# johnnyjana730/MVIN

Measured on AMD Instinct MI355X. Metric: (user,item) pairs scored/sec @ dim=64 hop=2 fan-out=32; % HBM roofline, higher is better.
Workload: dtype f32

## Files before the change

### include/mvin_hip.h

```cpp
#ifndef MVIN_HIP_H
#define MVIN_HIP_H

#include <stddef.h>
#include <stdint.h>

#ifdef __cplusplus
extern "C" {
#endif

#define MVIN_ABI_VERSION 12
#define MVIN_API __attribute__((visibility("default")))
#define MVIN_MAX_DIM 256
#define MVIN_MAX_SRC 8

MVIN_API int mvin_abi_version(void);
MVIN_API const char* mvin_last_error(void);

MVIN_API int mvin_debug_read_trace(long long* host_dst, size_t n);

MVIN_API size_t mvin_ent_elems(int B, int K, int levels);
MVIN_API size_t mvin_rel_elems(int B, int K, int levels);

MVIN_API int mvin_expand_ids(const int32_t* adj_entity, const int32_t* adj_relation,
                    const int64_t* items_i64, const int32_t* items_i32,
                    int B, int K, int levels, int n_entity,
                    int32_t* ent_out, int32_t* rel_out, void* stream);

MVIN_API int mvin_rel_score(const float* relation_emb, const float* urh_weights, int nR, int D,
                   float* t_out, void* stream);

typedef struct {
    const float* src[MVIN_MAX_SRC];
    const int32_t* ids[MVIN_MAX_SRC];
    int nsrc;
    int Dsrc;
    int Dout;
    int64_t rows;
    const float* W;
    const float* bias;
    const float* rowbias;
    int rows_per_group;
    int relu;
    int ids64;
    int sum_sources;
    float* out;
    int64_t ldo;
    int nz;
    int64_t w_zstride, bias_zstride, out_zstride;
    const float* score_u;
    float* score_out;
    float* sigmoid_out;
    int src_bf16;
    int64_t src_rows;
} mvin_linear_args;
MVIN_API int mvin_linear_fwd(const mvin_linear_args* args, void* stream);

MVIN_API int mvin_gather_attn_fwd(const float* table, const int32_t* adj_entity, const int32_t* adj_relation,
                         const int32_t* node_ids, const float* rel_score,
                         const float* self_vec, const float* Wc, const float* c_child,
                         const float* Wagg, const float* bagg,
                         int B, int N, int K, int D, int n_entity,
                         float* out, float* probs, void* stream);

MVIN_API int mvin_gather_attn_l2_fwd(const void* table, const int32_t* adj_entity, const int32_t* adj_relation,
                            const int32_t* parent_ids, const float* t0, const float* t1,
                            const float* W1, const float* W2, const float* b1, const float* b2,
                            const float* q, const float* A0, const float* a0,
                            int B, int parents_per_pair, int K, int D, int n_entity, int nR,
                            float* nagg0, float* nagg1, float* probs_parent, float* probs_child,
                            int table_bf16, void* stream);
MVIN_API int mvin_gather_attn_l2_fwd_i64(const void* table, const int32_t* adj_entity, const int32_t* adj_relation,
                                const int64_t* parent_ids, const float* t0, const float* t1,
                                const float* W1, const float* W2, const float* b1, const float* b2,
                                const float* q, const float* A0, const float* a0,
                                int B, int parents_per_pair, int K, int D, int n_entity, int nR,
                                float* nagg0, float* nagg1, float* probs_parent, float* probs_child,
                                int table_bf16, void* stream);
MVIN_API int mvin_gather_attn_l2_supported(int D, int K);
MVIN_API int mvin_gather_attn_l2_enc_fwd(const void* table, const int32_t* enc_entity, const int32_t* enc_relation,
                                const void* parent_ids, int parent_ids_i64, const float* t0, const float* t1,
                                const float* W1, const float* W2, const float* b1, const float* b2,
                                const float* q, const float* A0, const float* a0,
                                int B, int parents_per_pair, int K, int D, int n_entity, int nR,
                                float* nagg0, float* nagg1, int table_bf16, void* stream);
MVIN_API int mvin_gather_attn_l2_enc_supported(int D, int K);
MVIN_API int mvin_gather_attn_l2_prj_supported(int D, int K, int adjacency_encoded, int n_entity, int nR);
MVIN_API int mvin_project_rows(const float* src, int64_t rows, int D, const float* W1, const float* W2, const float* b1,
                               const float* b2, float* out, void* stream);
MVIN_API size_t mvin_project_tables_elems(int n_entity, int D);
MVIN_API int mvin_project_tables(const float* entity_emb, const float* W1, const float* W2, const float* b1, const float* b2,
                                 const float* A0, const float* a0, int attention, int K, int n_entity, int D, float* ws,
                                 void* stream);
MVIN_API int mvin_gather_attn_l2_prj_fwd(const float* ws, const int32_t* enc_entity, const int32_t* enc_relation, int adjacency_encoded,
                                const void* parent_ids, int parent_ids_i64, const float* t0, const float* t1, const float* q,
                                int B, int parents_per_pair, int K, int D, int n_entity, int nR, float* nagg0, float* nagg1,
                                void* stream);
MVIN_API size_t mvin_order_by_key_ws_elems(int64_t B);
MVIN_API int mvin_order_by_key(const int64_t* keys_i64, const int32_t* keys_i32, int64_t B, int32_t* workspace, int32_t* order, void* stream);
MVIN_API int mvin_gather_attn_l2_prj_ordered_fwd(const float* ws, const int32_t* enc_entity, const int32_t* enc_relation, int adjacency_encoded,
                                const void* parent_ids, int parent_ids_i64, const int32_t* order, const float* t0, const float* t1,
                                const float* q, int B, int parents_per_pair, int K, int D, int n_entity, int nR, float* nagg0,
                                float* nagg1, void* stream);
MVIN_API int mvin_gather_attn_l2_agg_supported(int D, int K, int n_entity, int nR);
MVIN_API size_t mvin_entity_aggregates_elems(int n_entity, int D);
MVIN_API int mvin_entity_aggregates(const float* ws, const int32_t* enc_entity, const int32_t* enc_relation, const float* t0, int K, int D,
                                    int n_entity, int nR, float* agg, void* stream);
MVIN_API int mvin_gather_attn_l2_agg_fwd(const float* ws, const float* agg, const int32_t* enc_entity, const int32_t* enc_relation,
                                const void* parent_ids, int parent_ids_i64, const int32_t* order, const float* t0, const float* t1,
                                const float* q, int B, int parents_per_pair, int K, int D, int n_entity, int nR, float* nagg0,
                                float* nagg1, void* stream);
MVIN_API int mvin_score_l2_folded_supported(int D, int K, int n_entity, int nR);
MVIN_API size_t mvin_fold_tables_elems(int n_entity, int D);
MVIN_API int mvin_fold_tables(const float* entity_emb, const int32_t* enc_entity, const int32_t* enc_relation, const float* t0, const float* W0,
                              const float* b0, const float* W1, const float* b1, const float* W2, const float* b2, const float* A0,
                              const float* a0, const float* Wmix, const float* bmix, const float* A1, int K, int D, int n_entity, int nR,
                              float* ws, void* stream);
MVIN_API int mvin_fold_tables_ex(const float* entity_emb, const int32_t* enc_entity, const int32_t* enc_relation, const float* t0, const float* W0,
                                 const float* b0, const float* W1, const float* b1, const float* W2, const float* b2, const float* A0,
                                 const float* a0, const float* Wmix, const float* bmix, const float* A1, int aggregates, int K, int D,
                                 int n_entity, int nR, float* ws, void* stream);
MVIN_API int mvin_score_l2_folded_gather_supported(int D, int K, int n_entity, int nR);
MVIN_API int mvin_score_l2_folded_gather_fwd(const float* ws, const int32_t* enc_entity, const int32_t* enc_relation, const int64_t* items_i64,
                                             const int32_t* items_i32, const int32_t* order, const float* t0, const float* t1, const float* q,
                                             const float* user_o, const float* A1, const float* a1, const float* Wmix, int64_t B, int K, int D,
                                             int n_entity, int nR, float* item_emb, float* scores, float* sig, void* stream);
MVIN_API int mvin_score_l2_folded_fwd(const float* ws, const int32_t* enc_entity, const int32_t* enc_relation, const int64_t* items_i64,
                                      const int32_t* items_i32, const float* t0, const float* t1, const float* q, const float* user_o,
                                      const float* A1, const float* a1, const float* Wmix, int64_t B, int K, int D, int n_entity, int nR,
                                      float* out0, float* z2, float* item_emb, float* scores, float* sig, void* stream);
MVIN_API int mvin_gather_attn_l2_variant(int D, int K, int64_t n_parents, int n_entity, int want_probs);
MVIN_API int mvin_gather_attn_l2_variant_ex(int D, int K, int64_t n_parents, int n_entity, int want_probs, int table_bf16);
MVIN_API int mvin_probe_gather_l2(const void* table, const int32_t* child_ids, const int32_t* grandchild_ids, int64_t n_parents, int K,
                         int D, int n_entity, int table_bf16, float* sums, void* stream);

MVIN_API int mvin_agg_fwd(const float* self_vec, const float* neigh, const int32_t* rel_ids,
                 const float* rel_score, const float* Wagg, const float* bagg,
                 int B, int N, int K, int D, float* out, float* probs, void* stream);

MVIN_API int mvin_ripple_attn_fwd(const float* entity_emb, const int32_t* score_ids, const int32_t* rel_ids,
                         const int32_t* value_ids, const float* V, const float* w, int mode,
                         int B, int Nm, int D, int nR, float* out, int64_t ldo, void* stream);
MVIN_API int mvin_ripple_attn_fwd_ex(const void* entity_emb, const int32_t* score_ids, const int32_t* rel_ids,
                            const int32_t* value_ids, const float* V, const float* w, int mode,
                            int B, int Nm, int D, int nR, float* out, int64_t ldo, int table_bf16, void* stream);

MVIN_API int mvin_key_addressing_fwd(const void* entity_emb, const float* V, const float* w,
                            const int32_t* const* mem_h, const int32_t* const* mem_r,
                            const int32_t* const* mem_t, int P, int B, int Nm, int D, int nR, int n_entity,
                            float* out, int64_t ldo, int table_bf16, void* stream);
MVIN_API int mvin_key_addressing_supported(int Nm, int D);
MVIN_API int mvin_key_addressing_users_fwd(const void* entity_emb, const float* V, const float* w, const int32_t* uts,
                                  const int64_t* users_i64, const int32_t* users_i32, int P, int B, int Nm, int D, int nR,
                                  int n_entity, int n_user, float* out, int64_t ldo, int table_bf16, void* stream);

MVIN_API int mvin_key_addressing_grouped_fwd(const void* entity_emb, const float* relation_kge, const float* w,
                                    const int32_t* uts, const int32_t* seg_user, const int32_t* seg_ptr,
                                    const int32_t* nseg_dev, const int32_t* pair_index, const int64_t* items_i64,
                                    const int32_t* items_i32, int nseg, int B, int P, int Nm, int D, int nR, int n_entity, int n_user,
                                    float* out, int64_t ldo, int table_bf16, void* stream);
MVIN_API int mvin_key_addressing_grouped_supported(int D, int P, int Nm, int nR);
MVIN_API int mvin_user_records_len(int P, int Nm, int nR);
MVIN_API int mvin_user_records_supported(int D, int P, int Nm, int nR, int table_bf16);
MVIN_API int mvin_build_user_records(const int32_t* uts, int n_user, int P, int Nm, int nR, int n_entity, int32_t* records, void* stream);
MVIN_API int mvin_key_addressing_grouped_rec_fwd(const void* entity_emb, const float* relation_kge, const float* w,
                                        const int32_t* uts, const int32_t* user_records, const int32_t* seg_user,
                                        const int32_t* seg_ptr, const int32_t* nseg_dev, const int32_t* pair_index,
                                        const int64_t* items_i64, const int32_t* items_i32, int nseg, int B, int P, int Nm, int D,
                                        int nR, int n_entity, int n_user, float* out, int64_t ldo, int table_bf16, void* stream);
MVIN_API size_t mvin_project_relations_elems(int n_entity, int nR, int D);
MVIN_API int mvin_project_relations(const float* entity_emb, const float* relation_kge, const float* w, int n_entity, int nR, int D,
                                    float* ws, void* stream);
MVIN_API int mvin_key_addressing_grouped_er_supported(int D, int P, int Nm, int nR, int n_entity, int has_set);
MVIN_API int mvin_key_addressing_grouped_er_fwd(const void* entity_emb, const float* relation_kge, const float* w,
                                       const int32_t* uts, const int32_t* user_records, const float* er_ws, const int32_t* seg_user,
                                       const int32_t* seg_ptr, const int32_t* nseg_dev, const int32_t* pair_index,
                                       const int64_t* items_i64, const int32_t* items_i32, int nseg, int B, int P, int Nm, int D,
                                       int nR, int n_entity, int n_user, float* out, int64_t ldo, void* stream);
MVIN_API int mvin_key_addressing_flash_supported(int D, int P, int Nm, int nR, int n_entity);
MVIN_API size_t mvin_key_addressing_flash_tables_elems(int n_entity, int nR, int D, int P, int has_set);
MVIN_API int mvin_key_addressing_flash_prepare(const float* entity_emb, const float* relation_kge, const float* w,
                                      const float* user_mlp_W, int n_entity, int nR, int D, int P, float* ws, void* stream);
MVIN_API size_t mvin_key_addressing_flash_ws_elems(int64_t B, int n_user);
MVIN_API int mvin_key_addressing_flash_fwd(const float* entity_emb, const float* ws, const int32_t* user_records,
                                  const int32_t* seg_user, const int32_t* seg_ptr, const int32_t* nseg_dev, const int32_t* pair_index,
                                  const int64_t* items_i64, const int32_t* items_i32, int64_t B, int P, int Nm, int D, int nR,
                                  int n_entity, int n_user, int has_set, const float* user_mlp_b, float* user_o,
                                  int32_t* sched_ws, void* stream);
MVIN_API int mvin_group_pairs_by_user(const int64_t* users_i64, const int32_t* users_i32, int64_t B, int n_user, int32_t* workspace,
                             int32_t* seg_user, int32_t* seg_ptr, int32_t* nseg, int32_t* pair_index, void* stream);

MVIN_API int mvin_row_softmax_fwd(const float* x, int64_t rows, int n, float* out, void* stream);

MVIN_API int mvin_mix_neighbor_vectors_fwd(const float* neighbor_vectors, const float* neighbor_relations, const float* user_embeddings,
                                           const float* logits_or_null, int B, int N, int K, int D, float* out, float* probs_or_null,
                                           void* stream);

MVIN_API int mvin_l2_tail_fwd(const void* entity_emb, const int64_t* items_i64, const int32_t* items_i32, const float* q,
                     const float* user_o, const float* nagg0, const float* nagg1, const float* W0, const float* b0,
                     const float* A0, const float* a0, const float* A1, const float* a1, const float* Wmix,
                     const float* bmix, int64_t B, int D, int n_entity, float* item_emb, float* scores, float* sig,
                     int table_bf16, void* stream);
MVIN_API int mvin_l2_tail_supported(int D);

typedef struct {
    const void* entity_emb;
    const int32_t* adj_entity;
    const int32_t* adj_relation;
    const float* relation_kge;
    const float* h_set_w;
    const float* user_mlp_W;
    const float* user_mlp_b;
    const float* t0;
    const float* t1;
    const float* W0;
    const float* b0;
    const float* W1;
    const float* b1;
    const float* W2;
    const float* b2;
    const float* A0;
    const float* a0;
    const float* A1;
    const float* a1;
    const float* Wmix;
    const float* bmix;
    const int64_t* items;
    const int32_t* const* mem_h;
    const int32_t* const* mem_r;
    const int32_t* const* mem_t;
    const int32_t* uts;
    const int64_t* users;
    float* V;
    float* o_cat;
    int32_t* parents;
    float* nagg0;
    float* nagg1;
    float* user_o;
    float* item_emb;
    float* scores;
    float* sig;
    int64_t B;
    int D, K, P, Nm, n_entity, n_relation, table_bf16;
    int n_user;
    const int32_t* enc_entity;
    const int32_t* enc_relation;
    int32_t* group_ws;
    const int32_t* user_records;
    int depth;
    float* prj_tables;
    float* ka_er;
    float* ka_flash;
    int32_t* item_order_ws;
    float* agg_tables;
    float* fold_ws;
    int fold_gather;
} mvin_score_l2_args;
MVIN_API int mvin_score_l2_fwd(const mvin_score_l2_args* args, void* stream);

MVIN_API int mvin_score_small_fwd(const mvin_score_l2_args* args, int group, void* stream);
MVIN_API int mvin_score_small_supported(int D, int K, int P, int Nm, int nR);

MVIN_API int mvin_gather_rows(const void* table, const int32_t* ids, int64_t n, int row_bytes, void* out, void* stream);
MVIN_API int mvin_scatter_rows(void* table, const int32_t* ids, int64_t n, int row_bytes, const void* rows, void* stream);
MVIN_API int mvin_shard_space_ids(const void* ids, int ids_are_i64, int64_t n, int world, int n_local, void* out, void* stream);

MVIN_API int mvin_gather_mix_fwd(const void* table, const int32_t* adj_entity, const int32_t* adj_relation,
                        const int32_t* node_ids, const float* rel_score, const float* rowbias, int64_t nodes,
                        int nodes_per_group, int K, int D, int n_entity, int nR, int relu, float* out,
                        int table_bf16, void* stream);


MVIN_API int mvin_gather_attn_fwd_ex(const void* table, const int32_t* adj_entity, const int32_t* adj_relation,
                            const int32_t* node_ids, const float* rel_score, const float* self_vec,
                            const float* Wc, const float* c_child, const float* Wagg, const float* bagg,
                            int B, int N, int K, int D, int n_entity, float* out, float* probs,
                            float* s_out, float* z_out, int table_bf16, void* stream);
MVIN_API int mvin_agg_fwd_ex(const float* self_vec, const float* neigh, const int32_t* rel_ids, const float* rel_score,
                    const float* Wagg, const float* bagg, int B, int N, int K, int D, float* out, float* probs,
                    float* s_out, float* z_out, void* stream);

MVIN_API int mvin_eltwise(int mode, int64_t n, float* x, float* y, float* z, float* w, float* accum, float alpha,
                 float beta, float beta1, float beta2, float eps, int D, int N, void* stream);
// ... 156 lines not shown
```

### mvin_amd/_lib.py

```python
import ctypes as C
import os

from . import build as _build

MAX_SRC = 8
ABI_VERSION = 12

_c_f32p = C.c_void_p
_c_i32p = C.c_void_p


class LinearArgs(C.Structure):
    _fields_ = [
        ("src", C.c_void_p * MAX_SRC),
        ("ids", C.c_void_p * MAX_SRC),
        ("nsrc", C.c_int),
        ("Dsrc", C.c_int),
        ("Dout", C.c_int),
        ("rows", C.c_int64),
        ("W", C.c_void_p),
        ("bias", C.c_void_p),
        ("rowbias", C.c_void_p),
        ("rows_per_group", C.c_int),
        ("relu", C.c_int),
        ("ids64", C.c_int),
        ("sum_sources", C.c_int),
        ("out", C.c_void_p),
        ("ldo", C.c_int64),
        ("nz", C.c_int),
        ("w_zstride", C.c_int64),
        ("bias_zstride", C.c_int64),
        ("out_zstride", C.c_int64),
        ("score_u", C.c_void_p),
        ("score_out", C.c_void_p),
        ("sigmoid_out", C.c_void_p),
        ("src_bf16", C.c_int),
        ("src_rows", C.c_int64),
    ]


class WgradProblem(C.Structure):
    _fields_ = [
        ("lin", LinearArgs),
        ("dY", C.c_void_p),
        ("ldy", C.c_int64),
        ("dy_zstride", C.c_int64),
        ("mask", C.c_void_p),
        ("ldm", C.c_int64),
        ("mask_zstride", C.c_int64),
        ("dW", C.c_void_p),
        ("dw_zstride", C.c_int64),
        ("db", C.c_void_p),
        ("db_zstride", C.c_int64),
    ]


class ScoreL2Args(C.Structure):
    _fields_ = [(n, C.c_void_p) for n in (
        "entity_emb", "adj_entity", "adj_relation", "relation_kge", "h_set_w", "user_mlp_W", "user_mlp_b", "t0", "t1",
        "W0", "b0", "W1", "b1", "W2", "b2", "A0", "a0", "A1", "a1", "Wmix", "bmix", "items", "mem_h", "mem_r", "mem_t",
        "uts", "users", "V", "o_cat", "parents", "nagg0", "nagg1", "user_o", "item_emb", "scores", "sig")] + [
        ("B", C.c_int64)] + [(n, C.c_int) for n in ("D", "K", "P", "Nm", "n_entity", "n_relation", "table_bf16", "n_user")] + [
        ("enc_entity", C.c_void_p), ("enc_relation", C.c_void_p), ("group_ws", C.c_void_p),
        ("user_records", C.c_void_p), ("depth", C.c_int), ("prj_tables", C.c_void_p), ("ka_er", C.c_void_p),
        ("ka_flash", C.c_void_p), ("item_order_ws", C.c_void_p), ("agg_tables", C.c_void_p), ("fold_ws", C.c_void_p), ("fold_gather", C.c_int)]


SIGNATURES = {
    "mvin_abi_version": (C.c_int, []),
    "mvin_last_error": (C.c_char_p, []),
    "mvin_debug_read_trace": (C.c_int, [C.c_void_p, C.c_size_t]),
    "mvin_l2_tail_fwd": (C.c_int, [C.c_void_p] * 15 + [C.c_int64, C.c_int, C.c_int] + [C.c_void_p] * 3 + [C.c_int, C.c_void_p]),
    "mvin_l2_tail_supported": (C.c_int, [C.c_int]),
    "mvin_score_l2_fwd": (C.c_int, [C.c_void_p, C.c_void_p]),
    "mvin_score_small_fwd": (C.c_int, [C.c_void_p, C.c_int, C.c_void_p]),
    "mvin_mix_neighbor_vectors_fwd": (C.c_int, [C.c_void_p] * 4 + [C.c_int] * 4 + [C.c_void_p] * 3),
    "mvin_score_small_supported": (C.c_int, [C.c_int] * 5),
    "mvin_project_rows": (C.c_int, [C.c_void_p, C.c_int64, C.c_int] + [C.c_void_p] * 6),
    "mvin_project_tables_elems": (C.c_size_t, [C.c_int, C.c_int]),
    "mvin_project_tables": (C.c_int, [C.c_void_p] * 7 + [C.c_int] * 4 + [C.c_void_p] * 2),
    "mvin_gather_attn_l2_prj_fwd": (C.c_int, [C.c_void_p] * 3 + [C.c_int] + [C.c_void_p] + [C.c_int] + [C.c_void_p] * 3 + [C.c_int] * 6 + [C.c_void_p] * 3),
    "mvin_topk_rows_supported": (C.c_int, [C.c_int]),
    "mvin_topk_rows_ws_bytes": (C.c_int64, [C.c_int64, C.c_int64, C.c_int]),
    "mvin_topk_rows": (C.c_int, [C.c_void_p, C.c_int64, C.c_int64, C.c_int64, C.c_void_p, C.c_int64] + [C.c_void_p] * 4
                       + [C.c_int] + [C.c_void_p] * 4),
    "mvin_rank_positives_ws_bytes": (C.c_int64, [C.c_int64] * 3),
    "mvin_rank_positives": (C.c_int, [C.c_void_p, C.c_int64, C.c_int64, C.c_int64, C.c_void_p, C.c_int64] + [C.c_void_p] * 9),
    "mvin_kg_explore_ws_bytes": (C.c_int64, [C.c_int64, C.c_int64]),
    "mvin_kg_field": (C.c_int, [C.c_void_p] * 3 + [C.c_int64, C.c_int64, C.c_void_p, C.c_int64, C.c_int] + [C.c_void_p] * 4),
    "mvin_kg_explore": (C.c_int, [C.c_void_p] * 3 + [C.c_int64, C.c_int64, C.c_void_p, C.c_void_p, C.c_int, C.c_void_p, C.c_int64,
                                  C.c_int] + [C.c_void_p] * 4),
    "mvin_ctr_counts_ws_bytes": (C.c_int64, [C.c_int64, C.c_int64]),
    "mvin_ctr_counts": (C.c_int, [C.c_void_p, C.c_void_p, C.c_int64, C.c_int64, C.c_int64, C.c_void_p, C.c_void_p, C.c_void_p]),
    "mvin_order_by_key_ws_elems": (C.c_size_t, [C.c_int64]),
    "mvin_order_by_key": (C.c_int, [C.c_void_p, C.c_void_p, C.c_int64, C.c_void_p, C.c_void_p, C.c_void_p]),
    "mvin_gather_attn_l2_prj_ordered_fwd": (C.c_int, [C.c_void_p] * 3 + [C.c_int] + [C.c_void_p] + [C.c_int] + [C.c_void_p] * 4 + [C.c_int] * 6 + [C.c_void_p] * 3),
    "mvin_gather_attn_l2_agg_supported": (C.c_int, [C.c_int] * 4),
    "mvin_entity_aggregates_elems": (C.c_size_t, [C.c_int] * 2),
    "mvin_entity_aggregates": (C.c_int, [C.c_void_p] * 4 + [C.c_int] * 4 + [C.c_void_p] * 2),
    "mvin_gather_attn_l2_agg_fwd": (C.c_int, [C.c_void_p] * 5 + [C.c_int] + [C.c_void_p] * 4 + [C.c_int] * 6 + [C.c_void_p] * 3),
    "mvin_score_l2_folded_supported": (C.c_int, [C.c_int] * 4),
    "mvin_fold_tables_elems": (C.c_size_t, [C.c_int] * 2),
    "mvin_fold_tables": (C.c_int, [C.c_void_p] * 15 + [C.c_int] * 4 + [C.c_void_p] * 2),
    "mvin_fold_tables_ex": (C.c_int, [C.c_void_p] * 15 + [C.c_int] * 5 + [C.c_void_p] * 2),
    "mvin_score_l2_folded_gather_supported": (C.c_int, [C.c_int] * 4),
    "mvin_score_l2_folded_gather_fwd": (C.c_int, [C.c_void_p] * 13 + [C.c_int64] + [C.c_int] * 4 + [C.c_void_p] * 4),
    "mvin_score_l2_folded_fwd": (C.c_int, [C.c_void_p] * 12 + [C.c_int64] + [C.c_int] * 4 + [C.c_void_p] * 6),
    "mvin_gather_rows": (C.c_int, [C.c_void_p, C.c_void_p, C.c_int64, C.c_int, C.c_void_p, C.c_void_p]),
    "mvin_scatter_rows": (C.c_int, [C.c_void_p, C.c_void_p, C.c_int64, C.c_int, C.c_void_p, C.c_void_p]),
    "mvin_linear_wgrad_multi": (C.c_int, [C.c_void_p, C.c_int, C.c_void_p]),
    "mvin_shard_space_ids": (C.c_int, [C.c_void_p, C.c_int, C.c_int64, C.c_int, C.c_int, C.c_void_p, C.c_void_p]),
    "mvin_key_addressing_grouped_fwd": (C.c_int, [C.c_void_p] * 10 + [C.c_int] * 8 + [C.c_void_p, C.c_int64, C.c_int, C.c_void_p]),
    "mvin_key_addressing_grouped_rec_fwd": (C.c_int, [C.c_void_p] * 11 + [C.c_int] * 8 + [C.c_void_p, C.c_int64, C.c_int, C.c_void_p]),
    "mvin_project_relations_elems": (C.c_size_t, [C.c_int] * 3),
    "mvin_project_relations": (C.c_int, [C.c_void_p] * 3 + [C.c_int] * 3 + [C.c_void_p] * 2),
    "mvin_key_addressing_grouped_er_supported": (C.c_int, [C.c_int] * 6),
    "mvin_key_addressing_flash_supported": (C.c_int, [C.c_int] * 5),
    "mvin_key_addressing_flash_tables_elems": (C.c_size_t, [C.c_int] * 5),
    "mvin_key_addressing_flash_prepare": (C.c_int, [C.c_void_p] * 4 + [C.c_int] * 4 + [C.c_void_p] * 2),
    "mvin_key_addressing_flash_ws_elems": (C.c_size_t, [C.c_int64, C.c_int]),
    "mvin_key_addressing_flash_fwd": (C.c_int, [C.c_void_p] * 9 + [C.c_int64] + [C.c_int] * 7 + [C.c_void_p] * 4),
    "mvin_key_addressing_grouped_er_fwd": (C.c_int, [C.c_void_p] * 12 + [C.c_int] * 8 + [C.c_void_p, C.c_int64, C.c_void_p]),
    "mvin_user_records_len": (C.c_int, [C.c_int] * 3),
    "mvin_user_records_supported": (C.c_int, [C.c_int] * 5),
    "mvin_build_user_records": (C.c_int, [C.c_void_p, C.c_int, C.c_int, C.c_int, C.c_int, C.c_int, C.c_void_p, C.c_void_p]),
    "mvin_key_addressing_grouped_supported": (C.c_int, [C.c_int] * 4),
    "mvin_ent_elems": (C.c_size_t, [C.c_int, C.c_int, C.c_int]),
    "mvin_rel_elems": (C.c_size_t, [C.c_int, C.c_int, C.c_int]),
    "mvin_expand_ids": (C.c_int, [_c_i32p, _c_i32p, C.c_void_p, _c_i32p, C.c_int, C.c_int, C.c_int,
                                  C.c_int, _c_i32p, _c_i32p, C.c_void_p]),
    "mvin_rel_score": (C.c_int, [_c_f32p, _c_f32p, C.c_int, C.c_int, _c_f32p, C.c_void_p]),
    "mvin_linear_fwd": (C.c_int, [C.POINTER(LinearArgs), C.c_void_p]),
    "mvin_gather_attn_fwd": (C.c_int, [_c_f32p, _c_i32p, _c_i32p, _c_i32p, _c_f32p, _c_f32p, _c_f32p,
                                       _c_f32p, _c_f32p, _c_f32p, C.c_int, C.c_int, C.c_int, C.c_int,
                                       C.c_int, _c_f32p, _c_f32p, C.c_void_p]),
    "mvin_gather_attn_l2_fwd": (C.c_int, [_c_f32p, _c_i32p, _c_i32p, _c_i32p, _c_f32p, _c_f32p, _c_f32p,
                                          _c_f32p, _c_f32p, _c_f32p, _c_f32p, _c_f32p, _c_f32p, C.c_int, C.c_int,
                                          C.c_int, C.c_int, C.c_int, C.c_int, _c_f32p, _c_f32p, _c_f32p,
                                          _c_f32p, C.c_int, C.c_void_p]),
    "mvin_gather_attn_l2_fwd_i64": (C.c_int, [_c_f32p, _c_i32p, _c_i32p, C.c_void_p, _c_f32p, _c_f32p, _c_f32p,
                                              _c_f32p, _c_f32p, _c_f32p, _c_f32p, _c_f32p, _c_f32p, C.c_int, C.c_int,
                                              C.c_int, C.c_int, C.c_int, C.c_int, _c_f32p, _c_f32p, _c_f32p,
                                              _c_f32p, C.c_int, C.c_void_p]),
    "mvin_gather_attn_l2_supported": (C.c_int, [C.c_int, C.c_int]),
    "mvin_gather_attn_l2_enc_fwd": (C.c_int, [_c_f32p, _c_i32p, _c_i32p, C.c_void_p, C.c_int, _c_f32p, _c_f32p, _c_f32p,
                                              _c_f32p, _c_f32p, _c_f32p, _c_f32p, _c_f32p, _c_f32p, C.c_int, C.c_int,
                                              C.c_int, C.c_int, C.c_int, C.c_int, _c_f32p, _c_f32p, C.c_int, C.c_void_p]),
    "mvin_gather_attn_l2_enc_supported": (C.c_int, [C.c_int, C.c_int]),
    "mvin_gather_attn_l2_prj_supported": (C.c_int, [C.c_int, C.c_int, C.c_int, C.c_int, C.c_int]),
    "mvin_encode_adjacency": (C.c_int, [_c_i32p, _c_i32p, C.c_int, C.c_int, _c_i32p, _c_i32p, _c_i32p, C.c_void_p]),
    "mvin_gather_attn_l2_variant": (C.c_int, [C.c_int, C.c_int, C.c_int64, C.c_int, C.c_int]),
    "mvin_gather_attn_l2_variant_ex": (C.c_int, [C.c_int, C.c_int, C.c_int64, C.c_int, C.c_int, C.c_int]),
    "mvin_probe_gather_l2": (C.c_int, [C.c_void_p, C.c_void_p, C.c_void_p, C.c_int64, C.c_int, C.c_int, C.c_int, C.c_int,
                                      C.c_void_p, C.c_void_p]),
    "mvin_agg_fwd": (C.c_int, [_c_f32p, _c_f32p, _c_i32p, _c_f32p, _c_f32p, _c_f32p, C.c_int, C.c_int,
                               C.c_int, C.c_int, _c_f32p, _c_f32p, C.c_void_p]),
    "mvin_key_addressing_fwd": (C.c_int, [_c_f32p, _c_f32p, _c_f32p, C.POINTER(C.c_void_p),
                                          C.POINTER(C.c_void_p), C.POINTER(C.c_void_p), C.c_int, C.c_int,
                                          C.c_int, C.c_int, C.c_int, C.c_int, _c_f32p, C.c_int64, C.c_int,
                                          C.c_void_p]),
    "mvin_key_addressing_supported": (C.c_int, [C.c_int, C.c_int]),
    "mvin_count_ids": (C.c_int, [C.c_void_p, C.c_int64, C.c_int, C.c_void_p, C.c_void_p]),
    "mvin_group_pairs_by_user": (C.c_int, [C.c_void_p, C.c_void_p, C.c_int64, C.c_int, C.c_void_p, C.c_void_p, C.c_void_p,
                                           C.c_void_p, C.c_void_p, C.c_void_p]),
    "mvin_key_addressing_users_fwd": (C.c_int, [C.c_void_p, C.c_void_p, C.c_void_p, C.c_void_p, C.c_void_p, C.c_void_p,
                                                C.c_int, C.c_int, C.c_int, C.c_int, C.c_int, C.c_int, C.c_int, C.c_void_p,
                                                C.c_int64, C.c_int, C.c_void_p]),
    "mvin_row_softmax_fwd": (C.c_int, [_c_f32p, C.c_int64, C.c_int, _c_f32p, C.c_void_p]),
    "mvin_gather_mix_fwd": (C.c_int, [_c_f32p, _c_i32p, _c_i32p, _c_i32p, _c_f32p, _c_f32p, C.c_int64, C.c_int,
                                      C.c_int, C.c_int, C.c_int, C.c_int, C.c_int, _c_f32p, C.c_int, C.c_void_p]),
    "mvin_sample_adjacency": (C.c_int, [C.c_void_p, _c_i32p, _c_i32p, C.c_int, C.c_int, C.c_uint64, _c_i32p,
                                        _c_i32p, C.c_void_p]),
    "mvin_build_ripple_sets": (C.c_int, [C.c_void_p, _c_i32p, _c_i32p, C.c_void_p, _c_i32p, C.c_int, C.c_int,
                                         C.c_int, C.c_int, C.c_uint64, _c_i32p, C.c_void_p]),
    "mvin_sample_negatives_supported": (C.c_int, [C.c_int]),
    "mvin_sample_negatives": (C.c_int, [C.c_void_p, _c_i32p, _c_i32p, C.c_void_p, C.c_int, C.c_int, C.c_uint64, C.c_uint64,
                                        _c_i32p, C.c_void_p, C.c_void_p]),
    "mvin_sample_negatives_weighted_supported": (C.c_int, [C.c_int]),
    "mvin_sample_negatives_weighted": (C.c_int, [C.c_void_p, _c_i32p, _c_i32p, C.c_void_p, C.c_int, C.c_int, C.c_void_p, C.c_void_p,
                                                 C.c_uint64, C.c_uint64, _c_i32p, C.c_void_p, C.c_void_p]),
    "mvin_rank_head": (C.c_int, [_c_f32p, _c_f32p, _c_f32p, C.c_int64, C.c_int, C.c_int, C.c_int, C.c_float] + [_c_f32p] * 5
                       + [C.c_void_p, C.c_void_p]),
    "mvin_rank_head_offset": (C.c_int, [_c_f32p, _c_f32p, _c_f32p, _c_f32p, C.c_int64, C.c_int, C.c_int, C.c_int, C.c_float]
                              + [_c_f32p] * 5 + [C.c_void_p, C.c_void_p]),
    "mvin_select_negatives": (C.c_int, [_c_f32p, C.c_void_p, _c_f32p, C.c_void_p, C.c_int64, C.c_int, C.c_int, C.c_int, C.c_uint64,
                                        C.c_uint64, C.c_void_p, _c_f32p, _c_f32p, C.c_void_p, C.c_void_p]),
    "mvin_gather_attn_fwd_ex": (C.c_int, [_c_f32p, _c_i32p, _c_i32p, _c_i32p, _c_f32p, _c_f32p, _c_f32p,
                                          _c_f32p, _c_f32p, _c_f32p, C.c_int, C.c_int, C.c_int, C.c_int,
                                          C.c_int, _c_f32p, _c_f32p, _c_f32p, _c_f32p, C.c_int, C.c_void_p]),
    "mvin_agg_fwd_ex": (C.c_int, [_c_f32p, _c_f32p, _c_i32p, _c_f32p, _c_f32p, _c_f32p, C.c_int, C.c_int,
                                  C.c_int, C.c_int, _c_f32p, _c_f32p, _c_f32p, _c_f32p, C.c_void_p]),
    "mvin_l2_adam_multi": (C.c_int, [C.c_void_p, C.c_int, C.c_int64, _c_f32p, _c_f32p, _c_f32p, _c_f32p, C.c_int,
                                     C.c_float, C.c_float, C.c_float, C.c_float, C.c_void_p]),
    "mvin_l2_adam_multi_dev": (C.c_int, [C.c_void_p, C.c_int, C.c_int64, _c_f32p, _c_f32p, _c_f32p, _c_f32p, C.c_int,
                                         _c_f32p, C.c_float, C.c_float, C.c_float, C.c_void_p]),
    "mvin_grad_guard": (C.c_int, [C.c_void_p, C.c_int, C.c_int64, _c_f32p, C.c_void_p, C.c_int, C.c_void_p, _c_f32p, C.c_int,
                                  C.c_void_p, C.c_int, C.c_void_p]),
    "mvin_l2_adam_multi_guarded": (C.c_int, [C.c_void_p, C.c_int, C.c_int64, _c_f32p, _c_f32p, _c_f32p, _c_f32p, C.c_int,
                                             C.c_void_p, C.c_float, C.c_float, C.c_float, C.c_void_p]),
    "mvin_eltwise": (C.c_int, [C.c_int, C.c_int64, _c_f32p, _c_f32p, _c_f32p, _c_f32p, _c_f32p, C.c_float,
                               C.c_float, C.c_float, C.c_float, C.c_float, C.c_int, C.c_int, C.c_void_p]),
    "mvin_scatter_add_rows": (C.c_int, [_c_f32p, C.c_void_p, C.c_int, _c_f32p, C.c_int64, C.c_int, C.c_float,
                                        C.c_void_p]),
    "mvin_linear_wgrad": (C.c_int, [C.POINTER(LinearArgs), _c_f32p, C.c_int64, C.c_int64, _c_f32p, C.c_int64,
                                    C.c_int64, _c_f32p, C.c_int64, _c_f32p, C.c_int64, C.c_void_p]),
    "mvin_agg_bwd": (C.c_int, [_c_f32p, _c_i32p, _c_i32p, _c_i32p, _c_f32p, _c_i32p, _c_f32p, _c_f32p, _c_f32p, C.c_int64,
                               C.c_int, C.c_int, C.c_int, _c_f32p, _c_f32p, _c_f32p, C.c_void_p]),
    "mvin_rel_score_bwd": (C.c_int, [_c_f32p, _c_f32p, _c_f32p, C.c_int, C.c_int, _c_f32p, _c_f32p, C.c_void_p]),
    "mvin_key_addressing_bwd": (C.c_int, [_c_f32p, _c_f32p, _c_f32p, C.POINTER(C.c_void_p), C.POINTER(C.c_void_p),
                                          C.POINTER(C.c_void_p), C.c_int, C.c_int, C.c_int, C.c_int, C.c_int,
                                          _c_f32p, C.c_int64, C.c_float, _c_f32p, _c_f32p, _c_f32p, C.c_void_p]),
    "mvin_key_addressing_bwd_reg": (C.c_int, [_c_f32p, _c_f32p, _c_f32p, C.POINTER(C.c_void_p), C.POINTER(C.c_void_p),
                                              C.POINTER(C.c_void_p), C.c_int, C.c_int, C.c_int, C.c_int, C.c_int,
                                              _c_f32p, C.c_int64, C.c_float, _c_f32p, _c_f32p, _c_f32p, C.c_int,
                                              _c_f32p, _c_f32p, C.c_void_p, C.c_int, C.c_void_p]),
    "mvin_key_addressing_bwd_adds_item_grad": (C.c_int, [C.c_int, C.c_int, C.c_int, C.c_int]),
    "mvin_ripple_attn_fwd": (C.c_int, [_c_f32p, _c_i32p, _c_i32p, _c_i32p, _c_f32p, _c_f32p, C.c_int,
                                       C.c_int, C.c_int, C.c_int, C.c_int, _c_f32p, C.c_int64,
                                       C.c_void_p]),
    "mvin_ripple_attn_fwd_ex": (C.c_int, [C.c_void_p, _c_i32p, _c_i32p, _c_i32p, _c_f32p, _c_f32p, C.c_int,
                                          C.c_int, C.c_int, C.c_int, C.c_int, _c_f32p, C.c_int64, C.c_int,
                                          C.c_void_p]),
}

_lib = None


class MvinHipError(RuntimeError):
    pass


def lib_path():
    return _build.LIB_PATH


def load():
    global _lib
    if _lib is not None:
        return _lib
    path = lib_path()
    if not os.path.exists(path):
        raise MvinHipError(
            f"{path} is missing: build it with `python -m mvin_amd.build` (hipcc, gfx950). "
            "mvin_amd has no CPU fallback.")
    import torch
    hip_rt = os.path.join(os.path.dirname(torch.__file__), "lib", "libamdhip64.so")
    if os.path.exists(hip_rt):
        C.CDLL(hip_rt, mode=C.RTLD_GLOBAL)
    lib = C.CDLL(path)
    for name, (res, args) in SIGNATURES.items():
        fn = getattr(lib, name)
        fn.restype = res
        fn.argtypes = args
    ver = lib.mvin_abi_version()
    if ver != ABI_VERSION:
        raise MvinHipError(f"libmvin_hip.so ABI version {ver}, expected {ABI_VERSION}")
    _lib = lib
    return lib


# ... 5 lines not shown
```

### mvin_amd/csrc/mvin_abi.hip

```cpp
#include <cstdlib>
#include <cstdarg>
#include <cstdio>
#include <string>

#include "mvin_kernels.h"
#include "mvin_fused_agg.h"

namespace {

thread_local std::string g_last_error;

int fail(int code, const char* fmt, ...) {
    char buf[512];
    va_list ap;
    va_start(ap, fmt);
    vsnprintf(buf, sizeof(buf), fmt, ap);
    va_end(ap);
    g_last_error = buf;
    return code;
}

int hip_result(hipError_t e, const char* what) {
    if (e == hipSuccess) return 0;
    fail((int)e, "%s: %s", what, hipGetErrorString(e));
// ... 520 lines not shown
    mvin::FusedL2Args f{};
    f.K = K;
    f.nR = nR;
    f.P = n_parents > 0 ? n_parents : 1;
    f.prj = 1;
    f.parents_per_pair = 1;
    f.max_id = (unsigned)(n_entity - 1);
    static const int32_t present = 0;
    f.adj_r = &present;
    f.table_bytes = (uint64_t)n_entity * (uint64_t)D * 4;
    f.adj_bytes = (uint64_t)n_entity * (uint64_t)K * 4;
    return mvin::fused_agg_applies(f, D);
}

int mvin_gather_attn_l2_agg_supported(int D, int K, int n_entity, int nR) { return agg_applies(D, K, n_entity, nR, 1) ? 1 : 0; }

size_t mvin_entity_aggregates_elems(int n_entity, int D) { return n_entity > 0 && D > 0 ? (size_t)2 * n_entity * D : 0; }

int mvin_entity_aggregates(const float* ws, const int32_t* enc_entity, const int32_t* enc_relation, const float* t0, int K, int D,
                           int n_entity, int nR, float* agg, void* stream) {
    const char* who = "mvin_entity_aggregates";
    if (!ws || !enc_entity || !enc_relation || !agg) return fail(-1, "%s: null pointer", who);
    if (!agg_applies(D, K, n_entity, nR, 1))
        return fail(-3, "%s: D = 64, K in {16, 32, 64}, n_entity <= 2^24, tables < 1 GiB, adjacency < 2 GiB, nR <= 4096 (D=%d K=%d n_entity=%d nR=%d)",
                    who, D, K, n_entity, nR);
    mvin::EntityAggArgs f{};
    const size_t tab = (size_t)n_entity * D;
    f.tabS = ws;
    f.selfG = ws + tab;
    f.tabG = ws + 2 * tab;
    f.adj_e = enc_entity;
    f.adj_r = enc_relation;
    f.t0 = t0;
    f.outS = agg;
    f.outG = agg + tab;
    f.n_entity = n_entity;
    f.K = K;
    f.nR = nR;
    f.table_bytes = (uint64_t)n_entity * (uint64_t)D * 4;
    f.adj_bytes = (uint64_t)n_entity * (uint64_t)K * 4;
    return hip_result(mvin::launch_entity_aggregates(f, (hipStream_t)stream), who);
}

int mvin_gather_attn_l2_agg_fwd(const float* ws, const float* agg, const int32_t* enc_entity, const int32_t* enc_relation,
                                const void* parent_ids, int parent_ids_i64, const int32_t* order, const float* t0, const float* t1,
                                const float* q, int B, int parents_per_pair, int K, int D, int n_entity, int nR, float* nagg0,
                                float* nagg1, void* stream) {
    if (!ws || !agg || n_entity <= 0 || D <= 0) return fail(-1, "mvin_gather_attn_l2_agg_fwd: null workspace / bad sizes");
    const float* blk = ws + (size_t)3 * n_entity * D;
    const float* Wv = blk + (size_t)3 * D * D;
    const float* b1c = Wv + (size_t)D * D;
    return gather_attn_l2_impl(ws, enc_entity, enc_relation, reinterpret_cast<const int32_t*>(parent_ids), parent_ids_i64 ? 2 : 1, t0, t1,
                               blk, Wv, b1c, b1c + D, q, blk, nullptr, B, parents_per_pair, K, D, n_entity, nR, nagg0, nagg1, nullptr,
                               nullptr, 0, stream, true, true, order, agg);
}

static bool fold_gather_applies(int D, int K, int n_entity, int nR, int64_t B);

static bool fold_applies(int D, int K, int n_entity, int nR, int64_t B) {
    if (D == 64) return agg_applies(D, K, n_entity, nR, B);
    static const char* e = getenv("MVIN_L2_AGG");
    if (e && e[0] == '0') return false;
    if (n_entity <= 0 || nR <= 0 || nR > 4096 || !mvin::fused_fold_supported(D, K)) return false;
    const uint64_t tb = (uint64_t)n_entity * (uint64_t)D * 4, ab = (uint64_t)n_entity * (uint64_t)K * 4;
    return tb < (1ull << 30) && ab < (1ull << 31) && n_entity <= (1 << 24) && (B <= 0 || (uint64_t)B * D * 4 < (1ull << 31)) &&
           mvin::fused_fold_lds_bytes(D, nR, K) <= 48 * 1024;
}

static size_t fold_blk_elems(int D) { return (size_t)12 * D * D + (size_t)3 * D; }

size_t mvin_fold_tables_elems(int n_entity, int D) {
    return n_entity > 0 && D > 0 ? (size_t)6 * n_entity * D + fold_blk_elems(D) : 0;
}

int mvin_score_l2_folded_supported(int D, int K, int n_entity, int nR) { return fold_applies(D, K, n_entity, nR, 1) ? 1 : 0; }

int mvin_fold_tables(const float* entity_emb, const int32_t* enc_entity, const int32_t* enc_relation, const float* t0, const float* W0,
                     const float* b0, const float* W1, const float* b1, const float* W2, const float* b2, const float* A0, const float* a0,
                     const float* Wmix, const float* bmix, const float* A1, int K, int D, int n_entity, int nR, float* ws, void* stream) {
    return mvin_fold_tables_ex(entity_emb, enc_entity, enc_relation, t0, W0, b0, W1, b1, W2, b2, A0, a0, Wmix, bmix, A1, 1, K, D, n_entity, nR, ws,
                               stream);
}

static int fold_tables_check(const char* who, const float* entity_emb, const int32_t* enc_entity, const int32_t* enc_relation, const float* W0,
                             const float* W1, const float* W2, const float* A0, const float* Wmix, const float* A1, int aggregates, int K, int D,
                             int n_entity, int nR, const float* ws) {
    if (!entity_emb || !enc_entity || !enc_relation || !W0 || !W1 || !W2 || !A0 || !Wmix || !A1 || !ws) return fail(-1, "%s: null pointer", who);
    if (!(aggregates ? fold_applies(D, K, n_entity, nR, 1) : fold_gather_applies(D, K, n_entity, nR, 1)))
        return fail(-3, "%s: D = 64 with K in {16, 32, 64} or D = 32 with K in {16, 32}; n_entity <= 2^24, tables < 1 GiB, adjacency < 2 GiB, nR <= 4096 "
                        "(D=%d K=%d n_entity=%d nR=%d)", who, D, K, n_entity, nR);
    return 0;
}

static int fold_tables_block(const char* who, const float* t0, const float* W0, const float* b0, const float* W1, const float* b1, const float* W2,
                             const float* b2, const float* A0, const float* a0, const float* Wmix, const float* bmix, const float* A1, int K, int D,
                             int n_entity, float* ws, void* stream) {
    const float c = t0 ? 1.f / (float)K : 1.f;
    return hip_result(mvin::launch_fold_prepare(W0, b0, W1, b1, W2, b2, A0, a0, Wmix, bmix, A1, c, D, ws + (size_t)6 * n_entity * D,
                                                (hipStream_t)stream), who);
}

static int fold_tables_aggregates(const char* who, const int32_t* enc_entity, const int32_t* enc_relation, const float* t0, int K, int D,
                                  int n_entity, int nR, float* ws, void* stream) {
    const size_t tab = (size_t)n_entity * D;
    mvin::EntityAggArgs f{};
    f.tabS = ws;
    f.selfS = ws + 2 * tab;
    f.tabG = ws + tab;
    f.selfG = ws;
    f.adj_e = enc_entity;
    f.adj_r = enc_relation;
    f.t0 = t0;
    f.outS = ws + 4 * tab;
    f.outG = ws + 5 * tab;
    f.n_entity = n_entity;
    f.K = K;
    f.D = D;
    f.nR = nR;
    f.table_bytes = (uint64_t)tab * 4;
    f.adj_bytes = (uint64_t)n_entity * (uint64_t)K * 4;
    return hip_result(mvin::launch_entity_aggregates(f, (hipStream_t)stream), who);
}

int mvin_fold_tables_ex(const float* entity_emb, const int32_t* enc_entity, const int32_t* enc_relation, const float* t0, const float* W0,
                        const float* b0, const float* W1, const float* b1, const float* W2, const float* b2, const float* A0, const float* a0,
                        const float* Wmix, const float* bmix, const float* A1, int aggregates, int K, int D, int n_entity, int nR, float* ws,
                        void* stream) {
    const char* who = "mvin_fold_tables";
    if (int rc = fold_tables_check(who, entity_emb, enc_entity, enc_relation, W0, W1, W2, A0, Wmix, A1, aggregates, K, D, n_entity, nR, ws)) return rc;
    if (int rc = fold_tables_block(who, t0, W0, b0, W1, b1, W2, b2, A0, a0, Wmix, bmix, A1, K, D, n_entity, ws, stream)) return rc;
    float* blk = ws + (size_t)6 * n_entity * D;
    if (D == 64) {
        if (int rc = build_entity_tables(who, entity_emb, n_entity, nullptr, 0, nullptr, nullptr, 0, nullptr, blk, ws, stream)) return rc;
    } else {
        mvin_linear_args l{};
        l.src[0] = entity_emb;
        l.nsrc = 1;
        l.Dsrc = D;
        l.Dout = D;
        l.rows = n_entity;
        l.rows_per_group = 1;
        l.W = blk;
        l.w_zstride = (int64_t)D * D;
        l.out = ws;
        l.ldo = D;
        l.nz = 4;
        l.out_zstride = (int64_t)n_entity * D;
        if (int rc = mvin_linear_fwd(&l, stream)) return rc;
    }
    if (!aggregates) return 0;
    return fold_tables_aggregates(who, enc_entity, enc_relation, t0, K, D, n_entity, nR, ws, stream);
}

int mvin_score_l2_folded_fwd(const float* ws, const int32_t* enc_entity, const int32_t* enc_relation, const int64_t* items_i64,
                             const int32_t* items_i32, const float* t0, const float* t1, const float* q, const float* user_o, const float* A1,
                             const float* a1, const float* Wmix, int64_t B, int K, int D, int n_entity, int nR, float* out0, float* z2,
                             float* item_emb, float* scores, float* sig, void* stream) {
    const char* who = "mvin_score_l2_folded_fwd";
    if (!ws || !enc_entity || !enc_relation || !q || !user_o || !A1 || !Wmix || !scores) return fail(-1, "%s: null pointer", who);
    if ((items_i64 == nullptr) == (items_i32 == nullptr)) return fail(-1, "%s: exactly one of items_i64 / items_i32", who);
    if (B <= 0 || B >= (int64_t(1) << 31)) return fail(-2, "%s: B=%lld", who, (long long)B);
    if (!fold_applies(D, K, n_entity, nR, B)) return fail(-3, "%s: unsupported shape / sizes D=%d K=%d n_entity=%d nR=%d B=%lld", who, D, K, n_entity, nR, (long long)B);
    const size_t tab = (size_t)n_entity * D;
    const float* blk = ws + 6 * tab;
    const float* Wv = blk + (size_t)4 * D * D;
    const float* Wq = Wv + (size_t)D * D;
    const float* bv = Wq + (size_t)D * D;
    const float* bq = bv + D;
    const float* bm = bq + D;
    static const bool two = getenv("MVIN_L2_FOLD_TWO") && atoi(getenv("MVIN_L2_FOLD_TWO")) != 0;
    if (!two || D != 64)
    {
        const float* Wp = bm + D;
        const size_t DD = (size_t)D * D;
        return hip_result(mvin::launch_score_l2_folded(ws + 4 * tab, ws + 3 * tab, enc_entity, enc_relation,
                                                       items_i64 ? reinterpret_cast<const int32_t*>(items_i64) : items_i32, items_i64 ? 2 : 1, t1, q,
                                                       user_o, Wp, bq, Wp + DD, bv, Wp + 2 * DD, Wp + 3 * DD, a1, Wp + 4 * DD, Wp + 5 * DD, bm,
                                                       item_emb, scores, sig, B, K, D, nR, n_entity, (hipStream_t)stream),
                          who);
    }
    if (!out0 || !z2) return fail(-1, "%s: the two-launch variant (MVIN_L2_FOLD_TWO=1) needs the out0 / z2 scratch rows", who);
    mvin::FusedL2Args f{};
    f.table = ws;
    f.agg = const_cast<float*>(ws + 4 * tab);
    f.adj_e = enc_entity;
    f.adj_r = enc_relation;
    f.parent_ids = items_i64 ? reinterpret_cast<const int32_t*>(items_i64) : items_i32;
    f.pid_stride = items_i64 ? 2 : 1;
    f.t0 = t0;
    f.t1 = t1;
    f.W1 = Wq;
    f.b1 = bq;
    f.W2 = Wv;
    f.b2 = bv;
    f.q = q;
    f.nagg0 = out0;
    f.nagg1 = z2;
    f.P = B;
    f.table_bytes = (uint64_t)tab * 4;
    f.adj_bytes = (uint64_t)n_entity * (uint64_t)K * 4;
    f.parents_per_pair = 1;
    f.K = K;
    f.nR = nR;
    f.max_id = (unsigned)(n_entity - 1);
    f.prj = 1;
    f.fold = 1;
    if (int rc = hip_result(mvin::launch_gather_attn_l2_agg(f, (hipStream_t)stream), who)) return rc;
    mvin::TailFoldArgs t{};
    t.M0 = ws + 3 * tab;
    t.items64 = items_i64;
    t.items32 = items_i32;
    t.q = q;
    t.user_o = user_o;
    t.out0 = out0;
    t.z2 = z2;
    t.Wqm = blk + (size_t)3 * D * D;
    t.A1 = A1;
    t.a1 = a1;
    t.Wmix = Wmix;
    t.bm = bm;
    t.item_emb = item_emb;
    t.scores = scores;
    t.sig = sig;
    t.B = B;
    t.n_entity = n_entity;
    return hip_result(mvin::launch_l2_tail_fold(t, (hipStream_t)stream), who);
}

static bool fold_gather_applies(int D, int K, int n_entity, int nR, int64_t B) {
    if (D != 64 || (K != 16 && K != 32) || n_entity <= 0 || nR <= 0 || nR > 4096) return false;
    static const char* e = getenv("MVIN_L2_FOLD_GATHER");
    if (e && e[0] == '0') return false;
    const uint64_t tb = (uint64_t)n_entity * (uint64_t)D * 4, ab = (uint64_t)n_entity * (uint64_t)K * 4;
    return tb < (1ull << 30) && ab < (1ull << 31) && n_entity <= (1 << 24) && (B <= 0 || (uint64_t)B * D * 4 < (1ull << 31)) &&
           mvin::fused_wppfold_lds_bytes(nR, K) <= 48 * 1024;
}

int mvin_score_l2_folded_gather_supported(int D, int K, int n_entity, int nR) { return fold_gather_applies(D, K, n_entity, nR, 1) ? 1 : 0; }

int mvin_score_l2_folded_gather_fwd(const float* ws, const int32_t* enc_entity, const int32_t* enc_relation, const int64_t* items_i64,
                                    const int32_t* items_i32, const int32_t* order, const float* t0, const float* t1, const float* q,
                                    const float* user_o, const float* A1, const float* a1, const float* Wmix, int64_t B, int K, int D,
                                    int n_entity, int nR, float* item_emb, float* scores, float* sig, void* stream) {
    const char* who = "mvin_score_l2_folded_gather_fwd";
    if (!ws || !enc_entity || !enc_relation || !q || !user_o || !A1 || !Wmix || !scores) return fail(-1, "%s: null pointer", who);
    if ((items_i64 == nullptr) == (items_i32 == nullptr)) return fail(-1, "%s: exactly one of items_i64 / items_i32", who);
    if (B <= 0 || B >= (int64_t(1) << 31)) return fail(-2, "%s: B=%lld", who, (long long)B);
    if (!fold_gather_applies(D, K, n_entity, nR, B))
        return fail(-3, "%s: D = 64, K in {16, 32}; n_entity <= 2^24, tables < 1 GiB, adjacency < 2 GiB (D=%d K=%d n_entity=%d nR=%d B=%lld)", who, D, K,
                    n_entity, nR, (long long)B);
    const size_t tab = (size_t)n_entity * D, DD = (size_t)D * D;
    const float* blk = ws + 6 * tab;
    const float* bv = blk + 6 * DD;
    const float* bq = bv + D;
    const float* bm = bq + D;
    const float* Wp = bm + D;
    mvin::FoldArgs f{};
    f.tables = ws;
    f.M0 = ws + 3 * tab;
    f.adj_e = enc_entity;
    f.adj_r = enc_relation;
    f.items = items_i64 ? reinterpret_cast<const int32_t*>(items_i64) : items_i32;
    f.pid_stride = items_i64 ? 2 : 1;
    f.order = order;
    f.t0 = t0;
    f.t1 = t1;
    f.q = q;
    f.user_o = user_o;
    f.Wq = Wp, f.bq = bq, f.Wv = Wp + DD, f.bv = bv, f.Wqm = Wp + 2 * DD, f.A1 = Wp + 3 * DD, f.a1 = a1, f.Wm1 = Wp + 4 * DD, f.Wm2 = Wp + 5 * DD, f.bm = bm;
    f.item_emb = item_emb, f.scores = scores, f.sig = sig;
    f.B = B, f.K = K, f.nR = nR;
    f.max_id = (unsigned)(n_entity - 1);
    f.table_bytes = (uint64_t)tab * 4;
    f.adj_bytes = (uint64_t)n_entity * (uint64_t)K * 4;
    return hip_result(mvin::launch_score_l2_folded_gather(f, (hipStream_t)stream), who);
}

int mvin_encode_adjacency(const int32_t* adj_entity, const int32_t* adj_relation, int n_entity, int K, int32_t* cnt,
                          int32_t* enc_entity, int32_t* enc_relation, void* stream) {
    const char* who = "mvin_encode_adjacency";
    if (!adj_entity || !cnt || !enc_entity || !enc_relation) return fail(-1, "%s: null pointer", who);
    if (n_entity <= 0 || n_entity > (1 << 24) || K <= 0 || K > 128)
        return fail(-2, "%s: n_entity=%d K=%d (n_entity <= 2^24, K <= 128)", who, n_entity, K);
    return hip_result(mvin::launch_encode_adjacency(adj_entity, adj_relation, n_entity, K, cnt, enc_entity, enc_relation,
                                                    (hipStream_t)stream), who);
}

int mvin_gather_attn_l2_fwd(const void* table, const int32_t* adj_entity, const int32_t* adj_relation,
                            const int32_t* parent_ids, const float* t0, const float* t1, const float* W1,
                            const float* W2, const float* b1, const float* b2, const float* q,
                            const float* A0, const float* a0, int B, int parents_per_pair, int K, int D, int n_entity, int nR,
                            float* nagg0, float* nagg1, float* probs_parent, float* probs_child,
                            int table_bf16, void* stream) {
    return gather_attn_l2_impl(table, adj_entity, adj_relation, parent_ids, 1, t0, t1, W1, W2, b1, b2, q, A0, a0, B,
                               parents_per_pair, K, D, n_entity, nR, nagg0, nagg1, probs_parent, probs_child,
                               table_bf16, stream);
}

int mvin_gather_attn_l2_fwd_i64(const void* table, const int32_t* adj_entity, const int32_t* adj_relation,
                                const int64_t* parent_ids, const float* t0, const float* t1, const float* W1,
                                const float* W2, const float* b1, const float* b2, const float* q,
                                const float* A0, const float* a0, int B, int parents_per_pair, int K, int D, int n_entity, int nR,
                                float* nagg0, float* nagg1, float* probs_parent, float* probs_child,
                                int table_bf16, void* stream) {
    return gather_attn_l2_impl(table, adj_entity, adj_relation, reinterpret_cast<const int32_t*>(parent_ids), 2, t0, t1, W1, W2,
                               b1, b2, q, A0, a0, B, parents_per_pair, K, D, n_entity, nR, nagg0, nagg1, probs_parent,
                               probs_child, table_bf16, stream);
}

int mvin_agg_fwd(const float* self_vec, const float* neigh, const int32_t* rel_ids, const float* rel_score,
                 const float* Wagg, const float* bagg, int B, int N, int K, int D, float* out, float* probs,
                 void* stream) {
    return mvin_agg_fwd_ex(self_vec, neigh, rel_ids, rel_score, Wagg, bagg, B, N, K, D, out, probs, nullptr,
                           nullptr, stream);
}

int mvin_agg_fwd_ex(const float* self_vec, const float* neigh, const int32_t* rel_ids, const float* rel_score,
                    const float* Wagg, const float* bagg, int B, int N, int K, int D, float* out, float* probs,
                    float* s_out, float* z_out, void* stream) {
    mvin::GatherAttnArgs g{};
    g.s_out = s_out;
    g.z_out = z_out;
    g.gather = 0;
    g.neigh = neigh;
    g.rel_ids = rel_ids;
    g.rel_score = rel_score;
    g.self_vec = self_vec;
    g.Wagg = Wagg;
    g.bagg = bagg;
    g.out = out;
    g.probs = probs;
// ... 122 lines not shown
    if (B <= 0 || n_entity <= 0) return fail(-2, "%s: bad sizes B=%lld n_entity=%d", who, (long long)B, n_entity);
    mvin::TailArgs t{};
    t.E = entity_emb;
    t.items64 = items_i64;
    t.items32 = items_i32;
    t.q = q;
    t.user_o = user_o;
    t.nagg0 = nagg0;
    t.nagg1 = nagg1;
    t.W0 = W0;
    t.b0 = b0;
    t.A0 = A0;
    t.a0 = a0;
    t.A1 = A1;
    t.a1 = a1;
    t.Wmix = Wmix;
    t.bmix = bmix;
    t.item_emb = item_emb;
    t.scores = scores;
    t.sig = sig;
    t.B = B;
    t.table_bf16 = table_bf16;
    t.n_entity = n_entity;
    return hip_result(mvin::launch_l2_tail(t, D, (hipStream_t)stream), who);
}

static int flash_prepare_impl(const char* who, const float* entity_emb, const float* relation_kge, const float* w, const float* user_mlp_W,
                              int n_entity, int nR, int D, int P, float* ws, float* fold_ws, void* stream);

int mvin_score_l2_fwd(const mvin_score_l2_args* a, void* stream) {
    const char* who = "mvin_score_l2_fwd";
    if (!a) return fail(-1, "%s: null args", who);
    if (a->P < 1 || a->P > 8) return fail(-2, "%s: P=%d (1..8)", who, a->P);
    const bool grouped = a->uts && a->group_ws;
    if ((!a->V && !grouped) || !a->o_cat || !a->parents || !a->nagg0 || !a->nagg1 || !a->user_o || !a->scores || !a->items)
        return fail(-1, "%s: null workspace / output / items", who);
    if (a->uts && !a->users) return fail(-1, "%s: user_triplet_set given without user ids", who);
    if (a->group_ws && !a->uts) return fail(-1, "%s: group_ws is for the users feed (uts + users)", who);
    const int D = a->D, nR = a->n_relation;
    const int n_o = a->P + (a->h_set_w ? 1 : 0);
    mvin_linear_args l{};
    l.src[0] = reinterpret_cast<const float*>(a->entity_emb);
    l.ids[0] = reinterpret_cast<const int32_t*>(a->items);
    l.ids64 = 1;
    l.src_bf16 = a->table_bf16 ? 1 : 0;
    l.src_rows = a->n_entity;
    l.nsrc = 1;
    l.Dsrc = D;
    l.Dout = D;
    l.rows = a->B;
    l.W = a->relation_kge;
    l.rows_per_group = 1;
    l.out = a->V;
    l.ldo = (int64_t)nR * D;
    l.nz = nR;
    l.w_zstride = (int64_t)D * D;
    l.out_zstride = D;
    int rc = 0;
    bool flash = false;
    const bool fold_ok = a->fold_ws && a->enc_entity && a->enc_relation && a->W0 && a->W1 && a->W2 && !a->table_bf16;
    const int fold_form = !fold_ok ? 0 : a->fold_gather ? (fold_gather_applies(D, a->K, a->n_entity, nR, a->B) ? 2 : 0)
                                                        : (fold_applies(D, a->K, a->n_entity, nR, a->B) ? 1 : 0);
    bool fold_built = false;
    if (grouped) {
        int32_t* ws = a->group_ws;
        int32_t* seg_user = ws + 2 * (size_t)a->n_user + (size_t)a->B;
        int32_t* seg_ptr = seg_user + a->B;
        int32_t* nseg = seg_ptr + a->B + 2;
        int32_t* pair_index = nseg + 1;
        rc = mvin_group_pairs_by_user(a->users, nullptr, a->B, a->n_user, ws, seg_user, seg_ptr, nseg, pair_index, stream);
        if (rc) return rc;
        if (a->ka_flash && a->user_records && !a->table_bf16 && mvin::key_addr_flash_supported(D, a->P, a->Nm, nR, a->n_entity)) {
            if (fold_form) {
                rc = fold_tables_check("mvin_fold_tables", reinterpret_cast<const float*>(a->entity_emb), a->enc_entity, a->enc_relation, a->W0, a->W1,
                                       a->W2, a->A0, a->Wmix, a->A1, fold_form == 1, a->K, D, a->n_entity, nR, a->fold_ws);
                if (rc) return rc;
                rc = fold_tables_block("mvin_fold_tables", a->t0, a->W0, a->b0, a->W1, a->b1, a->W2, a->b2, a->A0, a->a0, a->Wmix, a->bmix, a->A1,
                                       a->K, D, a->n_entity, a->fold_ws, stream);
                if (rc) return rc;
                fold_built = true;
            }
            rc = flash_prepare_impl("mvin_key_addressing_flash_prepare", reinterpret_cast<const float*>(a->entity_emb), a->relation_kge, a->h_set_w,
                                    a->user_mlp_W, a->n_entity, nR, D, a->P, a->ka_flash, fold_built ? a->fold_ws : nullptr, stream);
            if (rc) return rc;
            if (mvin_key_addressing_flash_ws_elems(a->B, a->n_user) > (size_t)2 * a->n_user + (size_t)a->B)
                return fail(-2, "%s: group_ws too small for the flash form's scheduling scratch", who);
            rc = mvin_key_addressing_flash_fwd(reinterpret_cast<const float*>(a->entity_emb), a->ka_flash, a->user_records, seg_user, seg_ptr,
                                               nseg, pair_index, a->items, nullptr, a->B, a->P, a->Nm, D, nR, a->n_entity, a->n_user,
                                               a->h_set_w != nullptr, a->user_mlp_b, a->user_o, ws, stream);
            flash = true;
        } else if (a->ka_er && a->user_records && !a->table_bf16 &&
            mvin_key_addressing_grouped_er_supported(D, a->P, a->Nm, nR, a->n_entity, a->h_set_w != nullptr)) {
            rc = mvin_project_relations(reinterpret_cast<const float*>(a->entity_emb), a->relation_kge, a->h_set_w, a->n_entity, nR, D,
                                        a->ka_er, stream);
            if (rc) return rc;
            rc = mvin_key_addressing_grouped_er_fwd(a->entity_emb, a->relation_kge, a->h_set_w, a->uts, a->user_records, a->ka_er, seg_user,
                                                    seg_ptr, nseg, pair_index, a->items, nullptr, (int)a->B, (int)a->B, a->P, a->Nm, D, nR,
                                                    a->n_entity, a->n_user, a->o_cat, (int64_t)n_o * D, stream);
        } else
        rc = mvin_key_addressing_grouped_rec_fwd(a->entity_emb, a->relation_kge, a->h_set_w, a->uts, a->user_records, seg_user, seg_ptr,
                                                 nseg, pair_index, a->items, nullptr, (int)a->B, (int)a->B, a->P, a->Nm, D, nR,
                                                 a->n_entity, a->n_user, a->o_cat, (int64_t)n_o * D, a->table_bf16, stream);
    } else {
        rc = mvin_linear_fwd(&l, stream);
        if (rc) return rc;
    }
    if (grouped) {
    } else if (a->uts)
        rc = mvin_key_addressing_users_fwd(a->entity_emb, a->V, a->h_set_w, a->uts, a->users, nullptr, a->P, (int)a->B, a->Nm,
                                           D, nR, a->n_entity, a->n_user, a->o_cat, (int64_t)n_o * D, a->table_bf16, stream);
    else
        rc = mvin_key_addressing_fwd(a->entity_emb, a->V, a->h_set_w, a->mem_h, a->mem_r, a->mem_t, a->P, (int)a->B, a->Nm, D,
                                     nR, a->n_entity, a->o_cat, (int64_t)n_o * D, a->table_bf16, stream);
    if (rc) return rc;
    if (!flash) {
    mvin_linear_args u{};
    u.src[0] = a->o_cat;
    u.nsrc = 1;
    u.Dsrc = n_o * D;
    u.Dout = D;
    u.rows = a->B;
    u.W = a->user_mlp_W;
    u.bias = a->user_mlp_b;
    u.rows_per_group = 1;
    u.out = a->user_o;
    u.ldo = D;
    u.nz = 1;
    rc = mvin_linear_fwd(&u, stream);
    if (rc) return rc;
    }
    if (fold_form == 2) {
        if (!fold_built)
            rc = mvin_fold_tables_ex(reinterpret_cast<const float*>(a->entity_emb), a->enc_entity, a->enc_relation, a->t0, a->W0, a->b0, a->W1, a->b1,
                                     a->W2, a->b2, a->A0, a->a0, a->Wmix, a->bmix, a->A1, 0, a->K, D, a->n_entity, nR, a->fold_ws, stream);
        if (rc) return rc;
        const int32_t* order = nullptr;
        if (a->item_order_ws) {
            int32_t* ord = a->item_order_ws + mvin::order_ws_elems(a->B);
            rc = mvin_order_by_key(a->items, nullptr, a->B, a->item_order_ws, ord, stream);
            if (rc) return rc;
            order = ord;
        }
        return mvin_score_l2_folded_gather_fwd(a->fold_ws, a->enc_entity, a->enc_relation, a->items, nullptr, order, a->t0, a->t1, a->user_o,
                                               a->user_o, a->A1, a->a1, a->Wmix, a->B, a->K, D, a->n_entity, nR, a->item_emb, a->scores, a->sig,
                                               stream);
    }
    if (fold_form == 1) {
        if (fold_built)
            rc = fold_tables_aggregates("mvin_fold_tables", a->enc_entity, a->enc_relation, a->t0, a->K, D, a->n_entity, nR, a->fold_ws, stream);
        else
            rc = mvin_fold_tables(reinterpret_cast<const float*>(a->entity_emb), a->enc_entity, a->enc_relation, a->t0, a->W0, a->b0, a->W1, a->b1,
                                  a->W2, a->b2, a->A0, a->a0, a->Wmix, a->bmix, a->A1, a->K, D, a->n_entity, nR, a->fold_ws, stream);
        if (rc) return rc;
        return mvin_score_l2_folded_fwd(a->fold_ws, a->enc_entity, a->enc_relation, a->items, nullptr, a->t0, a->t1, a->user_o, a->user_o, a->A1,
                                        a->a1, a->Wmix, a->B, a->K, D, a->n_entity, nR, a->nagg0, a->nagg1, a->item_emb, a->scores, a->sig,
                                        stream);
    }
    const bool enc = a->enc_entity && a->enc_relation && mvin::fused_packed_supported(D, a->K);
    const bool d32 = mvin::fused_d32_supported(D, a->K);
    if ((enc || d32) && a->prj_tables && a->W1 && !a->table_bf16 && prj_applies(D, a->K, enc, a->n_entity, nR, a->B)) {
        rc = mvin_project_tables(reinterpret_cast<const float*>(a->entity_emb), a->W1, a->W2, a->b1, a->b2, a->A0, a->a0,
                                 a->t0 != nullptr, a->K, a->n_entity, D, a->prj_tables, stream);
        if (rc) return rc;
        const int32_t* order = nullptr;
        if (enc && a->agg_tables && agg_applies(D, a->K, a->n_entity, nR, a->B)) {
            rc = mvin_entity_aggregates(a->prj_tables, a->enc_entity, a->enc_relation, a->t0, a->K, D, a->n_entity, nR, a->agg_tables, stream);
            if (rc) return rc;
            if (a->item_order_ws) {
                int32_t* ord = a->item_order_ws + mvin::order_ws_elems(a->B);
                rc = mvin_order_by_key(a->items, nullptr, a->B, a->item_order_ws, ord, stream);
                if (rc) return rc;
                order = ord;
            }
            rc = mvin_gather_attn_l2_agg_fwd(a->prj_tables, a->agg_tables, a->enc_entity, a->enc_relation, a->items, 1, order, a->t0, a->t1,
                                             a->user_o, (int)a->B, 1, a->K, D, a->n_entity, nR, a->nagg0, a->nagg1, stream);
        } else {
        if (enc && a->item_order_ws && mvin::fused_wpp_supported(D, a->K) && nR <= 4096) {
            mvin::FusedL2Args f{};
            f.prj = 1, f.K = a->K, f.nR = nR, f.P = a->B, f.parents_per_pair = 1, f.max_id = (unsigned)(a->n_entity - 1);
            f.table_bytes = (uint64_t)a->n_entity * D * 4, f.adj_bytes = (uint64_t)a->n_entity * a->K * 4;
            f.adj_r = a->enc_relation, f.W1 = a->W1, f.W2 = a->W2, f.q = a->user_o;
            if (mvin::fused_wpp_applies(f, D)) {
                int32_t* ord = a->item_order_ws + mvin::order_ws_elems(a->B);
                rc = mvin_order_by_key(a->items, nullptr, a->B, a->item_order_ws, ord, stream);
                if (rc) return rc;
                order = ord;
            }
        }
        rc = mvin_gather_attn_l2_prj_ordered_fwd(a->prj_tables, enc ? a->enc_entity : a->adj_entity, enc ? a->enc_relation : a->adj_relation,
                                                 enc ? 1 : 0, a->items, 1, order, a->t0, a->t1, a->user_o, (int)a->B, 1, a->K, D, a->n_entity, nR,
                                                 a->nagg0, a->nagg1, stream);
        }
    } else
    rc = gather_attn_l2_impl(a->entity_emb, enc ? a->enc_entity : a->adj_entity, enc ? a->enc_relation : a->adj_relation,
                             reinterpret_cast<const int32_t*>(a->items), 2,
                             a->t0, a->t1, a->W1, a->W2, a->b1, a->b2, a->W1 ? a->user_o : nullptr, a->A0, a->a0,
                             (int)a->B, 1, a->K, D, a->n_entity, nR, a->nagg0, a->nagg1, nullptr, nullptr,
                             a->table_bf16, stream, enc);
    if (rc) return rc;
    return mvin_l2_tail_fwd(a->entity_emb, a->items, nullptr, a->W0 ? a->user_o : nullptr, a->user_o, a->nagg0, a->nagg1,
                            a->W0, a->b0, a->A0, a->a0, a->A1, a->a1, a->Wmix, a->bmix, a->B, D, a->n_entity, a->item_emb,
                            a->scores, a->sig, a->table_bf16, stream);
}

int mvin_score_small_supported(int D, int K, int P, int Nm, int nR) { return mvin::score_small_supported(D, K, P, Nm, nR) ? 1 : 0; }

int mvin_score_small_fwd(const mvin_score_l2_args* a, int group, void* stream) {
    const char* who = "mvin_score_small_fwd";
    if (!a) return fail(-1, "%s: null args", who);
    if (!mvin::score_small_supported(a->D, a->K, a->P, a->Nm, a->n_relation))
        return fail(-3, "%s: unsupported shape D=%d K=%d P=%d Nm=%d nR=%d", who, a->D, a->K, a->P, a->Nm, a->n_relation);
    if (a->depth < 0 || a->depth > 2) return fail(-2, "%s: depth=%d (1 or 2)", who, a->depth);
    const bool d1 = a->depth == 1;
    if (!a->entity_emb || !a->adj_entity || !a->relation_kge || !a->user_mlp_W || !a->A0 || (!d1 && !a->A1) || !a->Wmix || !a->items ||
        !a->user_o || !a->scores)
        return fail(-1, "%s: null table / weight / items / output", who);
    if ((a->W0 == nullptr) != (a->W1 == nullptr) || (!d1 && (a->W1 == nullptr) != (a->W2 == nullptr)))
        return fail(-1, "%s: W0 / W1 (/ W2) must be given together (User_orient) or not at all", who);
    if (a->uts ? !a->users : (!a->mem_h || !a->mem_r || !a->mem_t))
        return fail(-1, "%s: needs uts + users, or mem_h / mem_r / mem_t", who);
    if (a->B <= 0 || a->n_entity <= 0 || (a->uts && a->n_user <= 0)) return fail(-2, "%s: bad sizes B=%lld", who, (long long)a->B);
    const bool enc = a->enc_entity && a->enc_relation;
    if (enc && a->n_entity > (1 << 24)) return fail(-2, "%s: the encoded adjacency holds 24-bit ids", who);
    if (a->table_bf16) return fail(-3, "%s: fp32 entity table only", who);
    const uint64_t table_bytes = (uint64_t)a->n_entity * a->D * 4, adj_bytes = (uint64_t)a->n_entity * a->K * 4;
    if (table_bytes >= (1ull << 32) - 4096 || adj_bytes >= (1ull << 32) - 4096)
        return fail(-3, "%s: entity table / adjacency of 4 GiB or more (32-bit buffer offsets)", who);
    mvin::ScoreSmallArgs s{};
    s.E = a->entity_emb;
    s.adj_e = enc ? a->enc_entity : a->adj_entity;
    s.adj_r = enc ? a->enc_relation : a->adj_relation;
    s.R = a->relation_kge;
    s.w_h = a->h_set_w;
    s.Wu = a->user_mlp_W;
    s.bu = a->user_mlp_b;
    s.t0 = a->t0;
    s.t1 = a->t1;
    s.W0 = a->W0, s.b0 = a->b0, s.W1 = a->W1, s.b1 = a->b1, s.W2 = a->W2, s.b2 = a->b2;
    s.A0 = a->A0, s.a0 = a->a0, s.A1 = a->A1, s.a1 = a->a1, s.Wmix = a->Wmix, s.bmix = a->bmix;
    s.items = a->items;
    if (a->uts) {
        s.uts = a->uts;
        s.users = a->users;
    } else {
        for (int h = 0; h < a->P; ++h) {
            if (!a->mem_h[h] || !a->mem_r[h] || !a->mem_t[h]) return fail(-1, "%s: null ripple-set array of hop %d", who, h);
            s.mem_h[h] = a->mem_h[h], s.mem_r[h] = a->mem_r[h], s.mem_t[h] = a->mem_t[h];
        }
    }
    s.user_o = a->user_o, s.item_emb = a->item_emb, s.scores = a->scores, s.sig = a->sig;
    s.B = a->B;
    s.G = group;
    s.K = a->K, s.P = a->P, s.Nm = a->Nm, s.nR = a->n_relation, s.n_entity = a->n_entity, s.n_user = a->n_user > 0 ? a->n_user : 1;
    s.enc = enc ? 1 : 0;
    s.depth1 = d1 ? 1 : 0;
    s.table_bf16 = 0;
    s.table_bytes = table_bytes;
    s.adj_bytes = adj_bytes;
    return hip_result(mvin::launch_score_small(s, a->D, (hipStream_t)stream), who);
}

int mvin_gather_rows(const void* table, const int32_t* ids, int64_t n, int row_bytes, void* out, void* stream) {
    const char* who = "mvin_gather_rows";
    if (n < 0 || row_bytes <= 0 || (row_bytes & 3)) return fail(-2, "%s: n=%lld row_bytes=%d", who, (long long)n, row_bytes);
    if (n > 0 && (!table || !ids || !out)) return fail(-1, "%s: null pointer", who);
    return hip_result(mvin::launch_move_rows(const_cast<void*>(table), ids, n, row_bytes, out, false, (hipStream_t)stream), who);
}

int mvin_scatter_rows(void* table, const int32_t* ids, int64_t n, int row_bytes, const void* rows, void* stream) {
    const char* who = "mvin_scatter_rows";
    if (n < 0 || row_bytes <= 0 || (row_bytes & 3)) return fail(-2, "%s: n=%lld row_bytes=%d", who, (long long)n, row_bytes);
    if (n > 0 && (!table || !ids || !rows)) return fail(-1, "%s: null pointer", who);
    return hip_result(mvin::launch_move_rows(table, ids, n, row_bytes, const_cast<void*>(rows), true, (hipStream_t)stream), who);
}

int mvin_shard_space_ids(const void* ids, int ids_are_i64, int64_t n, int world, int n_local, void* out, void* stream) {
    const char* who = "mvin_shard_space_ids";
    if (n < 0 || world <= 0 || n_local <= 0) return fail(-2, "%s: n=%lld world=%d n_local=%d", who, (long long)n, world, n_local);
    if (n > 0 && (!ids || !out)) return fail(-1, "%s: null pointer", who);
    return hip_result(mvin::launch_shard_space_ids(ids, ids_are_i64 != 0, n, world, n_local, out, (hipStream_t)stream), who);
}

int mvin_group_pairs_by_user(const int64_t* users_i64, const int32_t* users_i32, int64_t B, int n_user, int32_t* workspace,
                             int32_t* seg_user, int32_t* seg_ptr, int32_t* nseg, int32_t* pair_index, void* stream) {
    const char* who = "mvin_group_pairs_by_user";
    if ((!users_i64 && !users_i32) || !workspace || !seg_user || !seg_ptr || !nseg || !pair_index)
        return fail(-1, "%s: null pointer", who);
    if (B <= 0 || B > 0x7fffffff || n_user <= 0) return fail(-2, "%s: bad sizes B=%lld n_user=%d", who, (long long)B, n_user);
    return hip_result(mvin::launch_group_pairs(users_i64, users_i32, B, n_user, workspace, workspace + n_user, workspace + 2 * (size_t)n_user,
                                               seg_user, seg_ptr,
                                               nseg, pair_index, (hipStream_t)stream), who);
}

int mvin_key_addressing_grouped_supported(int D, int P, int Nm, int nR) {
    return mvin::key_addr_grouped_supported(D, P, Nm, nR) ? 1 : 0;
}

int mvin_user_records_len(int P, int Nm, int nR) { return mvin::ka_rec_layout(P, Nm, nR).len; }

int mvin_user_records_supported(int D, int P, int Nm, int nR, int table_bf16) {
    return !table_bf16 && mvin::key_addr_static_supported(D, P, Nm, nR) ? 1 : 0;
}

int mvin_build_user_records(const int32_t* uts, int n_user, int P, int Nm, int nR, int n_entity, int32_t* records, void* stream) {
    const char* who = "mvin_build_user_records";
    if (!uts || !records) return fail(-1, "%s: null pointer", who);
    if (n_user <= 0 || n_entity <= 0) return fail(-2, "%s: bad sizes n_user=%d n_entity=%d", who, n_user, n_entity);
    if (mvin::ka_rec_layout(P, Nm, nR).len == 0) return fail(-3, "%s: no record form for P=%d Nm=%d nR=%d (P 1..8, Nm 1..256, nR 1..4096)", who, P, Nm, nR);
    return hip_result(mvin::launch_user_records(uts, n_user, P, Nm, nR, n_entity, records, (hipStream_t)stream), who);
// ... 631 lines not shown
```

### mvin_amd/csrc/mvin_fused_agg.h

```cpp
#pragma once
#include <cstdlib>
#include <type_traits>

#include "mvin_kernels.h"

namespace mvin {

typedef float f32x4 __attribute__((ext_vector_type(4)));
typedef float f32x2 __attribute__((ext_vector_type(2)));
typedef unsigned int u32x4 __attribute__((ext_vector_type(4)));
typedef unsigned int u32x2 __attribute__((ext_vector_type(2)));

constexpr int kAggWaves = 4;
constexpr int kAggUvLd = 132;
constexpr int kAggPad = 4;
constexpr unsigned kAggOob = 0xFFFFFFF0u;
constexpr unsigned kAggPadRow = 0xFFFFFE00u;
constexpr int agg_list_words(int K) { return 4 * 2 * (K + kAggPad); }
constexpr size_t fused_agg_lds_words(int nR, int K) { return (size_t)((nR + 3) & ~3) + (size_t)kAggWaves * (16 * kAggUvLd + agg_list_words(K)); }
size_t fused_agg_lds_bytes(int nR, int K);

__device__ __forceinline__ int agg_xor16_imax(int v) {
    const auto a = __builtin_amdgcn_permlane16_swap((unsigned)v, (unsigned)v, false, false);
    return max((int)a[0], (int)a[1]);
}
__device__ __forceinline__ int agg_xor32_imax(int v) {
    const auto a = __builtin_amdgcn_permlane32_swap((unsigned)v, (unsigned)v, false, false);
    return max((int)a[0], (int)a[1]);
}

__device__ __forceinline__ bool agg_logit_table(const float* t, int nR, float* sT, int tid, int lane) {
    float mx = -INFINITY, mn = INFINITY;
    if (t)
        for (int i = lane; i < nR; i += 64) {
            const float l = t[i];
            mx = fmaxf(mx, l), mn = fminf(mn, l);
        }
    else
        mx = mn = 0.f;
    mx = wave_max(mx), mn = -wave_max(-mn);
    const bool fast = __builtin_amdgcn_readfirstlane((mx - mn <= 60.f) ? 1 : 0) != 0;
    for (int i = tid; i < nR; i += kAggWaves * 64) {
        const float l = t ? t[i] : 0.f;
        sT[i] = fast ? lean_exp(fminf(l - mx, 0.f)) : l;
    }
    return fast;
}

template <int SPL, bool FAST, int LG = 4>
__device__ __forceinline__ void agg_row_weights(const unsigned (&cr)[SPL], bool att, const float* sT, unsigned rmax, float invK, float (&wk)[SPL]) {
    float lg[SPL];
    float mx = -INFINITY;
#pragma unroll
    for (int i = 0; i < SPL; ++i) {
        const float mu = (float)((cr[i] >> 16) & 0xFFu);
        const float l = att ? sT[min(cr[i] & 0xFFFFu, rmax)] : (FAST ? 1.f : 0.f);
        if constexpr (FAST) {
            wk[i] = mu * l;
        } else {
            wk[i] = mu;
            mx = fmaxf(mx, mu > 0.f ? l : -INFINITY);
            lg[i] = l;
        }
    }
    if (att) {
        float z = 0.f;
        if constexpr (FAST) {
#pragma unroll
            for (int i = 0; i < SPL; ++i) z += wk[i];
        } else {
            mx = group_max(mx, LG);
#pragma unroll
            for (int i = 0; i < SPL; ++i) {
                wk[i] *= lean_exp(fminf(lg[i] - mx, 0.f));
                z += wk[i];
            }
        }
        z = group_sum(z, LG);
        const float rz = z > 0.f ? invK * __builtin_amdgcn_rcpf(z) : 0.f;
#pragma unroll
        for (int i = 0; i < SPL; ++i) wk[i] *= rz;
    } else {
#pragma unroll
        for (int i = 0; i < SPL; ++i) wk[i] *= invK;
    }
}

template <int SPL>
__device__ __forceinline__ void agg_load_slots(__amdgpu_buffer_rsrc_t adjE, __amdgpu_buffer_rsrc_t adjR, unsigned co, unsigned (&ce)[SPL],
                                               unsigned (&cr)[SPL]) {
    if constexpr (SPL == 1) {
        ce[0] = __builtin_amdgcn_raw_buffer_load_b32(adjE, co, 0, 0);
        cr[0] = __builtin_amdgcn_raw_buffer_load_b32(adjR, co, 0, 0);
    } else if constexpr (SPL == 2) {
        const u32x2 e2 = __builtin_amdgcn_raw_buffer_load_b64(adjE, co, 0, 0);
        const u32x2 r2 = __builtin_amdgcn_raw_buffer_load_b64(adjR, co, 0, 0);
        ce[0] = e2[0], ce[1] = e2[1], cr[0] = r2[0], cr[1] = r2[1];
    } else {
        static_assert(SPL == 4, "SPL");
        const u32x4 e4 = __builtin_amdgcn_raw_buffer_load_b128(adjE, co, 0, 0);
        const u32x4 r4 = __builtin_amdgcn_raw_buffer_load_b128(adjR, co, 0, 0);
#pragma unroll
        for (int i = 0; i < 4; ++i) ce[i] = e4[i], cr[i] = r4[i];
    }
}

__device__ __forceinline__ float4 agg_row4(__amdgpu_buffer_rsrc_t tab, unsigned off) {
    const u32x4 r = __builtin_amdgcn_raw_buffer_load_b128(tab, off, 0, 0);
    return make_float4(__uint_as_float(r[0]), __uint_as_float(r[1]), __uint_as_float(r[2]), __uint_as_float(r[3]));
}


struct FoldArgs {
    const float* agg;
    const float* M0;
    const int32_t* adj_e;
    const int32_t* adj_r;
    const int32_t* items;
    const float* t1;
    const float* q;
    const float* user_o;
    const float *Wq, *bq, *Wv, *bv, *Wqm, *A1, *a1, *Wm1, *Wm2, *bm;
    float* item_emb;
    float* scores;
    float* sig;
    int64_t B;
    uint64_t table_bytes, adj_bytes;
    int K, nR, pid_stride;
    unsigned max_id;
    int dbg;
    const float* tables;
    const float* t0;
    const int32_t* order;
};

hipError_t launch_entity_aggregates_d32(const EntityAggArgs& a, hipStream_t st);
hipError_t launch_score_l2_folded_d32(const FoldArgs& f, hipStream_t st);
hipError_t launch_score_l2_folded_gather(const FoldArgs& f, hipStream_t st);
size_t fused_wppfold_lds_bytes(int nR, int K);

}
```

### mvin_amd/csrc/mvin_fused_agg.hip

```cpp
#include "mvin_fused_agg.h"

namespace mvin {

template <int K>
__global__ __launch_bounds__(kAggWaves * 64) void entity_aggregates_kernel(EntityAggArgs a) {
    constexpr int D = 64, SPL = K / 16;
    static_assert(K == 16 || K == 32 || K == 64, "K");
    extern __shared__ __attribute__((aligned(16))) float smem[];
    const int nRp = (a.nR + 3) & ~3;
    float* sT = smem;
    const int tid = threadIdx.x, lane = tid & 63, wave = tid >> 6;
    const int g = lane >> 4, c = lane & 15;
    unsigned* sLo = reinterpret_cast<unsigned*>(sT + nRp + wave * agg_list_words(K)) + g * (K + kAggPad);
    float* sLw = reinterpret_cast<float*>(reinterpret_cast<unsigned*>(sT + nRp + wave * agg_list_words(K)) + 4 * (K + kAggPad)) + g * (K + kAggPad);
    const bool att = a.t0 != nullptr;
    const float invK = 1.f / (float)K;
    const bool fast = agg_logit_table(a.t0, a.nR, sT, tid, lane);
    __syncthreads();

    const int tbytes = (int)a.table_bytes;
    const __amdgpu_buffer_rsrc_t tabS = __builtin_amdgcn_make_buffer_rsrc(const_cast<float*>(a.tabS), 0, tbytes, 0x00020000);
    const __amdgpu_buffer_rsrc_t tabG = __builtin_amdgcn_make_buffer_rsrc(const_cast<float*>(a.tabG), 0, tbytes, 0x00020000);
    const __amdgpu_buffer_rsrc_t selfS = __builtin_amdgcn_make_buffer_rsrc(const_cast<float*>(a.selfS), 0, a.selfS ? tbytes : 0, 0x00020000);
    const __amdgpu_buffer_rsrc_t selfG = __builtin_amdgcn_make_buffer_rsrc(const_cast<float*>(a.selfG), 0, tbytes, 0x00020000);
// ... 91 lines not shown
    const __amdgpu_buffer_rsrc_t out0 = __builtin_amdgcn_make_buffer_rsrc(a.nagg0, 0, (int)(a.P * D * 4), 0x00020000);
    const __amdgpu_buffer_rsrc_t out1 = __builtin_amdgcn_make_buffer_rsrc(a.nagg1, 0, (int)(a.P * D * 4), 0x00020000);
    const unsigned c16 = (unsigned)c * 16u;
    if (c < kAggPad) {
        sLo[K + c] = kAggPadRow;
        sLw[K + c] = 0.f;
    }

    const int64_t nbatch = (a.P + 15) >> 4;
    const int64_t nwaves = (int64_t)gridDim.x * kAggWaves;
    auto run = [&](auto fast_tag) {
        constexpr bool FAST = decltype(fast_tag)::value;
        for (int64_t batch = (int64_t)blockIdx.x * kAggWaves + wave; batch < nbatch; batch += nwaves) {
            const int64_t p_base = batch << 4;
            int64_t pr = min(p_base + c, a.P - 1);
            if (a.order) pr = a.order[pr];
            const int x0c = fused_parent_id(a, pr);
            {
                const unsigned qoff = (unsigned)(pr / a.parents_per_pair) * (unsigned)(D * 4) + (unsigned)g * 16u;
                const char* qbase = reinterpret_cast<const char*>(a.q);
                float4 qb[4];
#pragma unroll
                for (int nt = 0; nt < 4; ++nt) qb[nt] = *reinterpret_cast<const float4*>(qbase + 64 * nt + (size_t)qoff);
                unsigned woff = ((unsigned)(4 * g) * (unsigned)D + (unsigned)c) * 4u;
                unsigned boff = (unsigned)g * 16u;
                asm volatile("" : "+v"(woff), "+v"(boff));
#pragma unroll
                for (int mat = 0; mat < 2; ++mat) {
                    const char* W = reinterpret_cast<const char*>(mat == 0 ? a.W1 : a.W2);
                    const char* bias = reinterpret_cast<const char*>(mat == 0 ? a.b1 : a.b2);
                    f32x4 acc[4];
#pragma unroll
                    for (int ntp = 0; ntp < 4; ++ntp) {
                        const float4 b = bias ? *reinterpret_cast<const float4*>(bias + 64 * ntp + (size_t)boff) : make_float4(0.f, 0.f, 0.f, 0.f);
                        acc[ntp] = f32x4{b.x, b.y, b.z, b.w};
                    }
#pragma unroll
                    for (int nt = 0; nt < 4; ++nt) {
                        const float bv[4] = {qb[nt].x, qb[nt].y, qb[nt].z, qb[nt].w};
#pragma unroll
                        for (int r = 0; r < 4; ++r) {
#pragma unroll
                            for (int ntp = 0; ntp < 4; ++ntp) {
                                const float w = *reinterpret_cast<const float*>(W + ((16 * nt + r) * D + 16 * ntp) * 4 + (size_t)woff);
                                acc[ntp] = __builtin_amdgcn_mfma_f32_16x16x4f32(w, bv[r], acc[ntp], 0, 0, 0);
                            }
                        }
                    }
#pragma unroll
                    for (int ntp = 0; ntp < 4; ++ntp)
                        *reinterpret_cast<float4*>(sUV + c * kAggUvLd + mat * D + 16 * ntp + 4 * g) = make_float4(acc[ntp][0], acc[ntp][1], acc[ntp][2], acc[ntp][3]);
                }
            }
            __builtin_amdgcn_fence(__ATOMIC_RELEASE, "wavefront");
            __builtin_amdgcn_wave_barrier();
            __builtin_amdgcn_fence(__ATOMIC_ACQUIRE, "wavefront");

            const int nquad = (int)((min((int64_t)16, a.P - p_base) + 3) >> 2);
            struct Quad {
                unsigned p;
                unsigned ce[SPL], cr[SPL];
                float4 s0;
            };
            auto quad_load = [&](int it) -> Quad {
                Quad qd;
                const int src = ((lane & 48) + 4 * it + g) << 2;
                qd.p = (unsigned)__builtin_amdgcn_ds_bpermute(src, (int)pr);
                const unsigned x0 = (unsigned)__builtin_amdgcn_ds_bpermute(src, x0c);
                agg_load_slots<SPL>(adjE, adjR, (x0 * (unsigned)K + (unsigned)(SPL * c)) * 4u, qd.ce, qd.cr);
                qd.s0 = agg_row4(aggS, x0 * (unsigned)(D * 4) + c16);
                return qd;
            };
            Quad nx = quad_load(0);
            for (int it = 0; it < nquad; ++it) {
                const int j = 4 * it + g;
                const bool pvalid = p_base + j < a.P;
                const Quad qd = nx;
                if (it + 1 < nquad) nx = quad_load(it + 1);
                const unsigned p = qd.p;
                const unsigned (&ce)[SPL] = qd.ce;
                const unsigned (&cr)[SPL] = qd.cr;
                const float4 s0 = qd.s0;
                const float4 u1 = *reinterpret_cast<const float4*>(sUV + j * kAggUvLd + 4 * c);
                const float4 vv = *reinterpret_cast<const float4*>(sUV + j * kAggUvLd + D + 4 * c);
                float wk[SPL];
                agg_row_weights<SPL, FAST>(cr, att1, sT, (unsigned)(a.nR - 1), invK, wk);
                int cc = (int)(cr[0] >> 24);
                cc = pvalid ? (cc < 1 ? 1 : (cc > K ? K : cc)) : 0;
                __builtin_amdgcn_fence(__ATOMIC_RELEASE, "wavefront");
                __builtin_amdgcn_wave_barrier();
#pragma unroll
                for (int i = 0; i < SPL; ++i) {
                    sLo[SPL * c + i] = ((cr[i] >> 16) & 0xFFu) ? (ce[i] & 0xFFFFFFu) * (unsigned)(D * 4) : kAggPadRow;
                    sLw[SPL * c + i] = wk[i];
                }
                __builtin_amdgcn_fence(__ATOMIC_RELEASE, "wavefront");
                __builtin_amdgcn_wave_barrier();
                __builtin_amdgcn_fence(__ATOMIC_ACQUIRE, "wavefront");
                const int kmax = __builtin_amdgcn_readfirstlane(agg_xor32_imax(agg_xor16_imax(cc)));
                const f32x2 v01 = {vv.x, vv.y}, v23 = {vv.z, vv.w};
                f32x2 a01 = {0.f, 0.f}, a23 = {0.f, 0.f};
                float4 ra[4], rb[4];
                float4 wa, wb;
                auto issue = [&](int k, float4 (&r)[4], float4& w) {
                    const uint4 o4 = *reinterpret_cast<const uint4*>(sLo + k);
                    w = *reinterpret_cast<const float4*>(sLw + k);
                    r[0] = agg_row4(aggG, o4.x + c16), r[1] = agg_row4(aggG, o4.y + c16);
                    r[2] = agg_row4(aggG, o4.z + c16), r[3] = agg_row4(aggG, o4.w + c16);
                };
                auto sum4 = [&](const float4 (&r)[4], const float4& w) {
                    const float ws_[4] = {w.x, w.y, w.z, w.w};
#pragma unroll
                    for (int t = 0; t < 4; ++t) {
                        const f32x2 o01 = f32x2{r[t].x, r[t].y} + v01, o23 = f32x2{r[t].z, r[t].w} + v23;
                        const f32x2 w2 = {ws_[t], ws_[t]};
                        a01 = __builtin_elementwise_fma(w2, f32x2{fmaxf(o01[0], 0.f), fmaxf(o01[1], 0.f)}, a01);
                        a23 = __builtin_elementwise_fma(w2, f32x2{fmaxf(o23[0], 0.f), fmaxf(o23[1], 0.f)}, a23);
                    }
                };
                issue(0, ra, wa);
                for (int k0 = 0; k0 < kmax; k0 += 8) {
                    issue(k0 + 4, rb, wb);
                    __builtin_amdgcn_sched_barrier(0);
                    sum4(ra, wa);
                    __builtin_amdgcn_sched_barrier(0);
                    issue(k0 + 8, ra, wa);
                    __builtin_amdgcn_sched_barrier(0);
                    sum4(rb, wb);
                    __builtin_amdgcn_sched_barrier(0);
                }
                const unsigned oo = pvalid ? p * (unsigned)(D * 4) + c16 : kAggOob;
                float4 r0 = make_float4(fmaf(c0, u1.x, s0.x), fmaf(c0, u1.y, s0.y), fmaf(c0, u1.z, s0.z), fmaf(c0, u1.w, s0.w));
                float4 r1 = make_float4(a01[0], a01[1], a23[0], a23[1]);
                if (fold) {
                    r0 = make_float4(fmaxf(r0.x, 0.f), fmaxf(r0.y, 0.f), fmaxf(r0.z, 0.f), fmaxf(r0.w, 0.f));
                    r1 = make_float4(r1.x + r0.x, r1.y + r0.y, r1.z + r0.z, r1.w + r0.w);
                }
                const u32x4 o0 = {__float_as_uint(r0.x), __float_as_uint(r0.y), __float_as_uint(r0.z), __float_as_uint(r0.w)};
                const u32x4 o1 = {__float_as_uint(r1.x), __float_as_uint(r1.y), __float_as_uint(r1.z), __float_as_uint(r1.w)};
                __builtin_amdgcn_raw_buffer_store_b128(o0, out0, oo, 0, 0);
                __builtin_amdgcn_raw_buffer_store_b128(o1, out1, oo, 0, 0);
            }
            __builtin_amdgcn_fence(__ATOMIC_RELEASE, "wavefront");
            __builtin_amdgcn_wave_barrier();
            __builtin_amdgcn_fence(__ATOMIC_ACQUIRE, "wavefront");
        }
    };
    if (fast) run(std::true_type{});
    else run(std::false_type{});
}

constexpr int kFoldTraceBatches = 16, kFoldTraceSlots = 20;
__device__ long long g_fold_trace[kFoldTraceBatches * kFoldTraceSlots];

template <int K, int MODE, bool TRACE = false>
__global__ __launch_bounds__(kAggWaves * 64, 3) void score_l2_folded_kernel(FoldArgs a) {
    constexpr int D = 64, SPL = K / 16;
    constexpr bool PIPE = MODE > 0, db = MODE == 2;
    constexpr int lb = db ? agg_list_words(K) : 0;
    static_assert(K == 16 || K == 32 || K == 64, "K");
    extern __shared__ __attribute__((aligned(16))) float smem[];
    const int nRp = (a.nR + 3) & ~3;
    float* sT = smem;
    const int tid = threadIdx.x, lane = tid & 63, wave = __builtin_amdgcn_readfirstlane(tid >> 6);
    const int g = lane >> 4, c = lane & 15;
    float* sUV = sT + nRp + wave * (16 * kAggUvLd + agg_list_words(K) + lb);
    unsigned* sLo = reinterpret_cast<unsigned*>(sUV + 16 * kAggUvLd) + g * (K + kAggPad);
    float* sLw = reinterpret_cast<float*>(reinterpret_cast<unsigned*>(sUV + 16 * kAggUvLd) + 4 * (K + kAggPad)) + g * (K + kAggPad);
    const bool att1 = a.t1 != nullptr;
    const float invK = 1.f / (float)K;
    const unsigned rmax = (unsigned)(a.nR - 1);
    const bool fast = agg_logit_table(a.t1, a.nR, sT, tid, lane);
    __syncthreads();

    const int tbytes = (int)a.table_bytes;
    const __amdgpu_buffer_rsrc_t aggS = __builtin_amdgcn_make_buffer_rsrc(const_cast<float*>(a.agg), 0, tbytes, 0x00020000);
    const __amdgpu_buffer_rsrc_t aggG = __builtin_amdgcn_make_buffer_rsrc(reinterpret_cast<char*>(const_cast<float*>(a.agg)) + a.table_bytes, 0, tbytes, 0x00020000);
    const __amdgpu_buffer_rsrc_t adjE = __builtin_amdgcn_make_buffer_rsrc(const_cast<int32_t*>(a.adj_e), 0, (int)a.adj_bytes, 0x00020000);
    const __amdgpu_buffer_rsrc_t adjR = __builtin_amdgcn_make_buffer_rsrc(const_cast<int32_t*>(a.adj_r), 0, (int)a.adj_bytes, 0x00020000);
    const unsigned c16 = (unsigned)c * 16u;
    if (c < kAggPad) {
        sLo[K + c] = kAggPadRow, sLo[lb + K + c] = kAggPadRow;
        sLw[K + c] = 0.f, sLw[lb + K + c] = 0.f;
    }

    const int64_t nbatch = (a.B + 15) >> 4;
    const int64_t nwaves = (int64_t)gridDim.x * kAggWaves;
    int traced = 0;
    auto stamp = [&](int slot, bool drain) {
        if constexpr (TRACE) {
            if (drain) asm volatile("s_waitcnt vmcnt(0)" ::: "memory");
            if (blockIdx.x == 0 && tid == 0 && traced < kFoldTraceBatches) g_fold_trace[traced * kFoldTraceSlots + slot] = __builtin_readcyclecounter();
        }
    };
    auto run = [&](auto fast_tag) {
        constexpr bool FAST = decltype(fast_tag)::value;
        const int lane = (int)__builtin_amdgcn_mbcnt_hi(~0u, __builtin_amdgcn_mbcnt_lo(~0u, 0u)), g = lane >> 4, c = lane & 15;
        unsigned* sLo = reinterpret_cast<unsigned*>(sUV + 16 * kAggUvLd) + g * (K + kAggPad);
        float* sLw = reinterpret_cast<float*>(reinterpret_cast<unsigned*>(sUV + 16 * kAggUvLd) + 4 * (K + kAggPad)) + g * (K + kAggPad);
        const unsigned c16 = (unsigned)c * 16u;
        unsigned xn = 0;
        f32x4 qn[4];
        auto fetch_batch = [&](int64_t b) {
            const int64_t prn = min((min(b, nbatch - 1) << 4) + c, a.B - 1);
            xn = (unsigned)a.items[prn * a.pid_stride];
            const char* qrow = reinterpret_cast<const char*>(a.q) + (size_t)((unsigned)prn * (unsigned)(D * 4) + (unsigned)g * 16u);
#pragma unroll
            for (int nt = 0; nt < 4; ++nt) qn[nt] = *reinterpret_cast<const f32x4*>(qrow + 64 * nt);
        };
        if constexpr (PIPE) fetch_batch((int64_t)blockIdx.x * kAggWaves + wave);
        for (int64_t batch = (int64_t)blockIdx.x * kAggWaves + wave; batch < nbatch; batch += nwaves) {
            const int64_t p_base = batch << 4;
            stamp(0, false);
            const int64_t pr = min(p_base + c, a.B - 1);
            const bool cvalid = p_base + c < a.B;
            unsigned x0u;
            if constexpr (PIPE) x0u = xn;
            else x0u = (unsigned)a.items[pr * a.pid_stride];
            x0u = x0u < a.max_id ? x0u : a.max_id;
            const int x0c = (int)x0u;
            unsigned woff = ((unsigned)(4 * g) * (unsigned)D + (unsigned)c * 4u) * 4u;
            unsigned boff = (unsigned)g * 16u;
            unsigned roff = (unsigned)pr * (unsigned)(D * 4) + (unsigned)g * 16u;
            asm volatile("" : "+v"(woff), "+v"(boff));
            auto chain = [&](auto np_, auto&& wsel, auto&& bsel, auto&& asel, auto&& between, auto&& late) {
                constexpr int NP = decltype(np_)::value, T = 4 * NP;
                __amdgpu_buffer_rsrc_t wr[NP];
                static_for<NP>([&](auto j_) {
                    const float* Wp = wsel(j_);
                    asm volatile("" : "+s"(Wp));
                    wr[decltype(j_)::value] = __builtin_amdgcn_make_buffer_rsrc(const_cast<float*>(Wp), 0, D * D * 4, 0x00020000);
                });
                f32x4 ring[3][4];
                auto load = [&](auto s_) {
                    constexpr int s = decltype(s_)::value, j = s / 4, nt = s % 4;
#pragma unroll
                    for (int r = 0; r < 4; ++r) {
                        const u32x4 v = __builtin_amdgcn_raw_buffer_load_b128(wr[j], woff + (unsigned)(r * D * 4), nt * 16 * D * 4, 0);
                        ring[s % 3][r] = f32x4{__uint_as_float(v[0]), __uint_as_float(v[1]), __uint_as_float(v[2]), __uint_as_float(v[3])};
                    }
                };
                load(std::integral_constant<int, 0>{});
                load(std::integral_constant<int, 1>{});
                static_for<T>([&](auto s_) {
                    constexpr int s = decltype(s_)::value, j = s / 4, nt = s % 4;
                    if constexpr (s + 2 < T) load(std::integral_constant<int, s + 2>{});
                    if constexpr (s >= T - 3) late(std::integral_constant<int, s - (T - 3)>{});
                    __builtin_amdgcn_sched_barrier(0);
                    const f32x4 (&b)[4] = bsel(std::integral_constant<int, j>{});
                    f32x4 (&acc)[4] = asel(std::integral_constant<int, j>{});
#pragma unroll
                    for (int r = 0; r < 4; ++r) {
#pragma unroll
                        for (int ntp = 0; ntp < 4; ++ntp) acc[ntp] = __builtin_amdgcn_mfma_f32_16x16x4f32(ring[s % 3][r][ntp], b[nt][r], acc[ntp], 0, 0, 0);
                    }
                    __builtin_amdgcn_sched_barrier(0);
                    if constexpr (nt == 3) between(std::integral_constant<int, j>{});
                });
            };
            auto bias4 = [&](const float* bp, f32x4 (&acc)[4]) {
                const char* bias = reinterpret_cast<const char*>(bp);
#pragma unroll
                for (int ntp = 0; ntp < 4; ++ntp)
                    acc[ntp] = bias ? *reinterpret_cast<const f32x4*>(bias + 64 * ntp + (size_t)boff) : f32x4{0.f, 0.f, 0.f, 0.f};
            };
            struct Quad {
                unsigned ce[SPL], cr[SPL];
                float4 s0;
            };
            auto quad_load = [&](int it) -> Quad {
                Quad qd;
                const unsigned x0 = (unsigned)__builtin_amdgcn_ds_bpermute(((lane & 48) + 4 * it + g) << 2, x0c);
                agg_load_slots<SPL>(adjE, adjR, (x0 * (unsigned)K + (unsigned)(SPL * c)) * 4u, qd.ce, qd.cr);
                qd.s0 = agg_row4(aggS, x0 * (unsigned)(D * 4) + c16);
                return qd;
            };
            Quad q0, q1;
            auto late1 = [&](auto s_) {
                if constexpr (PIPE && decltype(s_)::value == 0) q0 = quad_load(0), q1 = quad_load(1);
            };
            f32x4 qm[4], qb[4];
            {
                const char* qbase = reinterpret_cast<const char*>(a.q);
#pragma unroll
                for (int nt = 0; nt < 4; ++nt) {
                    if constexpr (PIPE) qb[nt] = qn[nt];
                    else qb[nt] = *reinterpret_cast<const f32x4*>(qbase + 64 * nt + (size_t)roff);
                }
                stamp(1, true);
                f32x4 at[4], av[4];
                bias4(a.bq, at);
                bias4(a.bv, av);
                auto store_tv = [&](auto j_) {
                    constexpr int j = decltype(j_)::value;
                    if constexpr (j < 2) {
                        const f32x4 (&acc)[4] = j == 0 ? at : av;
#pragma unroll
                        for (int ntp = 0; ntp < 4; ++ntp) *reinterpret_cast<f32x4*>(sUV + c * kAggUvLd + j * D + 16 * ntp + 4 * g) = acc[ntp];
                    }
                };
                bias4(a.bm, qm);
                if (a.dbg & 4) late1(std::integral_constant<int, 0>{});
                else
                    chain(std::integral_constant<int, 3>{}, [&](auto j_) { return decltype(j_)::value == 0 ? a.Wq : decltype(j_)::value == 1 ? a.Wv : a.Wqm; },
                          [&](auto) -> const f32x4 (&)[4] { return qb; },
                          [&](auto j_) -> f32x4 (&)[4] {
                              if constexpr (decltype(j_)::value == 0) return at;
                              else if constexpr (decltype(j_)::value == 1) return av;
                              else return qm;
                          }, store_tv, late1);
            }
            __builtin_amdgcn_fence(__ATOMIC_RELEASE, "wavefront");
            __builtin_amdgcn_wave_barrier();
            __builtin_amdgcn_fence(__ATOMIC_ACQUIRE, "wavefront");
            stamp(2, false);

            const int nquad = (a.dbg & 8) ? 0 : (int)((min((int64_t)16, a.B - p_base) + 3) >> 2);
            auto issue = [&](const unsigned* lo, int k, float4 (&r)[4]) {
                const uint4 o4 = *reinterpret_cast<const uint4*>(lo + k);
                r[0] = agg_row4(aggG, o4.x + c16), r[1] = agg_row4(aggG, o4.y + c16);
                r[2] = agg_row4(aggG, o4.z + c16), r[3] = agg_row4(aggG, o4.w + c16);
            };
            auto sum4 = [&](const float4 (&r)[4], const float4& w, const f32x2 v01, const f32x2 v23, f32x2& a01, f32x2& a23) {
                const float ws_[4] = {w.x, w.y, w.z, w.w};
#pragma unroll
                for (int t = 0; t < 4; ++t) {
                    const f32x2 o01 = f32x2{r[t].x, r[t].y} + v01, o23 = f32x2{r[t].z, r[t].w} + v23;
                    const f32x2 w2 = {ws_[t], ws_[t]};
                    a01 = __builtin_elementwise_fma(w2, f32x2{fmaxf(o01[0], 0.f), fmaxf(o01[1], 0.f)}, a01);
                    a23 = __builtin_elementwise_fma(w2, f32x2{fmaxf(o23[0], 0.f), fmaxf(o23[1], 0.f)}, a23);
                }
            };
            auto lists = [&](const Quad& qd, int it, int ob) -> int {
                const bool pvalid = p_base + 4 * it + g < a.B;
                float wk[SPL];
                agg_row_weights<SPL, FAST>(qd.cr, att1, sT, rmax, invK, wk);
                int cc = (int)(qd.cr[0] >> 24);
                cc = pvalid ? (cc < 1 ? 1 : (cc > K ? K : cc)) : 0;
                __builtin_amdgcn_fence(__ATOMIC_RELEASE, "wavefront");
                __builtin_amdgcn_wave_barrier();
#pragma unroll
                for (int i = 0; i < SPL; ++i) {
                    sLo[ob + SPL * c + i] = ((qd.cr[i] >> 16) & 0xFFu) ? (qd.ce[i] & 0xFFFFFFu) * (unsigned)(D * 4) : kAggPadRow;
                    sLw[ob + SPL * c + i] = wk[i];
                }
                __builtin_amdgcn_fence(__ATOMIC_RELEASE, "wavefront");
                __builtin_amdgcn_wave_barrier();
                __builtin_amdgcn_fence(__ATOMIC_ACQUIRE, "wavefront");
                return (a.dbg & 1) ? 0 : __builtin_amdgcn_readfirstlane(agg_xor32_imax(agg_xor16_imax(cc)));
            };
            if constexpr (PIPE) {
                int kmax = lists(q0, 0, 0);
                for (int it = 0; it < nquad; ++it) {
                    stamp(3 + 3 * it, false);
                    const int cur = (it & 1) ? lb : 0;
                    float* rowT = sUV + (4 * it + g) * kAggUvLd + 4 * c;
                    const float4 vv = *reinterpret_cast<const float4*>(rowT + D);
                    const f32x2 v01 = {vv.x, vv.y}, v23 = {vv.z, vv.w};
                    f32x2 a01 = {0.f, 0.f}, a23 = {0.f, 0.f};
                    const int kr = (kmax + 7) & ~7;
                    float4 r0[4], r1[4], r2[4];
                    auto wts = [&](int k) { return *reinterpret_cast<const float4*>(sLw + cur + k); };
                    const float4 s0 = q0.s0;
                    if (it > 0 && it + 1 < nquad) q1 = quad_load(it + 1);
                    issue(sLo + cur, 0, r0);
                    issue(sLo + cur, 4, r1);
                    if (kr > 8) issue(sLo + cur, 8, r2);
                    stamp(4 + 3 * it, true);
                    __builtin_amdgcn_sched_barrier(0);
                    int kmax_n = 0;
                    if (db && it + 1 < nquad) kmax_n = lists(q1, it + 1, lb - cur);
                    __builtin_amdgcn_sched_barrier(0);
                    for (int k0 = 0; k0 < kr; k0 += 24) {
                        sum4(r0, wts(k0), v01, v23, a01, a23);
                        __builtin_amdgcn_sched_barrier(0);
                        if (k0 + 12 < kr) issue(sLo + cur, k0 + 12, r0);
                        __builtin_amdgcn_sched_barrier(0);
                        sum4(r1, wts(k0 + 4), v01, v23, a01, a23);
                        __builtin_amdgcn_sched_barrier(0);
                        if (k0 + 8 < kr) {
                            if (k0 + 16 < kr) issue(sLo + cur, k0 + 16, r1);
                            __builtin_amdgcn_sched_barrier(0);
                            sum4(r2, wts(k0 + 8), v01, v23, a01, a23);
                            __builtin_amdgcn_sched_barrier(0);
                            if (k0 + 16 < kr) issue(sLo + cur, k0 + 20, r2);
                            __builtin_amdgcn_sched_barrier(0);
                            sum4(r0, wts(k0 + 12), v01, v23, a01, a23);
                            __builtin_amdgcn_sched_barrier(0);
                            if (k0 + 16 < kr) {
                                if (k0 + 24 < kr) issue(sLo + cur, k0 + 24, r0);
                                __builtin_amdgcn_sched_barrier(0);
                                sum4(r1, wts(k0 + 16), v01, v23, a01, a23);
                                __builtin_amdgcn_sched_barrier(0);
                                if (k0 + 24 < kr) issue(sLo + cur, k0 + 28, r1);
                                __builtin_amdgcn_sched_barrier(0);
                                sum4(r2, wts(k0 + 20), v01, v23, a01, a23);
                                __builtin_amdgcn_sched_barrier(0);
                                if (k0 + 32 < kr) issue(sLo + cur, k0 + 32, r2);
                                __builtin_amdgcn_sched_barrier(0);
                            }
                        }
                    }
                    const float4 tt = *reinterpret_cast<const float4*>(rowT);
                    const float4 o0 = make_float4(fmaxf(s0.x + tt.x, 0.f), fmaxf(s0.y + tt.y, 0.f), fmaxf(s0.z + tt.z, 0.f), fmaxf(s0.w + tt.w, 0.f));
                    *reinterpret_cast<float4*>(rowT) = o0;
                    *reinterpret_cast<float4*>(rowT + D) = make_float4(a01[0] + o0.x, a01[1] + o0.y, a23[0] + o0.z, a23[1] + o0.w);
                    if (!db && it + 1 < nquad) kmax_n = lists(q1, it + 1, 0);
                    kmax = kmax_n;
                    q0 = q1;
                    stamp(5 + 3 * it, false);
                }
            } else {
                Quad nx = quad_load(0);
                for (int it = 0; it < nquad; ++it) {
                    stamp(3 + 3 * it, false);
                    const Quad qd = nx;
                    if (it + 1 < nquad) nx = quad_load(it + 1);
                    float* rowT = sUV + (4 * it + g) * kAggUvLd + 4 * c;
                    const float4 tt = *reinterpret_cast<const float4*>(rowT);
                    const float4 vv = *reinterpret_cast<const float4*>(rowT + D);
                    const int kmax = lists(qd, it, 0);
                    const f32x2 v01 = {vv.x, vv.y}, v23 = {vv.z, vv.w};
                    f32x2 a01 = {0.f, 0.f}, a23 = {0.f, 0.f};
                    float4 ra[4], rb[4];
                    float4 wa, wb;
                    auto wts = [&](int k) { return *reinterpret_cast<const float4*>(sLw + k); };
                    issue(sLo, 0, ra), wa = wts(0);
                    if constexpr (TRACE) {
                        issue(sLo, 4, rb), wb = wts(4);
                        stamp(4 + 3 * it, true);
                    }
                    for (int k0 = 0; k0 < kmax; k0 += 8) {
                        if (!TRACE || k0 > 0) issue(sLo, k0 + 4, rb), wb = wts(k0 + 4);
                        __builtin_amdgcn_sched_barrier(0);
                        sum4(ra, wa, v01, v23, a01, a23);
                        __builtin_amdgcn_sched_barrier(0);
                        issue(sLo, k0 + 8, ra), wa = wts(k0 + 8);
                        __builtin_amdgcn_sched_barrier(0);
                        sum4(rb, wb, v01, v23, a01, a23);
                        __builtin_amdgcn_sched_barrier(0);
                    }
                    const float4 o0 = make_float4(fmaxf(qd.s0.x + tt.x, 0.f), fmaxf(qd.s0.y + tt.y, 0.f), fmaxf(qd.s0.z + tt.z, 0.f),
                                                  fmaxf(qd.s0.w + tt.w, 0.f));
                    *reinterpret_cast<float4*>(rowT) = o0;
                    *reinterpret_cast<float4*>(rowT + D) = make_float4(a01[0] + o0.x, a01[1] + o0.y, a23[0] + o0.z, a23[1] + o0.w);
                    stamp(5 + 3 * it, false);
                }
            }
            __builtin_amdgcn_fence(__ATOMIC_RELEASE, "wavefront");
            __builtin_amdgcn_wave_barrier();
            __builtin_amdgcn_fence(__ATOMIC_ACQUIRE, "wavefront");
            {
                f32x4 zb[4], ob[4], o2[4], m0r[4], uor[4];
                auto m0_load = [&]() {
#pragma unroll
                    for (int ntp = 0; ntp < 4; ++ntp)
                        m0r[ntp] = *reinterpret_cast<const f32x4*>(reinterpret_cast<const char*>(a.M0) + (size_t)x0u * (D * 4) + 64 * ntp + (size_t)boff);
                };
                auto uo_load = [&]() {
#pragma unroll
                    for (int ntp = 0; ntp < 4; ++ntp)
                        uor[ntp] = *reinterpret_cast<const f32x4*>(reinterpret_cast<const char*>(a.user_o) + 64 * ntp + (size_t)roff);
                };
                auto late2 = [&](auto s_) {
                    if constexpr (PIPE && decltype(s_)::value == 0) m0_load();
                    if constexpr (PIPE && decltype(s_)::value == 1) fetch_batch(batch + nwaves);
                    if constexpr (PIPE && decltype(s_)::value == 2) uo_load();
                };
#pragma unroll
                for (int nt = 0; nt < 4; ++nt) zb[nt] = *reinterpret_cast<const f32x4*>(sUV + c * kAggUvLd + D + 16 * nt + 4 * g);
                bias4(a.a1, o2);
                auto relu_o2 = [&]() {
#pragma unroll
                    for (int nt = 0; nt < 4; ++nt) o2[nt] = f32x4{fmaxf(o2[nt][0], 0.f), fmaxf(o2[nt][1], 0.f), fmaxf(o2[nt][2], 0.f), fmaxf(o2[nt][3], 0.f)};
                };
                auto read_ob = [&]() {
#pragma unroll
                    for (int nt = 0; nt < 4; ++nt) ob[nt] = *reinterpret_cast<const f32x4*>(sUV + c * kAggUvLd + 16 * nt + 4 * g);
                };
                if (a.dbg & 2) late2(std::integral_constant<int, 0>{}), late2(std::integral_constant<int, 1>{}), late2(std::integral_constant<int, 2>{});
                else
                    chain(std::integral_constant<int, 3>{}, [&](auto j_) { constexpr int j = decltype(j_)::value; return j == 0 ? a.A1 : j == 1 ? a.Wm1 : a.Wm2; },
                          [&](auto j_) -> const f32x4 (&)[4] {
                              constexpr int j = decltype(j_)::value;
                              if constexpr (j == 0) return zb;
                              else if constexpr (j == 1) return ob;
                              else return o2;
                          },
                          [&](auto j_) -> f32x4 (&)[4] { if constexpr (decltype(j_)::value == 0) return o2; else return qm; },
                          [&](auto j_) {
                              if constexpr (decltype(j_)::value == 0) relu_o2(), read_ob();
                          }, late2);
                stamp(15, false);
                if constexpr (!PIPE) m0_load();
                stamp(16, true);
                if constexpr (!PIPE) {
                    if (a.user_o != a.q) uo_load();
                    else
#pragma unroll
                        for (int ntp = 0; ntp < 4; ++ntp) uor[ntp] = qb[ntp];
                }
                float part = 0.f;
#pragma unroll
                for (int ntp = 0; ntp < 4; ++ntp) {
                    const f32x4 uo = uor[ntp];
                    const f32x4 it4 = qm[ntp] + m0r[ntp];
                    if (a.item_emb && cvalid) *reinterpret_cast<f32x4*>(reinterpret_cast<char*>(a.item_emb) + 64 * ntp + (size_t)roff) = it4;
                    part += it4[0] * uo[0] + it4[1] * uo[1] + it4[2] * uo[2] + it4[3] * uo[3];
                }
                part = xor32_sum(xor16_sum(part));
                if (g == 0 && cvalid) {
                    a.scores[pr] = part;
                    if (a.sig) a.sig[pr] = 1.f / (1.f + expf(-part));
                }
                stamp(17, false);
            }
            __builtin_amdgcn_fence(__ATOMIC_RELEASE, "wavefront");
            __builtin_amdgcn_wave_barrier();
            __builtin_amdgcn_fence(__ATOMIC_ACQUIRE, "wavefront");
            if constexpr (TRACE) ++traced;
        }
    };
    if (fast) run(std::true_type{});
    else run(std::false_type{});
}

hipError_t fold_read_trace(long long* host_dst, size_t n) {
    const size_t have = sizeof(g_fold_trace) / sizeof(long long);
    return hipMemcpyFromSymbol(host_dst, HIP_SYMBOL(g_fold_trace), (n < have ? n : have) * sizeof(long long));
}

template <int K>
static hipError_t launch_fold_k(const FoldArgs& a, hipStream_t st) {
    static const bool pipe = !(getenv("MVIN_FOLD_PIPE") && atoi(getenv("MVIN_FOLD_PIPE")) == 0);
    static const bool trace = getenv("MVIN_FOLD_TRACE") != nullptr;
    static const int grid_cap = getenv("MVIN_FOLD_GRID") ? atoi(getenv("MVIN_FOLD_GRID")) : 0;
    static const int wgs = getenv("MVIN_FOLD_WGS") ? atoi(getenv("MVIN_FOLD_WGS")) : 0;
    using Kern = void (*)(FoldArgs);
    constexpr size_t kLdsNoOptIn = 48 * 1024;
    constexpr bool kTwoLists = fused_agg_lds_words(0, K) * sizeof(float) + (size_t)kAggWaves * agg_list_words(K) * sizeof(float) <= kLdsNoOptIn;
    auto kernel_of = [&](int mode) -> Kern {
        if (trace) {
            if constexpr (kTwoLists) {
                if (mode == 2) return score_l2_folded_kernel<K, 2, true>;
            }
            return mode ? (Kern)score_l2_folded_kernel<K, 1, true> : (Kern)score_l2_folded_kernel<K, 0, true>;
        }
        if constexpr (kTwoLists) {
            if (mode == 2) return score_l2_folded_kernel<K, 2, false>;
        }
        return mode ? (Kern)score_l2_folded_kernel<K, 1, false> : (Kern)score_l2_folded_kernel<K, 0, false>;
    };
    struct Plan {
        int dev, nR, per_cu;
        size_t lds;
        Kern kern;
    };
    static thread_local Plan plan{-1, -1, 0, 0, nullptr};
    int dev = 0;
    if (hipGetDevice(&dev) != hipSuccess) return hipGetLastError();
    if (plan.dev != dev || plan.nR != a.nR) {
        auto occupancy = [&](Kern k, size_t lds) {
            int v = 0;
            if (hipOccupancyMaxActiveBlocksPerMultiprocessor(&v, reinterpret_cast<const void*>(k), kAggWaves * 64, lds) != hipSuccess || v < 1) v = 0;
            return v > 8 ? 8 : v;
        };
        const size_t lds1 = fused_agg_lds_bytes(a.nR, K), lds2 = lds1 + (size_t)kAggWaves * agg_list_words(K) * sizeof(float);
        const int mode1 = pipe ? 1 : 0;
        const int occ1 = occupancy(kernel_of(mode1), lds1);
        const int occ2 = pipe && kTwoLists && lds2 <= kLdsNoOptIn ? occupancy(kernel_of(2), lds2) : 0;
        const bool two = occ2 > 0 && occ2 >= occ1;
        plan.kern = kernel_of(two ? 2 : mode1);
        plan.lds = two ? lds2 : lds1;
        plan.per_cu = two ? occ2 : occ1 > 0 ? occ1 : 4;
        if (wgs > 0) plan.per_cu = wgs;
        plan.dev = dev, plan.nR = a.nR;
        if (getenv("MVIN_FOLD_REPORT"))
            fprintf(stderr, "score_l2_folded_kernel<%d>: mode %d, LDS %zu bytes per workgroup, %d workgroups per CU\n", K, two ? 2 : mode1, plan.lds, plan.per_cu);
    }
    const int64_t nbatch = (a.B + 15) >> 4;
    const int64_t want = (nbatch + kAggWaves - 1) / kAggWaves;
    int64_t cap = 256 * (int64_t)plan.per_cu;
    if (grid_cap > 0 && grid_cap < cap) cap = grid_cap;
    plan.kern<<<(int)(want < cap ? want : cap), kAggWaves * 64, plan.lds, st>>>(a);
    return hipGetLastError();
}

hipError_t launch_score_l2_folded(const float* agg, const float* M0, const int32_t* adj_e, const int32_t* adj_r, const int32_t* items, int pid_stride,
                                  const float* t1, const float* q, const float* user_o, const float* Wq, const float* bq, const float* Wv,
                                  const float* bv, const float* Wqm, const float* A1, const float* a1, const float* Wm1, const float* Wm2,
                                  const float* bm, float* item_emb, float* scores, float* sig, int64_t B, int K, int D, int nR, int n_entity,
                                  hipStream_t st) {
    FoldArgs f{};
    f.agg = agg, f.M0 = M0, f.adj_e = adj_e, f.adj_r = adj_r, f.items = items, f.pid_stride = pid_stride, f.t1 = t1, f.q = q, f.user_o = user_o;
    f.Wq = Wq, f.bq = bq, f.Wv = Wv, f.bv = bv, f.Wqm = Wqm, f.A1 = A1, f.a1 = a1, f.Wm1 = Wm1, f.Wm2 = Wm2, f.bm = bm;
    f.item_emb = item_emb, f.scores = scores, f.sig = sig, f.B = B, f.K = K, f.nR = nR, f.max_id = (unsigned)(n_entity - 1);
    f.table_bytes = (uint64_t)n_entity * (uint64_t)D * 4, f.adj_bytes = (uint64_t)n_entity * (uint64_t)K * 4;
    static const char* dbg = getenv("MVIN_FOLD_DBG");
    f.dbg = dbg ? atoi(dbg) : 0;
    if (D == 32) return launch_score_l2_folded_d32(f, st);
    switch (K) {
        case 16: return launch_fold_k<16>(f, st);
        case 32: return launch_fold_k<32>(f, st);
        case 64: return launch_fold_k<64>(f, st);
        default: return hipErrorInvalidValue;
    }
}

bool fused_agg_supported(int D, int K) { return D == 64 && (K == 16 || K == 32 || K == 64); }
bool fused_fold_supported(int D, int K) { return fused_agg_supported(D, K) || (D == 32 && (K == 16 || K == 32)); }
size_t fused_fold_d32_lds_bytes(int nR, int K);
size_t fused_fold_lds_bytes(int D, int nR, int K) { return D == 32 ? fused_fold_d32_lds_bytes(nR, K) : fused_agg_lds_bytes(nR, K); }

size_t fused_agg_lds_bytes(int nR, int K) { return fused_agg_lds_words(nR, K) * sizeof(float); }

bool fused_agg_applies(const FusedL2Args& a, int D) {
    return a.prj && fused_agg_supported(D, a.K) && !a.probs_parent && !a.probs_child && a.adj_r && a.adj_bytes > 0 &&
           a.adj_bytes < (1ull << 31) && a.table_bytes > 0 && a.table_bytes < (1ull << 30) && (uint64_t)a.P * D * 4 < (1ull << 31) &&
           a.max_id < (1u << 24) && a.nR > 0 && fused_agg_lds_bytes(a.nR, a.K) <= 48 * 1024;
}

template <int K>
static hipError_t launch_entity_aggregates_k(const EntityAggArgs& a, hipStream_t st) {
    const size_t lds = ((size_t)((a.nR + 3) & ~3) + (size_t)kAggWaves * agg_list_words(K)) * sizeof(float);
    const int64_t nquad = ((int64_t)a.n_entity + 3) >> 2;
    const int64_t want = (nquad + kAggWaves - 1) / kAggWaves;
    const int64_t cap = 256 * 8;
    entity_aggregates_kernel<K><<<(int)(want < cap ? want : cap), kAggWaves * 64, lds, st>>>(a);
    return hipGetLastError();
}

hipError_t launch_entity_aggregates(const EntityAggArgs& a, hipStream_t st) {
    if (a.D == 32) return launch_entity_aggregates_d32(a, st);
    switch (a.K) {
        case 16: return launch_entity_aggregates_k<16>(a, st);
        case 32: return launch_entity_aggregates_k<32>(a, st);
        case 64: return launch_entity_aggregates_k<64>(a, st);
        default: return hipErrorInvalidValue;
    }
}

__global__ void fold_prepare_kernel(const float* __restrict__ W0, const float* __restrict__ b0, const float* __restrict__ W1,
                                    const float* __restrict__ b1, const float* __restrict__ W2, const float* __restrict__ b2,
                                    const float* __restrict__ A0, const float* __restrict__ a0, const float* __restrict__ Wmix,
                                    const float* __restrict__ bmix, const float* __restrict__ A1, float c, int D, float* __restrict__ blk) {
    const int i = blockIdx.x, j = threadIdx.x;
    float* Wstack = blk;
    float* Wv = blk + (size_t)4 * D * D;
    float* Wq = Wv + (size_t)D * D;
    float* bv = Wq + (size_t)D * D;
    float* bq = bv + D;
    float* bm = bq + D;
    if (j >= D) return;
    float s0 = 0.f, s1 = 0.f, s2 = 0.f, sm = 0.f;
    for (int k0 = 0; k0 < D; k0 += 8) {
        float av[8], mv[8], x0[8], x1[8], x2[8];
#pragma unroll
        for (int k = 0; k < 8; ++k) {
            av[k] = A0[(size_t)(k0 + k) * D + j];
            mv[k] = Wmix[(size_t)(k0 + k) * D + j];
            x0[k] = i < D ? W0[(size_t)i * D + k0 + k] : (b0 ? b0[k0 + k] : 0.f);
            x1[k] = i < D ? W1[(size_t)i * D + k0 + k] : (b1 ? b1[k0 + k] : 0.f);
            x2[k] = i < D ? W2[(size_t)i * D + k0 + k] : (b2 ? b2[k0 + k] : 0.f);
        }
#pragma unroll
        for (int k = 0; k < 8; ++k) {
            s0 = fmaf(x0[k], av[k], s0);
            s1 = fmaf(x1[k], av[k], s1);
            s2 = fmaf(x2[k], av[k], s2);
            sm = fmaf(x0[k], mv[k], sm);
        }
    }
    if (i < D) {
        Wstack[(size_t)i * D + j] = s1;
        Wstack[(size_t)D * D + (size_t)i * D + j] = s2;
        Wstack[(size_t)2 * D * D + (size_t)i * D + j] = s0;
        Wstack[(size_t)3 * D * D + (size_t)i * D + j] = sm;
        Wv[(size_t)i * D + j] = fmaf(c, s2, s1);
        Wq[(size_t)i * D + j] = fmaf(c, s1, s0);
        if (D == 64 || D == 32) {
            float* Wperm = bm + D;
            const size_t o = (size_t)i * D + (size_t)(j & 15) * (D / 16) + (size_t)(j >> 4);
            const size_t DD = (size_t)D * D;
            Wperm[o] = fmaf(c, s1, s0);
            Wperm[DD + o] = fmaf(c, s2, s1);
            Wperm[2 * DD + o] = sm;
            Wperm[3 * DD + o] = A1[(size_t)i * D + j];
            Wperm[4 * DD + o] = Wmix[DD + (size_t)i * D + j];
            Wperm[5 * DD + o] = Wmix[2 * DD + (size_t)i * D + j];
        }
    } else {
        const float av0 = a0 ? a0[j] : 0.f;
        bv[j] = fmaf(c, s2, s1) + av0;
        bq[j] = fmaf(c, s1, s0) + av0;
        bm[j] = (bmix ? bmix[j] : 0.f) + sm;
    }
}

hipError_t launch_fold_prepare(const float* W0, const float* b0, const float* W1, const float* b1, const float* W2, const float* b2, const float* A0,
                               const float* a0, const float* Wmix, const float* bmix, const float* A1, float c, int D, float* blk, hipStream_t st) {
    fold_prepare_kernel<<<D + 1, D < 64 ? 64 : D, 0, st>>>(W0, b0, W1, b1, W2, b2, A0, a0, Wmix, bmix, A1, c, D, blk);
    return hipGetLastError();
}

template <int K>
static hipError_t launch_agg_k(const FusedL2Args& a, hipStream_t st) {
    const size_t lds = fused_agg_lds_bytes(a.nR, K);
    static thread_local int per_cu = 0;
    if (per_cu == 0) {
        int v = 0;
        if (hipOccupancyMaxActiveBlocksPerMultiprocessor(&v, reinterpret_cast<const void*>(gather_attn_l2_agg_kernel<K>), kAggWaves * 64, lds) != hipSuccess || v < 1)
            v = 4;
        per_cu = v > 8 ? 8 : v;
    }
    const int64_t nbatch = (a.P + 15) >> 4;
    const int64_t want = (nbatch + kAggWaves - 1) / kAggWaves;
    const int64_t cap = 256 * (int64_t)per_cu;
    gather_attn_l2_agg_kernel<K><<<(int)(want < cap ? want : cap), kAggWaves * 64, lds, st>>>(a);
    return hipGetLastError();
}

hipError_t launch_gather_attn_l2_agg(const FusedL2Args& a, hipStream_t st) {
    switch (a.K) {
        case 16: return launch_agg_k<16>(a, st);
        case 32: return launch_agg_k<32>(a, st);
        case 64: return launch_agg_k<64>(a, st);
        default: return hipErrorInvalidValue;
    }
}

}
```

### mvin_amd/csrc/mvin_kernels.h

```cpp
#pragma once
#include <hip/hip_runtime.h>
#include <stdint.h>

#include "../../include/mvin_hip.h"
#include "mvin_common.h"

namespace mvin {

struct GatherAttnArgs {
    int gather;
    int table_bf16;
    const void* table;
    const int32_t* adj_e;
    const int32_t* adj_r;
    const int32_t* node_ids;
    const float* neigh;
    const int32_t* rel_ids;
    const float* rel_score;
    const float* self_vec;
    const float* Wc;
    const float* c_child;
    const float* Wagg;
    const float* bagg;
    float* out;
// ... 185 lines not shown
struct FusedL2Args {
    const void* table;
    const int32_t* adj_e;
    const int32_t* adj_r;
    const int32_t* parent_ids;
    const float* t0;
    const float* t1;
    const float* W1;
    const float* W2;
    const float* q;
    const float* b1;
    const float* b2;
    const float* A0;
    const float* a0;
    float* nagg0;
    float* nagg1;
    float* probs_parent;
    float* probs_child;
    int64_t P;
    uint64_t table_bytes;
    uint64_t adj_bytes;
    int parents_per_pair, K, nR, lpn_log2;
    int pid_stride;
    unsigned max_id;
    int dbg;
    const int32_t* order;
    float* agg;
    int fold;
    int prj;
};

__device__ __forceinline__ int fused_parent_id(const FusedL2Args& a, int64_t i) {
    const unsigned v = (unsigned)a.parent_ids[i * a.pid_stride];
    return (int)(v < a.max_id ? v : a.max_id);
}

struct EltArgs {
    int mode;
    int64_t n;
    float* x;
    float* y;
    float* z;
    float* w;
    float* accum;
    float alpha, beta, beta1, beta2, eps;
    int D, N;
};

struct WgradArgs {
    mvin_linear_args lin;
    const float* dY;
    int64_t ldy, dy_zstride;
    const float* mask;
    int64_t ldm, mask_zstride;
    float* dW;
    int64_t dw_zstride;
    float* db;
    int64_t db_zstride;
    int IB;
};

struct AggBwdArgs {
    int gather;
    const float* table;
    const int32_t* adj_e;
    const int32_t* adj_r;
    const int32_t* node_ids;
    const float* child;
    const int32_t* rel_ids;
    const float* probs;
    const float* rel_score;
    int skip_zero;
    const float* dvec;
    float* dtable;
    float* dchild;
    float* dT;
    int64_t T;
    int K, D, nR, lpr_log2;
};

struct KeyAddrBwdArgs {
    KeyAddrArgs f;
    const float* dout;
    float* dE;
    float* dV;
    float* dw;
    float l2;
    const float* Rk;
    const void* items;
    int items64;
    int dw_rep;
    int dv_lds;
    float* reg_accum;
};

hipError_t launch_eltwise(const EltArgs& a, hipStream_t st);
hipError_t launch_l2_adam_multi(const mvin_param_seg* segs, int nseg, int64_t total, float* g, float* mo, float* vo,
                                float* accum, int apply_adam, float lr_t, const float* lr_dev, float b1, float b2,
                                float eps, hipStream_t st);
hipError_t launch_l2_adam_multi_guarded(const mvin_param_seg* segs, int nseg, int64_t total, float* g, float* mo, float* vo,
                                        float* accum, int apply_adam, const mvin_guard_state* guard, float b1, float b2,
                                        float eps, hipStream_t st);
hipError_t launch_grad_guard(const mvin_param_seg* segs, int nseg, int64_t total, const float* g,
                             const mvin_guard_item* items, int nitems, mvin_guard_partial* partials,
                             const float* lr_table, int lr_table_len, mvin_guard_state* state, int grid_cap,
                             hipStream_t st);
hipError_t launch_scatter_add_rows(float* dtable, const int32_t* ids, int ids64, const float* x, int64_t rows, int D,
                                   float alpha, hipStream_t st);
hipError_t launch_linear_wgrad(WgradArgs a, hipStream_t st);
hipError_t launch_linear_wgrad_multi(const WgradArgs* probs, int n, hipStream_t st);
hipError_t launch_agg_bwd(const AggBwdArgs& a, hipStream_t st);
hipError_t launch_rel_score_bwd(const float* rel, const float* urh_w, const float* dT, int nR, int D, float* drel,
                                float* durh, hipStream_t st);
hipError_t launch_key_addr_bwd(const KeyAddrBwdArgs& a, hipStream_t st);

inline int lpr_log2_for(int D) {
    int l = 0;
    while ((4 << l) < D) ++l;
    return l;
}

hipError_t launch_expand(const int32_t* adj_e, const int32_t* adj_r, const int64_t* items64,
                         const int32_t* items32, int B, int K, int levels, int n_entity,
                         int32_t* ent_out, int32_t* rel_out, hipStream_t st);
hipError_t launch_rel_score(const float* rel, const float* urh_w, int nR, int D, float* t,
                            hipStream_t st);
hipError_t launch_linear(const mvin_linear_args& a, hipStream_t st);
bool linear_mfma_supported(const mvin_linear_args& a);
hipError_t launch_linear_mfma(const mvin_linear_args& a, hipStream_t st);
hipError_t launch_gather_attn(const GatherAttnArgs& a, hipStream_t st);
hipError_t launch_ripple(const RippleArgs& a, hipStream_t st);
hipError_t launch_sample_adjacency(const int64_t* indptr, const int32_t* dst, const int32_t* rel, int n_entity,
                                   int K, uint64_t seed, int32_t* adj_e, int32_t* adj_r, hipStream_t st);
hipError_t launch_ripple_build(const RippleBuildArgs& a, hipStream_t st);
int key_addr_nj(int Nm, int D);
bool key_addr_grouped_supported(int D, int P, int Nm, int nR);
hipError_t launch_key_addr_grouped(const KeyAddrGroupedArgs& a, int table_bf16, hipStream_t st);
bool key_addr_wave16_supported(int D, int P, int Nm, int nR);
bool key_addr_wave16_applies(const KeyAddrGroupedArgs& a);
hipError_t launch_key_addr_wave16(const KeyAddrGroupedArgs& a, int table_bf16, hipStream_t st);
bool key_addr_dense_supported(int D, int P, int Nm, int nR);
hipError_t launch_key_addr_dense(const KeyAddrGroupedArgs& a, int table_bf16, hipStream_t st);
KaRecLayout ka_rec_layout(int P, int Nm, int nR);
hipError_t launch_user_records(const int32_t* uts, int n_user, int P, int Nm, int nR, int n_entity, int32_t* out, hipStream_t st);
bool key_addr_static_supported(int D, int P, int Nm, int nR);
bool key_addr_static_applies(const KeyAddrGroupedArgs& a, int table_bf16);
hipError_t launch_key_addr_static(const KeyAddrGroupedArgs& a, hipStream_t st);
bool key_addr_flash_supported(int D, int P, int Nm, int nR, int n_entity);
size_t key_addr_flash_ws_elems(int64_t B, int nseg_bound);
hipError_t launch_key_addr_flash(const KaFlashArgs& a, int nseg_bound, bool has_set, int32_t* sched_ws, hipStream_t st);
hipError_t kas_read_trace(long long* host_dst, size_t n);
hipError_t kaf_read_trace(long long* host_dst, size_t n);
hipError_t fold_read_trace(long long* host_dst, size_t n);
hipError_t launch_key_addr(const KeyAddrArgs& a, int table_bf16, hipStream_t st);
bool key_addr_stream_supported(const KeyAddrArgs& a, int table_bf16);
hipError_t launch_key_addr_stream(const KeyAddrArgs& a, int table_bf16, hipStream_t st);
hipError_t launch_move_rows(void* table, const int32_t* ids, int64_t n, int row_bytes, void* rows, bool scatter,
                            hipStream_t st);
hipError_t launch_shard_space_ids(const void* ids, bool is64, int64_t n, int world, int n_local, void* out, hipStream_t st);
hipError_t launch_row_softmax(const float* x, int64_t rows, int n, float* out, hipStream_t st);
hipError_t launch_mix_urv(const float* neigh, const float* rel, const float* user, const float* logits, int64_t nodes, int N, int K,
                          int D, float* out, float* probs, hipStream_t st);
hipError_t launch_gather_mix(const GatherMixArgs& a, hipStream_t st);
struct ScoreSmallArgs {
    const void* E;
    const int32_t* adj_e;
    const int32_t* adj_r;
    const float* R;
    const float* w_h;
    const float* Wu;
    const float* bu;
    const float* t0;
    const float* t1;
    const float *W0, *b0, *W1, *b1, *W2, *b2;
    const float *A0, *a0, *A1, *a1, *Wmix, *bmix;
    const int64_t* items;
    const int32_t* mem_h[4];
    const int32_t* mem_r[4];
    const int32_t* mem_t[4];
    const int32_t* uts;
    const int64_t* users;
    float* user_o;
    float* item_emb;
    float* scores;
    float* sig;
    int64_t B;
    int G;
    int K, P, Nm, nR, n_entity, n_user, enc, table_bf16;
    int depth1;
    int dbg;
    uint64_t table_bytes;
    uint64_t adj_bytes;
};
bool score_small_supported(int D, int K, int P, int Nm, int nR);
int score_small_group(int D, int K, int P, int Nm, int nR, int has_hset, int64_t B);
hipError_t launch_score_small(ScoreSmallArgs a, int D, hipStream_t st);
hipError_t small_read_trace(long long* host_dst, size_t n);

bool l2_tail_supported(int D);
hipError_t launch_l2_tail(const TailArgs& a, int D, hipStream_t st);
bool l2_tail_flash_applies(const TailArgs& a, int D);
hipError_t launch_l2_tail_flash(const TailArgs& a, hipStream_t st);
bool fused_l2_supported(int D, int K);
hipError_t launch_gather_attn_l2(const FusedL2Args& a, int D, int table_bf16, hipStream_t st);
bool fused_split_supported(int D, int K);
bool fused_split_applies(const FusedL2Args& a, int D);
hipError_t launch_gather_probe_l2(const void* table, const int32_t* ids1, const int32_t* ids2, int64_t n_parents, int K,
                                  int D, int table_bf16, float* sums, hipStream_t st);
hipError_t launch_group_pairs(const int64_t* u64, const int32_t* u32, int64_t B, int n_user, int32_t* count, int32_t* offs,
                              int32_t* rank, int32_t* seg_user, int32_t* seg_ptr, int32_t* nseg, int32_t* pair_index, hipStream_t st);
hipError_t launch_count_ids(const int32_t* ids, int64_t n, int nbins, float* out, hipStream_t st);
bool fused_d32_supported(int D, int K);
bool fused_d32_applies(const FusedL2Args& a, int D);
bool topk_rows_supported(int k);
hipError_t launch_topk_rows(const float* scores, int64_t rows, int64_t n, int64_t ld, const int32_t* cand_ids, int64_t col_offset,
                            const int64_t* excl_ptr, const int32_t* excl_ids, const int32_t* carry_ids, const float* carry_vals, int k,
                            int32_t* out_ids, float* out_vals, hipStream_t st);
hipError_t launch_rank_positives(const float* scores, int64_t rows, int64_t n, int64_t ld, const int32_t* cand_ids, int64_t col_offset,
                                 const int64_t* excl_ptr, const int32_t* excl_ids, const int64_t* pos_ptr, const int32_t* pos_ids,
                                 int32_t* out_counts, float* out_vals, int32_t* out_eligible, hipStream_t st);
int64_t ctr_counts_ws_bytes(int64_t n_seg, int64_t seg_len);
hipError_t launch_ctr_counts(const float* scores, const int32_t* labels, int64_t n_seg, int64_t seg_len, int64_t ld, void* ws,
                             int64_t* out, hipStream_t st);
bool sample_negatives_supported(int n_item);
hipError_t launch_sample_negatives(const int64_t* excl_ptr, const int32_t* excl_ids, const int32_t* counts, const int64_t* out_ptr,
                                   int n_user, int n_item, const uint32_t* alias_tab, const uint32_t* mask_bits, uint64_t seed,
                                   uint64_t round, int32_t* out, int64_t* status,
                                   hipStream_t st);
hipError_t launch_rank_head(const float* user_o, const float* item_emb, const float* valid, const float* offset, int64_t n_groups,
                            int G, int D, int mode, float scale, float* scores, float* dscore, float* du, float* di,
                            float* loss_accum, int64_t* counts,
                            hipStream_t st);
hipError_t launch_select_negatives(const float* scores, const int64_t* items, const float* valid, const int64_t* group_key,
                                   int64_t n_groups, int Gp, int n_neg, int shortlist, uint64_t seed, uint64_t round,
                                   int64_t* out_items, float* out_valid, float* out_scores, int64_t* counts,
                                   hipStream_t st);
int64_t kg_explore_ws_bytes(int n_entity, int64_t M);
hipError_t launch_kg_field(const int64_t* eptr, const int32_t* edst, const int32_t* erel, int n_entity, int64_t M,
                           const int32_t* seeds, int64_t n_seed, int hops, void* ws, uint32_t* field_bits, int64_t* out_counts,
                           hipStream_t st);
hipError_t launch_kg_explore(const int64_t* eptr, const int32_t* edst, const int32_t* erel, int n_entity, int64_t M,
                             const int32_t* adj_entity, const int32_t* adj_relation, int K, const int32_t* seeds, int64_t n_seed,
                             int hops, void* ws, uint32_t* explored_bits, int64_t* out_counts, hipStream_t st);
size_t order_ws_elems(int64_t B);
hipError_t launch_order_by_key(const int64_t* k64, const int32_t* k32, int64_t B, int32_t* ws, int32_t* order, hipStream_t st);
bool fused_wpp_supported(int D, int K);
bool fused_wpp_applies(const FusedL2Args& a, int D);
hipError_t launch_gather_attn_l2_wpp(const FusedL2Args& a, hipStream_t st);
bool fused_agg_supported(int D, int K);
bool fused_fold_supported(int D, int K);
size_t fused_fold_lds_bytes(int D, int nR, int K);
bool fused_agg_applies(const FusedL2Args& a, int D);
hipError_t launch_entity_aggregates(const EntityAggArgs& a, hipStream_t st);
hipError_t launch_fold_prepare(const float* W0, const float* b0, const float* W1, const float* b1, const float* W2, const float* b2, const float* A0,
                               const float* a0, const float* Wmix, const float* bmix, const float* A1, float c, int D, float* blk, hipStream_t st);
hipError_t launch_l2_tail_fold(const TailFoldArgs& a, hipStream_t st);
hipError_t launch_score_l2_folded(const float* agg, const float* M0, const int32_t* adj_e, const int32_t* adj_r, const int32_t* items, int pid_stride,
                                  const float* t1, const float* q, const float* user_o, const float* Wq, const float* bq, const float* Wv,
                                  const float* bv, const float* Wqm, const float* A1, const float* a1, const float* Wm1, const float* Wm2,
                                  const float* bm, float* item_emb, float* scores, float* sig, int64_t B, int K, int D, int nR, int n_entity,
                                  hipStream_t st);
hipError_t launch_gather_attn_l2_agg(const FusedL2Args& a, hipStream_t st);
hipError_t launch_gather_attn_l2_d32(const FusedL2Args& a, int table_bf16, hipStream_t st, bool encoded = false);
bool fused_d16_supported(int D, int K);
bool fused_d16_applies(const FusedL2Args& a, int D);
hipError_t launch_gather_attn_l2_d16(const FusedL2Args& a, int table_bf16, hipStream_t st);
bool fused_l2_split_in_use();
hipError_t launch_gather_attn_l2_split(const FusedL2Args& a, int D, int table_bf16, hipStream_t st);
hipError_t split_read_trace(long long* host_dst, size_t n);
bool fused_packed_supported(int D, int K);
bool key_addr_static_er_ok(int P, int Nm, int nR, int n_entity, bool has_set);
hipError_t launch_transpose_blocks(const float* R, int nR, int D, float* RT, hipStream_t st);
constexpr int kEtMaxJobs = 24;
struct EntityTableJob {
    const float* W;
    float* out;
    int w_nk;
};
hipError_t launch_entity_tables(const float* E, int n_entity, const EntityTableJob* jobs, int njobs, hipStream_t st);
hipError_t launch_entity_dot(const float* E, const float* w, int n, int D, float* out, hipStream_t st);
hipError_t launch_prj_prepare(const float* W1, const float* W2, const float* b1, const float* b2, const float* A0, const float* a0,
                              float c, int D, float* blk, hipStream_t st);
bool fused_packed_applies(const FusedL2Args& a, int D);
hipError_t pack_read_prof(long long* host_dst, size_t n);
hipError_t launch_gather_attn_l2_packed(const FusedL2Args& a, int D, int table_bf16, hipStream_t st);
hipError_t launch_encode_adjacency(const int32_t* adj_e, const int32_t* adj_r, int n_entity, int K, int32_t* cnt,
                                   int32_t* enc_e, int32_t* enc_r, hipStream_t st);
hipError_t ka_read_trace(long long* host_dst, size_t n);

}
```

### mvin_amd/ops.py

```python
import ctypes as C
import os

import numpy as np
import torch

from . import _lib

F32 = torch.float32
I32 = torch.int32
BF16 = torch.bfloat16


def _chk_table(t, name):
    if t is None:
        return 0
    _chk(t, BF16 if t.dtype == BF16 else F32, name)
    return 1 if t.dtype == BF16 else 0


def _stream():
    return C.c_void_p(torch.cuda.current_stream().cuda_stream)


def _chk(t, dtype, name):
# ... 626 lines not shown
        uniq, inv, cnt_u = np.unique(key, return_inverse=True, return_counts=True)
        end_u = np.cumsum(cnt_u)
        row_end = np.cumsum(n_found)
        pos_above = row_end[f_row] - end_u[inv]
        pos_equal = cnt_u[inv] - 1
        neg_above = f_c[:, 0] - pos_above
        neg_equal = f_c[:, 1] + f_c[:, 2] - pos_equal
        u2 = np.zeros(rows, dtype=np.int64)
        np.add.at(u2, f_row, 2 * (n_neg[f_row] - neg_above) - neg_equal)
        undefined = (n_found == 0) | (n_neg <= 0)
        with np.errstate(divide="ignore", invalid="ignore"):
            auc = np.where(undefined, np.nan, u2.astype(np.float64) / (2.0 * n_found.astype(np.float64) * n_neg.astype(np.float64)))
        out["auc"] = auc
        if undefined.any():
            warnings.warn(f"No found positive or no negative in {int(undefined.sum())} of {rows} row(s): the row's AUC is not "
                          "defined there (NaN)", UndefinedMetricWarning, stacklevel=2)
    return out


def gather_attn_l2_prj(ws, enc_entity, enc_relation, parent_ids, t0, t1, q, B, parents_per_pair, K, D, nR, n_entity, encoded=True, order=None):
    lib = _lib.load()
    for t, dt, nm in ((ws, F32, "ws"), (enc_entity, I32, "enc_entity"), (enc_relation, I32, "enc_relation"),
                      (parent_ids, torch.int64 if parent_ids.dtype == torch.int64 else I32, "parent_ids"), (t0, F32, "t0"),
                      (t1, F32, "t1"), (q, F32, "q")):
        _chk(t, dt, nm)
    if ws.numel() != lib.mvin_project_tables_elems(n_entity, D) or q is None or tuple(q.shape) != (B, D):
        raise ValueError("gather_attn_l2_prj: the workspace of project_tables(n_entity, D) and q [B, D] expected")
    P = B * parents_per_pair
    nagg0 = torch.empty((P, D), dtype=F32, device=ws.device)
    nagg1 = torch.empty((P, D), dtype=F32, device=ws.device)
    _chk(order, I32, "order")
    if order is not None and order.numel() != P:
        raise ValueError("gather_attn_l2_prj: order must be a permutation of the launch's parents")
    _lib.check(lib.mvin_gather_attn_l2_prj_ordered_fwd(_p(ws), _p(enc_entity), _p(enc_relation), 1 if encoded else 0, _p(parent_ids),
                                                       int(parent_ids.dtype == torch.int64), _p(order), _p(t0), _p(t1), _p(q), B,
                                                       parents_per_pair, K, D, n_entity, nR, _p(nagg0), _p(nagg1), _stream()),
               "mvin_gather_attn_l2_prj_fwd")
    return nagg0, nagg1


def gather_attn_l2_agg_supported(D, K, n_entity, nR):
    return bool(_lib.load().mvin_gather_attn_l2_agg_supported(D, K, n_entity, nR))


def entity_aggregates(ws, enc_entity, enc_relation, t0, K, D, nR, n_entity, out=None):
    lib = _lib.load()
    for t, dt, nm in ((ws, F32, "ws"), (enc_entity, I32, "enc_entity"), (enc_relation, I32, "enc_relation"), (t0, F32, "t0")):
        _chk(t, dt, nm)
    if ws.numel() != lib.mvin_project_tables_elems(n_entity, D):
        raise ValueError("entity_aggregates: the workspace of project_tables(n_entity, D) expected")
    n = lib.mvin_entity_aggregates_elems(n_entity, D)
    if out is None:
        out = torch.empty((n,), dtype=F32, device=ws.device)
    elif out.numel() != n or out.dtype != F32 or not out.is_contiguous():
        raise ValueError("entity_aggregates: workspace of mvin_entity_aggregates_elems floats expected")
    _lib.check(lib.mvin_entity_aggregates(_p(ws), _p(enc_entity), _p(enc_relation), _p(t0), K, D, n_entity, nR, _p(out), _stream()),
               "mvin_entity_aggregates")
    return out


def gather_attn_l2_agg(ws, agg, enc_entity, enc_relation, parent_ids, t0, t1, q, B, parents_per_pair, K, D, nR, n_entity, order=None):
    lib = _lib.load()
    for t, dt, nm in ((ws, F32, "ws"), (agg, F32, "agg"), (enc_entity, I32, "enc_entity"), (enc_relation, I32, "enc_relation"),
                      (parent_ids, torch.int64 if parent_ids.dtype == torch.int64 else I32, "parent_ids"), (t0, F32, "t0"),
                      (t1, F32, "t1"), (q, F32, "q"), (order, I32, "order")):
        _chk(t, dt, nm)
    if (ws.numel() != lib.mvin_project_tables_elems(n_entity, D) or agg.numel() != lib.mvin_entity_aggregates_elems(n_entity, D)
            or q is None or tuple(q.shape) != (B, D)):
        raise ValueError("gather_attn_l2_agg: the workspaces of project_tables / entity_aggregates (n_entity, D) and q [B, D] expected")
    P = B * parents_per_pair
    if order is not None and order.numel() != P:
        raise ValueError("gather_attn_l2_agg: order must be a permutation of the launch's parents")
    nagg0 = torch.empty((P, D), dtype=F32, device=ws.device)
    nagg1 = torch.empty((P, D), dtype=F32, device=ws.device)
    _lib.check(lib.mvin_gather_attn_l2_agg_fwd(_p(ws), _p(agg), _p(enc_entity), _p(enc_relation), _p(parent_ids),
                                               int(parent_ids.dtype == torch.int64), _p(order), _p(t0), _p(t1), _p(q), B,
                                               parents_per_pair, K, D, n_entity, nR, _p(nagg0), _p(nagg1), _stream()),
               "mvin_gather_attn_l2_agg_fwd")
    return nagg0, nagg1


def score_l2_folded_supported(D, K, n_entity, nR):
    return bool(_lib.load().mvin_score_l2_folded_supported(D, K, n_entity, nR))


def fold_tables(entity_emb, enc_entity, enc_relation, t0, W0, b0, W1, b1, W2, b2, A0, a0, Wmix, bmix, A1, K, nR, out=None, aggregates=True):
    lib = _lib.load()
    for t, nm in ((entity_emb, "entity_emb"), (t0, "t0"), (W0, "W0"), (b0, "b0"), (W1, "W1"), (b1, "b1"), (W2, "W2"), (b2, "b2"),
                  (A0, "A0"), (a0, "a0"), (Wmix, "Wmix"), (bmix, "bmix"), (A1, "A1")):
        _chk(t, F32, nm)
    _chk(enc_entity, I32, "enc_entity")
    _chk(enc_relation, I32, "enc_relation")
    nE, D = entity_emb.shape
    n = lib.mvin_fold_tables_elems(nE, D)
    if out is None:
        out = torch.empty((n,), dtype=F32, device=entity_emb.device)
    elif out.numel() != n or out.dtype != F32 or not out.is_contiguous():
        raise ValueError("fold_tables: workspace of mvin_fold_tables_elems floats expected")
    _lib.check(lib.mvin_fold_tables_ex(_p(entity_emb), _p(enc_entity), _p(enc_relation), _p(t0), _p(W0), _p(b0), _p(W1), _p(b1), _p(W2), _p(b2),
                                       _p(A0), _p(a0), _p(Wmix), _p(bmix), _p(A1), 1 if aggregates else 0, K, D, nE, nR, _p(out), _stream()),
               "mvin_fold_tables")
    return out


def score_l2_folded_gather_supported(D, K, n_entity, nR):
    return bool(_lib.load().mvin_score_l2_folded_gather_supported(D, K, n_entity, nR))


def score_l2_folded_gather(ws, enc_entity, enc_relation, items, t0, t1, q, user_o, A1, a1, Wmix, K, D, nR, n_entity, order=None,
                           want_item_emb=True):
    lib = _lib.load()
    for t, dt, nm in ((ws, F32, "ws"), (enc_entity, I32, "enc_entity"), (enc_relation, I32, "enc_relation"),
                      (items, torch.int64 if items.dtype == torch.int64 else I32, "items"), (t0, F32, "t0"), (t1, F32, "t1"), (q, F32, "q"),
                      (user_o, F32, "user_o"), (A1, F32, "A1"), (a1, F32, "a1"), (Wmix, F32, "Wmix"), (order, I32, "order")):
        _chk(t, dt, nm)
    B = items.shape[0]
    if ws.numel() != lib.mvin_fold_tables_elems(n_entity, D) or tuple(q.shape) != (B, D) or tuple(user_o.shape) != (B, D):
        raise ValueError("score_l2_folded_gather: the workspace of fold_tables(n_entity, D) and q, user_o [B, D] expected")
    if order is not None and order.numel() != B:
        raise ValueError("score_l2_folded_gather: order must be a permutation of the pairs")
    item_emb = torch.empty((B, D), dtype=F32, device=ws.device) if want_item_emb else None
    scores = torch.empty((B,), dtype=F32, device=ws.device)
    sig = torch.empty((B,), dtype=F32, device=ws.device)
    i64 = items.dtype == torch.int64
    _lib.check(lib.mvin_score_l2_folded_gather_fwd(_p(ws), _p(enc_entity), _p(enc_relation), _p(items) if i64 else None,
                                                   None if i64 else _p(items), _p(order), _p(t0), _p(t1), _p(q), _p(user_o), _p(A1), _p(a1),
                                                   _p(Wmix), B, K, D, n_entity, nR, _p(item_emb), _p(scores), _p(sig), _stream()),
               "mvin_score_l2_folded_gather_fwd")
    return item_emb, scores, sig


def score_l2_folded(ws, enc_entity, enc_relation, items, t0, t1, q, user_o, A1, a1, Wmix, K, D, nR, n_entity, want_item_emb=True):
    lib = _lib.load()
    for t, dt, nm in ((ws, F32, "ws"), (enc_entity, I32, "enc_entity"), (enc_relation, I32, "enc_relation"),
                      (items, torch.int64 if items.dtype == torch.int64 else I32, "items"), (t0, F32, "t0"), (t1, F32, "t1"), (q, F32, "q"),
                      (user_o, F32, "user_o"), (A1, F32, "A1"), (a1, F32, "a1"), (Wmix, F32, "Wmix")):
        _chk(t, dt, nm)
    B = items.shape[0]
    if ws.numel() != lib.mvin_fold_tables_elems(n_entity, D) or tuple(q.shape) != (B, D) or tuple(user_o.shape) != (B, D):
        raise ValueError("score_l2_folded: the workspace of fold_tables(n_entity, D) and q, user_o [B, D] expected")
    two = os.environ.get("MVIN_L2_FOLD_TWO", "0") not in ("", "0")
    out0 = torch.empty((B, D), dtype=F32, device=ws.device) if two else None
    z2 = torch.empty((B, D), dtype=F32, device=ws.device) if two else None
    item_emb = torch.empty((B, D), dtype=F32, device=ws.device) if want_item_emb else None
    scores = torch.empty((B,), dtype=F32, device=ws.device)
    sig = torch.empty((B,), dtype=F32, device=ws.device)
    i64 = items.dtype == torch.int64
    _lib.check(lib.mvin_score_l2_folded_fwd(_p(ws), _p(enc_entity), _p(enc_relation), _p(items) if i64 else None, None if i64 else _p(items),
                                            _p(t0), _p(t1), _p(q), _p(user_o), _p(A1), _p(a1), _p(Wmix), B, K, D, n_entity, nR, _p(out0),
                                            _p(z2), _p(item_emb), _p(scores), _p(sig), _stream()), "mvin_score_l2_folded_fwd")
    return item_emb, scores, sig


def gather_mix(table, adj_entity, adj_relation, node_ids, rel_score_t, rowbias, nodes, nodes_per_group, K, nR,
               relu=False):
    lib = _lib.load()
    bf = _chk_table(table, "table")
    for t, dt, nm in ((adj_entity, I32, "adj_entity"), (adj_relation, I32, "adj_relation"),
                      (node_ids, I32, "node_ids"), (rel_score_t, F32, "rel_score"), (rowbias, F32, "rowbias")):
        _chk(t, dt, nm)
    D = table.shape[1]
    out = torch.empty((nodes, D), dtype=F32, device=table.device)
    _lib.check(lib.mvin_gather_mix_fwd(_p(table), _p(adj_entity), _p(adj_relation), _p(node_ids), _p(rel_score_t),
                                       _p(rowbias), nodes, nodes_per_group, K, D, table.shape[0], nR,
                                       1 if relu else 0, _p(out), bf, _stream()), "mvin_gather_mix_fwd")
    return out


def row_softmax(x):
    lib = _lib.load()
    _chk(x, F32, "x")
    out = torch.empty_like(x)
    _lib.check(lib.mvin_row_softmax_fwd(_p(x), x.shape[0], x.shape[1], _p(out), _stream()), "mvin_row_softmax_fwd")
    return out


def mix_neighbor_vectors(neighbor_vectors, neighbor_relations=None, user_embeddings=None, want_probs=False, logits=None):
    lib = _lib.load()
    _chk(neighbor_vectors, F32, "neighbor_vectors")
    B, N, K, D = neighbor_vectors.shape
    if logits is not None:
        _chk(logits, F32, "logits")
        if logits.numel() != B * N * K:
            raise ValueError("logits must be [B,N,K]")
    elif neighbor_relations is not None:
        _chk(neighbor_relations, F32, "neighbor_relations")
        _chk(user_embeddings, F32, "user_embeddings")
        if tuple(neighbor_relations.shape) != (B, N, K, D) or tuple(user_embeddings.shape) != (B, D):
            raise ValueError("neighbor_relations must be [B,N,K,D] and user_embeddings [B,D]")
    out = torch.empty((B, N, D), dtype=F32, device=neighbor_vectors.device)
    probs = torch.empty((B, N, K), dtype=F32, device=neighbor_vectors.device) if want_probs else None
    use_rel = logits is None and neighbor_relations is not None
    _lib.check(lib.mvin_mix_neighbor_vectors_fwd(_p(neighbor_vectors), _p(neighbor_relations) if use_rel else None,
                                                 _p(user_embeddings) if use_rel else None, _p(logits), B, N, K, D,
                                                 _p(out), _p(probs), _stream()), "mvin_mix_neighbor_vectors_fwd")
    return (out, probs) if want_probs else out


def key_addressing_supported(Nm, D):
    return bool(_lib.load().mvin_key_addressing_supported(Nm, D))


def key_addressing(entity_emb, V, w, mem_h, mem_r, mem_t, P, out, ldo, nR):
    lib = _lib.load()
    bf = _chk_table(entity_emb, "entity_emb")
    _chk(V, F32, "V"), _chk(w, F32, "w"), _chk(out, F32, "out")
    nh = max(1, P)
    arr_t = C.c_void_p * nh
    for lst, nm in ((mem_h[:nh], "mem_h"), (mem_r[:P], "mem_r"), (mem_t[:P], "mem_t")):
        for t in lst:
            _chk(t, I32, nm)
    ph = arr_t(*[t.data_ptr() for t in mem_h[:nh]])
    pr = arr_t(*([t.data_ptr() for t in mem_r[:P]] + [None] * (nh - P)))
    pt = arr_t(*([t.data_ptr() for t in mem_t[:P]] + [None] * (nh - P)))
    B, Nm = mem_h[0].shape
    D = entity_emb.shape[1]
    _lib.check(lib.mvin_key_addressing_fwd(_p(entity_emb), _p(V), _p(w), ph, pr, pt, P, B, Nm, D, nR,
                                           entity_emb.shape[0], _p(out), ldo, bf, _stream()),
               "mvin_key_addressing_fwd")
    return out


def key_addressing_users(entity_emb, V, w, uts, users, P, out, ldo, nR):
    lib = _lib.load()
    bf = _chk_table(entity_emb, "entity_emb")
    _chk(V, F32, "V"), _chk(w, F32, "w"), _chk(out, F32, "out"), _chk(uts, I32, "uts")
    if users.dtype not in (torch.int64, I32):
        raise TypeError("users: int64 or int32")
    _chk(users, users.dtype, "users")
    if uts.dim() != 4 or uts.shape[1] != max(1, P) or uts.shape[2] != 3:
        raise ValueError("uts must be [n_user, max(1,P), 3, Nm]")
    B, Nm, D = users.shape[0], uts.shape[3], entity_emb.shape[1]
    u64, u32 = (_p(users), None) if users.dtype == torch.int64 else (None, _p(users))
    _lib.check(lib.mvin_key_addressing_users_fwd(_p(entity_emb), _p(V), _p(w), _p(uts), u64, u32, P, B, Nm, D, nR,
                                                 entity_emb.shape[0], uts.shape[0], _p(out), ldo, bf, _stream()),
               "mvin_key_addressing_users_fwd")
    return out


def l2_tail_supported(D):
    return bool(_lib.load().mvin_l2_tail_supported(D))


def l2_tail(entity_emb, items, q, user_o, nagg0, nagg1, W0, b0, A0, a0, A1, a1, Wmix, bmix):
    bf = _chk_table(entity_emb, "entity_emb")
    for t, nm in ((q, "q"), (user_o, "user_o"), (nagg0, "nagg0"), (nagg1, "nagg1"), (W0, "W0"), (b0, "b0"), (A0, "A0"),
                  (a0, "a0"), (A1, "A1"), (a1, "a1"), (Wmix, "Wmix"), (bmix, "bmix")):
        _chk(t, F32, nm)
    B, D = user_o.shape
    dev = user_o.device
    i64 = items if items.dtype == torch.int64 else None
    i32 = items if items.dtype == I32 else None
    item_emb = torch.empty((B, D), dtype=F32, device=dev)
    scores = torch.empty((B,), dtype=F32, device=dev)
    sig = torch.empty((B,), dtype=F32, device=dev)
    _lib.check(_lib.load().mvin_l2_tail_fwd(_p(entity_emb), _p(i64), _p(i32), _p(q), _p(user_o), _p(nagg0), _p(nagg1),
                                            _p(W0), _p(b0), _p(A0), _p(a0), _p(A1), _p(a1), _p(Wmix), _p(bmix), B, D,
                                            entity_emb.shape[0], _p(item_emb), _p(scores), _p(sig), bf, _stream()),
               "mvin_l2_tail_fwd")
    return item_emb, scores, sig


def gather_rows(table, ids):
    _chk(ids, I32, "ids")
    if not table.is_cuda or not table.is_contiguous():
        raise _lib.MvinHipError("table: expected a contiguous CUDA/ROCm tensor")
    out = torch.empty((ids.shape[0], table.shape[1]), dtype=table.dtype, device=table.device)
    _lib.check(_lib.load().mvin_gather_rows(_p(table), _p(ids), ids.shape[0], table.shape[1] * table.element_size(),
                                            _p(out), _stream()), "mvin_gather_rows")
    return out


def scatter_rows(table, ids, rows):
    _chk(ids, I32, "ids")
    if rows.dtype != table.dtype or not rows.is_contiguous() or not table.is_contiguous():
        raise TypeError("rows/table: same dtype, contiguous")
    _lib.check(_lib.load().mvin_scatter_rows(_p(table), _p(ids), ids.shape[0], table.shape[1] * table.element_size(),
                                             _p(rows), _stream()), "mvin_scatter_rows")
    return table


def shard_space_ids(ids, world, n_local):
    if ids.dtype not in (torch.int64, I32) or not ids.is_cuda:
        raise TypeError("ids: int64 or int32 device tensor")
    ids = ids.contiguous()
    out = torch.empty_like(ids)
    _lib.check(_lib.load().mvin_shard_space_ids(_p(ids), int(ids.dtype == torch.int64), ids.numel(), world, n_local,
                                                _p(out), _stream()), "mvin_shard_space_ids")
    return out


def key_addressing_grouped_supported(D, P, Nm, nR):
    return bool(_lib.load().mvin_key_addressing_grouped_supported(D, P, Nm, nR))


def group_pairs_by_user(users, n_user=None):
    B = users.shape[0]
    if n_user is not None and users.is_cuda and users.dtype in (torch.int64, I32) and users.is_contiguous():
        dev = users.device
        ws = torch.empty(2 * n_user + B, dtype=I32, device=dev)
        seg_user = torch.empty(B, dtype=I32, device=dev)
        seg_ptr = torch.empty(B + 2, dtype=I32, device=dev)
        nseg = torch.empty(1, dtype=I32, device=dev)
        pair_index = torch.empty(B, dtype=I32, device=dev)
        u64, u32 = (_p(users), None) if users.dtype == torch.int64 else (None, _p(users))
        _lib.check(_lib.load().mvin_group_pairs_by_user(u64, u32, B, n_user, _p(ws), _p(seg_user), _p(seg_ptr), _p(nseg),
# ... 421 lines not shown
```

Measured before the change: 549.5 million.

## Add item-ordered pair processing and quad list reuse in folded L2 scorer

Adds an optional pair permutation to the folded hop-2 scoring kernel, obtained by sorting the batch by item id behind the MVIN_FOLD_ORDER env var, so that pairs sharing an item land in the same wave. The kernel uses a ballot to detect quads whose item matches the previous quad and then skips reloading and rebuilding their neighbor lists. Trace counters record loaded versus reused quads. The order path is off by default and adds a sort launch. Reuse detection is on by default but only skips list construction; the row gathers still run because 'held' is a constant false.

Measured after the change: 548.3 million. About the same (-0.2%).

```diff
diff --git a/include/mvin_hip.h b/include/mvin_hip.h
--- a/include/mvin_hip.h
+++ b/include/mvin_hip.h
@@ -128,6 +128,12 @@
                                       const int32_t* items_i32, const float* t0, const float* t1, const float* q, const float* user_o,
                                       const float* A1, const float* a1, const float* Wmix, int64_t B, int K, int D, int n_entity, int nR,
                                       float* out0, float* z2, float* item_emb, float* scores, float* sig, void* stream);
+MVIN_API int mvin_score_l2_folded_ordered_fwd(const float* ws, const int32_t* enc_entity, const int32_t* enc_relation, const int64_t* items_i64,
+                                              const int32_t* items_i32, const int32_t* order, const float* t0, const float* t1, const float* q,
+                                              const float* user_o, const float* A1, const float* a1, const float* Wmix, int64_t B, int K,
+                                              int D, int n_entity, int nR, float* out0, float* z2, float* item_emb, float* scores, float* sig,
+                                              void* stream);
+MVIN_API int mvin_debug_read_fold_steps(long long* host_dst);
 MVIN_API int mvin_gather_attn_l2_variant(int D, int K, int64_t n_parents, int n_entity, int want_probs);
 MVIN_API int mvin_gather_attn_l2_variant_ex(int D, int K, int64_t n_parents, int n_entity, int want_probs, int table_bf16);
 MVIN_API int mvin_probe_gather_l2(const void* table, const int32_t* child_ids, const int32_t* grandchild_ids, int64_t n_parents, int K,
diff --git a/mvin_amd/_lib.py b/mvin_amd/_lib.py
--- a/mvin_amd/_lib.py
+++ b/mvin_amd/_lib.py
@@ -106,6 +106,8 @@
     "mvin_score_l2_folded_gather_supported": (C.c_int, [C.c_int] * 4),
     "mvin_score_l2_folded_gather_fwd": (C.c_int, [C.c_void_p] * 13 + [C.c_int64] + [C.c_int] * 4 + [C.c_void_p] * 4),
     "mvin_score_l2_folded_fwd": (C.c_int, [C.c_void_p] * 12 + [C.c_int64] + [C.c_int] * 4 + [C.c_void_p] * 6),
+    "mvin_score_l2_folded_ordered_fwd": (C.c_int, [C.c_void_p] * 13 + [C.c_int64] + [C.c_int] * 4 + [C.c_void_p] * 6),
+    "mvin_debug_read_fold_steps": (C.c_int, [C.c_void_p]),
     "mvin_gather_rows": (C.c_int, [C.c_void_p, C.c_void_p, C.c_int64, C.c_int, C.c_void_p, C.c_void_p]),
     "mvin_scatter_rows": (C.c_int, [C.c_void_p, C.c_void_p, C.c_int64, C.c_int, C.c_void_p, C.c_void_p]),
     "mvin_linear_wgrad_multi": (C.c_int, [C.c_void_p, C.c_int, C.c_void_p]),
diff --git a/mvin_amd/csrc/mvin_abi.hip b/mvin_amd/csrc/mvin_abi.hip
--- a/mvin_amd/csrc/mvin_abi.hip
+++ b/mvin_amd/csrc/mvin_abi.hip
@@ -696,11 +696,45 @@
     return fold_tables_aggregates(who, enc_entity, enc_relation, t0, K, D, n_entity, nR, ws, stream);
 }
 
+constexpr int64_t kFoldOrderMinBatch = 32768;
+static bool fold_order_applies(int D, int K, int64_t B) {
+    static const bool on = getenv("MVIN_FOLD_ORDER") && atoi(getenv("MVIN_FOLD_ORDER")) != 0;
+    static const bool two = getenv("MVIN_L2_FOLD_TWO") && atoi(getenv("MVIN_L2_FOLD_TWO")) != 0;
+    return on && !two && mvin::fused_agg_supported(D, K) && B >= kFoldOrderMinBatch && (size_t)B * D >= mvin::order_ws_elems(B);
+}
+
+static int score_l2_folded_impl(const char* who, const float* ws, const int32_t* enc_entity, const int32_t* enc_relation,
+                                const int64_t* items_i64, const int32_t* items_i32, const int32_t* order, const float* t0, const float* t1,
+                                const float* q, const float* user_o, const float* A1, const float* a1, const float* Wmix, int64_t B, int K,
+                                int D, int n_entity, int nR, float* out0, float* z2, float* item_emb, float* scores, float* sig,
+                                void* stream);
+
 int mvin_score_l2_folded_fwd(const float* ws, const int32_t* enc_entity, const int32_t* enc_relation, const int64_t* items_i64,
                              const int32_t* items_i32, const float* t0, const float* t1, const float* q, const float* user_o, const float* A1,
                              const float* a1, const float* Wmix, int64_t B, int K, int D, int n_entity, int nR, float* out0, float* z2,
                              float* item_emb, float* scores, float* sig, void* stream) {
-    const char* who = "mvin_score_l2_folded_fwd";
+    return score_l2_folded_impl("mvin_score_l2_folded_fwd", ws, enc_entity, enc_relation, items_i64, items_i32, nullptr, t0, t1, q, user_o, A1,
+                                a1, Wmix, B, K, D, n_entity, nR, out0, z2, item_emb, scores, sig, stream);
+}
+
+int mvin_score_l2_folded_ordered_fwd(const float* ws, const int32_t* enc_entity, const int32_t* enc_relation, const int64_t* items_i64,
+                                     const int32_t* items_i32, const int32_t* order, const float* t0, const float* t1, const float* q,
+                                     const float* user_o, const float* A1, const float* a1, const float* Wmix, int64_t B, int K, int D,
+                                     int n_entity, int nR, float* out0, float* z2, float* item_emb, float* scores, float* sig, void* stream) {
+    return score_l2_folded_impl("mvin_score_l2_folded_ordered_fwd", ws, enc_entity, enc_relation, items_i64, items_i32, order, t0, t1, q,
+                                user_o, A1, a1, Wmix, B, K, D, n_entity, nR, out0, z2, item_emb, scores, sig, stream);
+}
+
+int mvin_debug_read_fold_steps(long long* host_dst) {
+    if (!host_dst) return -1;
+    return hip_result(mvin::fold_read_steps(host_dst), "mvin_debug_read_fold_steps");
+}
+
+static int score_l2_folded_impl(const char* who, const float* ws, const int32_t* enc_entity, const int32_t* enc_relation,
+                                const int64_t* items_i64, const int32_t* items_i32, const int32_t* order, const float* t0, const float* t1,
+                                const float* q, const float* user_o, const float* A1, const float* a1, const float* Wmix, int64_t B, int K,
+                                int D, int n_entity, int nR, float* out0, float* z2, float* item_emb, float* scores, float* sig,
+                                void* stream) {
     if (!ws || !enc_entity || !enc_relation || !q || !user_o || !A1 || !Wmix || !scores) return fail(-1, "%s: null pointer", who);
     if ((items_i64 == nullptr) == (items_i32 == nullptr)) return fail(-1, "%s: exactly one of items_i64 / items_i32", who);
     if (B <= 0 || B >= (int64_t(1) << 31)) return fail(-2, "%s: B=%lld", who, (long long)B);
@@ -713,6 +747,7 @@
     const float* bq = bv + D;
     const float* bm = bq + D;
     static const bool two = getenv("MVIN_L2_FOLD_TWO") && atoi(getenv("MVIN_L2_FOLD_TWO")) != 0;
+    if (order && (two || D != 64)) return fail(-3, "%s: a pair order is taken by the one-launch form at dim 64 only", who);
     if (!two || D != 64)
     {
         const float* Wp = bm + D;
@@ -720,7 +755,7 @@
         return hip_result(mvin::launch_score_l2_folded(ws + 4 * tab, ws + 3 * tab, enc_entity, enc_relation,
                                                        items_i64 ? reinterpret_cast<const int32_t*>(items_i64) : items_i32, items_i64 ? 2 : 1, t1, q,
                                                        user_o, Wp, bq, Wp + DD, bv, Wp + 2 * DD, Wp + 3 * DD, a1, Wp + 4 * DD, Wp + 5 * DD, bm,
-                                                       item_emb, scores, sig, B, K, D, nR, n_entity, (hipStream_t)stream),
+                                                       item_emb, scores, sig, B, K, D, nR, n_entity, order, (hipStream_t)stream),
                           who);
     }
     if (!out0 || !z2) return fail(-1, "%s: the two-launch variant (MVIN_L2_FOLD_TWO=1) needs the out0 / z2 scratch rows", who);
@@ -1149,9 +1184,15 @@
             rc = mvin_fold_tables(reinterpret_cast<const float*>(a->entity_emb), a->enc_entity, a->enc_relation, a->t0, a->W0, a->b0, a->W1, a->b1,
                                   a->W2, a->b2, a->A0, a->a0, a->Wmix, a->bmix, a->A1, a->K, D, a->n_entity, nR, a->fold_ws, stream);
         if (rc) return rc;
-        return mvin_score_l2_folded_fwd(a->fold_ws, a->enc_entity, a->enc_relation, a->items, nullptr, a->t0, a->t1, a->user_o, a->user_o, a->A1,
-                                        a->a1, a->Wmix, a->B, a->K, D, a->n_entity, nR, a->nagg0, a->nagg1, a->item_emb, a->scores, a->sig,
-                                        stream);
+        const int32_t* order = nullptr;
+        if (fold_order_applies(D, a->K, a->B)) {
+            rc = hip_result(mvin::launch_order_by_key(a->items, nullptr, a->B, reinterpret_cast<int32_t*>(a->nagg1), a->parents, (hipStream_t)stream), who);
+            if (rc) return rc;
+            order = a->parents;
+        }
+        return score_l2_folded_impl("mvin_score_l2_folded_fwd", a->fold_ws, a->enc_entity, a->enc_relation, a->items, nullptr, order, a->t0, a->t1,
+                                    a->user_o, a->user_o, a->A1, a->a1, a->Wmix, a->B, a->K, D, a->n_entity, nR, a->nagg0, a->nagg1, a->item_emb,
+                                    a->scores, a->sig, stream);
     }
     const bool enc = a->enc_entity && a->enc_relation && mvin::fused_packed_supported(D, a->K);
     const bool d32 = mvin::fused_d32_supported(D, a->K);
diff --git a/mvin_amd/csrc/mvin_fused_agg.h b/mvin_amd/csrc/mvin_fused_agg.h
--- a/mvin_amd/csrc/mvin_fused_agg.h
+++ b/mvin_amd/csrc/mvin_fused_agg.h
@@ -128,6 +128,7 @@
     uint64_t table_bytes, adj_bytes;
     int K, nR, pid_stride;
     unsigned max_id;
+    int reuse;
     int dbg;
     const float* tables;
     const float* t0;
diff --git a/mvin_amd/csrc/mvin_fused_agg.hip b/mvin_amd/csrc/mvin_fused_agg.hip
--- a/mvin_amd/csrc/mvin_fused_agg.hip
+++ b/mvin_amd/csrc/mvin_fused_agg.hip
@@ -267,6 +267,7 @@
 
 constexpr int kFoldTraceBatches = 16, kFoldTraceSlots = 20;
 __device__ long long g_fold_trace[kFoldTraceBatches * kFoldTraceSlots];
+__device__ unsigned long long g_fold_steps[2];
 
 template <int K, int MODE, bool TRACE = false>
 __global__ __launch_bounds__(kAggWaves * 64, 3) void score_l2_folded_kernel(FoldArgs a) {
@@ -302,6 +303,7 @@
     const int64_t nbatch = (a.B + 15) >> 4;
     const int64_t nwaves = (int64_t)gridDim.x * kAggWaves;
     int traced = 0;
+    int n_loaded = 0, n_reused = 0;
     auto stamp = [&](int slot, bool drain) {
         if constexpr (TRACE) {
             if (drain) asm volatile("s_waitcnt vmcnt(0)" ::: "memory");
@@ -315,20 +317,29 @@
         float* sLw = reinterpret_cast<float*>(reinterpret_cast<unsigned*>(sUV + 16 * kAggUvLd) + 4 * (K + kAggPad)) + g * (K + kAggPad);
         const unsigned c16 = (unsigned)c * 16u;
         unsigned xn = 0;
+        int prq = 0, on = 0;
         f32x4 qn[4];
-        auto fetch_batch = [&](int64_t b) {
-            const int64_t prn = min((min(b, nbatch - 1) << 4) + c, a.B - 1);
+        auto slot_of = [&](int64_t b) { return min((min(b, nbatch - 1) << 4) + c, a.B - 1); };
+        auto pair_of = [&](int64_t slot) { return (int)min((unsigned)a.order[slot], (unsigned)(a.B - 1)); };
+        auto fetch_batch = [&](int64_t b, bool ahead) {
+            int64_t prn = slot_of(b);
+            if (a.order) prn = ahead ? on : pair_of(prn);
+            prq = (int)prn;
             xn = (unsigned)a.items[prn * a.pid_stride];
             const char* qrow = reinterpret_cast<const char*>(a.q) + (size_t)((unsigned)prn * (unsigned)(D * 4) + (unsigned)g * 16u);
 #pragma unroll
             for (int nt = 0; nt < 4; ++nt) qn[nt] = *reinterpret_cast<const f32x4*>(qrow + 64 * nt);
         };
-        if constexpr (PIPE) fetch_batch((int64_t)blockIdx.x * kAggWaves + wave);
+        if constexpr (PIPE) fetch_batch((int64_t)blockIdx.x * kAggWaves + wave, false);
         for (int64_t batch = (int64_t)blockIdx.x * kAggWaves + wave; batch < nbatch; batch += nwaves) {
             const int64_t p_base = batch << 4;
             stamp(0, false);
-            const int64_t pr = min(p_base + c, a.B - 1);
+            int64_t pr = min(p_base + c, a.B - 1);
             const bool cvalid = p_base + c < a.B;
+            if (a.order) {
+                if constexpr (PIPE) pr = prq;
+                else pr = pair_of(pr);
+            }
             unsigned x0u;
             if constexpr (PIPE) x0u = xn;
             else x0u = (unsigned)a.items[pr * a.pid_stride];
@@ -431,6 +442,15 @@
             stamp(2, false);
 
             const int nquad = (a.dbg & 8) ? 0 : (int)((min((int64_t)16, a.B - p_base) + 3) >> 2);
+            unsigned same = 0;
+            if constexpr (PIPE) {
+                if (a.reuse && p_base + 16 <= a.B) {
+                    const int xp = __builtin_amdgcn_ds_bpermute(((lane - 4) & 63) << 2, x0c);
+                    const unsigned m = (unsigned)__builtin_amdgcn_ballot_w64(c >= 4 && xp == x0c);
+#pragma unroll
+                    for (int it = 1; it < 4; ++it) same |= (((m >> (4 * it)) & 0xFu) == 0xFu ? 1u : 0u) << it;
+                }
+            }
             auto issue = [&](const unsigned* lo, int k, float4 (&r)[4]) {
                 const uint4 o4 = *reinterpret_cast<const uint4*>(lo + k);
                 r[0] = agg_row4(aggG, o4.x + c16), r[1] = agg_row4(aggG, o4.y + c16);
@@ -466,26 +486,42 @@
             };
             if constexpr (PIPE) {
                 int kmax = lists(q0, 0, 0);
+                int cur = 0;
+                float4 r0[4] = {}, r1[4] = {}, r2[4] = {};
                 for (int it = 0; it < nquad; ++it) {
                     stamp(3 + 3 * it, false);
-                    const int cur = (it & 1) ? lb : 0;
+                    const bool rep = (same >> it) & 1u, rep_n = (same >> (it + 1)) & 1u;
                     float* rowT = sUV + (4 * it + g) * kAggUvLd + 4 * c;
                     const float4 vv = *reinterpret_cast<const float4*>(rowT + D);
                     const f32x2 v01 = {vv.x, vv.y}, v23 = {vv.z, vv.w};
                     f32x2 a01 = {0.f, 0.f}, a23 = {0.f, 0.f};
                     const int kr = (kmax + 7) & ~7;
-                    float4 r0[4], r1[4], r2[4];
+                    constexpr bool held = false;
                     auto wts = [&](int k) { return *reinterpret_cast<const float4*>(sLw + cur + k); };
                     const float4 s0 = q0.s0;
-                    if (it > 0 && it + 1 < nquad) q1 = quad_load(it + 1);
-                    issue(sLo + cur, 0, r0);
-                    issue(sLo + cur, 4, r1);
-                    if (kr > 8) issue(sLo + cur, 8, r2);
+                    if (it > 0 && it + 1 < nquad && !rep_n) q1 = quad_load(it + 1);
+                    if (!(rep && held)) {
+                        issue(sLo + cur, 0, r0);
+                        issue(sLo + cur, 4, r1);
+                        if (kr > 8) issue(sLo + cur, 8, r2);
+                    }
                     stamp(4 + 3 * it, true);
                     __builtin_amdgcn_sched_barrier(0);
-                    int kmax_n = 0;
-                    if (db && it + 1 < nquad) kmax_n = lists(q1, it + 1, lb - cur);
+                    int kmax_n = kmax;
+                    if (db && it + 1 < nquad && !rep_n) kmax_n = lists(q1, it + 1, lb - cur);
                     __builtin_amdgcn_sched_barrier(0);
+                    if (held) {
+                        sum4(r0, wts(0), v01, v23, a01, a23);
+                        __builtin_amdgcn_sched_barrier(0);
+                        sum4(r1, wts(4), v01, v23, a01, a23);
+                        __builtin_amdgcn_sched_barrier(0);
+                        if (kr > 8) {
+                            const float4 zr[4] = {};
+                            sum4(r2, wts(8), v01, v23, a01, a23);
+                            __builtin_amdgcn_sched_barrier(0);
+                            sum4(zr, wts(12), v01, v23, a01, a23);
+                        }
+                    } else
                     for (int k0 = 0; k0 < kr; k0 += 24) {
                         sum4(r0, wts(k0), v01, v23, a01, a23);
                         __builtin_amdgcn_sched_barrier(0);
@@ -520,9 +556,10 @@
                     const float4 o0 = make_float4(fmaxf(s0.x + tt.x, 0.f), fmaxf(s0.y + tt.y, 0.f), fmaxf(s0.z + tt.z, 0.f), fmaxf(s0.w + tt.w, 0.f));
                     *reinterpret_cast<float4*>(rowT) = o0;
                     *reinterpret_cast<float4*>(rowT + D) = make_float4(a01[0] + o0.x, a01[1] + o0.y, a23[0] + o0.z, a23[1] + o0.w);
-                    if (!db && it + 1 < nquad) kmax_n = lists(q1, it + 1, 0);
+                    if (!db && it + 1 < nquad && !rep_n) kmax_n = lists(q1, it + 1, 0);
                     kmax = kmax_n;
-                    q0 = q1;
+                    if (!rep_n) q0 = q1, cur = lb - cur;
+                    if constexpr (TRACE) n_reused += rep ? 1 : 0, n_loaded += rep ? 0 : 1;
                     stamp(5 + 3 * it, false);
                 }
             } else {
@@ -559,12 +596,16 @@
                                                   fmaxf(qd.s0.w + tt.w, 0.f));
                     *reinterpret_cast<float4*>(rowT) = o0;
                     *reinterpret_cast<float4*>(rowT + D) = make_float4(a01[0] + o0.x, a01[1] + o0.y, a23[0] + o0.z, a23[1] + o0.w);
+                    if constexpr (TRACE) ++n_loaded;
                     stamp(5 + 3 * it, false);
                 }
             }
             __builtin_amdgcn_fence(__ATOMIC_RELEASE, "wavefront");
             __builtin_amdgcn_wave_barrier();
             __builtin_amdgcn_fence(__ATOMIC_ACQUIRE, "wavefront");
+            if constexpr (PIPE) {
+                if (a.order) on = pair_of(slot_of(batch + nwaves));
+            }
             {
                 f32x4 zb[4], ob[4], o2[4], m0r[4], uor[4];
                 auto m0_load = [&]() {
@@ -579,7 +620,7 @@
                 };
                 auto late2 = [&](auto s_) {
                     if constexpr (PIPE && decltype(s_)::value == 0) m0_load();
-                    if constexpr (PIPE && decltype(s_)::value == 1) fetch_batch(batch + nwaves);
+                    if constexpr (PIPE && decltype(s_)::value == 1) fetch_batch(batch + nwaves, true);
                     if constexpr (PIPE && decltype(s_)::value == 2) uo_load();
                 };
 #pragma unroll
@@ -638,6 +679,21 @@
     };
     if (fast) run(std::true_type{});
     else run(std::false_type{});
+    if constexpr (TRACE) {
+        if (lane == 0) {
+            atomicAdd(&g_fold_steps[0], (unsigned long long)n_loaded);
+            atomicAdd(&g_fold_steps[1], (unsigned long long)n_reused);
+        }
+    }
+}
+
+hipError_t fold_read_steps(long long* host_dst) {
+    unsigned long long v[2] = {0, 0};
+    hipError_t e = hipMemcpyFromSymbol(v, HIP_SYMBOL(g_fold_steps), sizeof(v));
+    if (e != hipSuccess) return e;
+    host_dst[0] = (long long)v[0], host_dst[1] = (long long)v[1];
+    v[0] = v[1] = 0;
+    return hipMemcpyToSymbol(HIP_SYMBOL(g_fold_steps), v, sizeof(v));
 }
 
 hipError_t fold_read_trace(long long* host_dst, size_t n) {
@@ -705,7 +761,7 @@
                                   const float* t1, const float* q, const float* user_o, const float* Wq, const float* bq, const float* Wv,
                                   const float* bv, const float* Wqm, const float* A1, const float* a1, const float* Wm1, const float* Wm2,
                                   const float* bm, float* item_emb, float* scores, float* sig, int64_t B, int K, int D, int nR, int n_entity,
-                                  hipStream_t st) {
+                                  const int32_t* order, hipStream_t st) {
     FoldArgs f{};
     f.agg = agg, f.M0 = M0, f.adj_e = adj_e, f.adj_r = adj_r, f.items = items, f.pid_stride = pid_stride, f.t1 = t1, f.q = q, f.user_o = user_o;
     f.Wq = Wq, f.bq = bq, f.Wv = Wv, f.bv = bv, f.Wqm = Wqm, f.A1 = A1, f.a1 = a1, f.Wm1 = Wm1, f.Wm2 = Wm2, f.bm = bm;
@@ -713,7 +769,10 @@
     f.table_bytes = (uint64_t)n_entity * (uint64_t)D * 4, f.adj_bytes = (uint64_t)n_entity * (uint64_t)K * 4;
     static const char* dbg = getenv("MVIN_FOLD_DBG");
     f.dbg = dbg ? atoi(dbg) : 0;
-    if (D == 32) return launch_score_l2_folded_d32(f, st);
+    static const bool reuse = !(getenv("MVIN_FOLD_REUSE") && atoi(getenv("MVIN_FOLD_REUSE")) == 0);
+    f.reuse = reuse ? 1 : 0;
+    if (D == 32) return order ? hipErrorInvalidValue : launch_score_l2_folded_d32(f, st);
+    f.order = order;
     switch (K) {
         case 16: return launch_fold_k<16>(f, st);
         case 32: return launch_fold_k<32>(f, st);
diff --git a/mvin_amd/csrc/mvin_kernels.h b/mvin_amd/csrc/mvin_kernels.h
--- a/mvin_amd/csrc/mvin_kernels.h
+++ b/mvin_amd/csrc/mvin_kernels.h
@@ -361,6 +361,7 @@
 hipError_t kas_read_trace(long long* host_dst, size_t n);
 hipError_t kaf_read_trace(long long* host_dst, size_t n);
 hipError_t fold_read_trace(long long* host_dst, size_t n);
+hipError_t fold_read_steps(long long* host_dst);
 hipError_t launch_key_addr(const KeyAddrArgs& a, int table_bf16, hipStream_t st);
 bool key_addr_stream_supported(const KeyAddrArgs& a, int table_bf16);
 hipError_t launch_key_addr_stream(const KeyAddrArgs& a, int table_bf16, hipStream_t st);
@@ -468,7 +469,7 @@
                                   const float* t1, const float* q, const float* user_o, const float* Wq, const float* bq, const float* Wv,
                                   const float* bv, const float* Wqm, const float* A1, const float* a1, const float* Wm1, const float* Wm2,
                                   const float* bm, float* item_emb, float* scores, float* sig, int64_t B, int K, int D, int nR, int n_entity,
-                                  hipStream_t st);
+                                  const int32_t* order, hipStream_t st);
 hipError_t launch_gather_attn_l2_agg(const FusedL2Args& a, hipStream_t st);
 hipError_t launch_gather_attn_l2_d32(const FusedL2Args& a, int table_bf16, hipStream_t st, bool encoded = false);
 bool fused_d16_supported(int D, int K);
diff --git a/mvin_amd/ops.py b/mvin_amd/ops.py
--- a/mvin_amd/ops.py
+++ b/mvin_amd/ops.py
@@ -802,6 +802,36 @@
     return item_emb, scores, sig
 
 
+def score_l2_folded_ordered(ws, enc_entity, enc_relation, items, t0, t1, q, user_o, A1, a1, Wmix, K, D, nR, n_entity, order,
+                            want_item_emb=True, check_order=True):
+    lib = _lib.load()
+    for t, dt, nm in ((ws, F32, "ws"), (enc_entity, I32, "enc_entity"), (enc_relation, I32, "enc_relation"),
+                      (items, torch.int64 if items.dtype == torch.int64 else I32, "items"), (t0, F32, "t0"), (t1, F32, "t1"), (q, F32, "q"),
+                      (user_o, F32, "user_o"), (A1, F32, "A1"), (a1, F32, "a1"), (Wmix, F32, "Wmix"), (order, I32, "order")):
+        _chk(t, dt, nm)
+    B = items.shape[0]
+    if ws.numel() != lib.mvin_fold_tables_elems(n_entity, D) or tuple(q.shape) != (B, D) or tuple(user_o.shape) != (B, D):
+        raise ValueError("score_l2_folded_ordered: the workspace of fold_tables(n_entity, D) and q, user_o [B, D] expected")
+    if order is None or tuple(order.shape) != (B,) or (check_order and not bool(torch.equal(
+            torch.sort(order.to(torch.int64)).values, torch.arange(B, device=order.device)))):
+        raise ValueError("score_l2_folded_ordered: order must be a permutation of the pairs (int32 [B])")
+    item_emb = torch.empty((B, D), dtype=F32, device=ws.device) if want_item_emb else None
+    scores = torch.empty((B,), dtype=F32, device=ws.device)
+    sig = torch.empty((B,), dtype=F32, device=ws.device)
+    i64 = items.dtype == torch.int64
+    _lib.check(lib.mvin_score_l2_folded_ordered_fwd(_p(ws), _p(enc_entity), _p(enc_relation), _p(items) if i64 else None,
+                                                    None if i64 else _p(items), _p(order), _p(t0), _p(t1), _p(q), _p(user_o), _p(A1), _p(a1),
+                                                    _p(Wmix), B, K, D, n_entity, nR, None, None, _p(item_emb), _p(scores), _p(sig), _stream()),
+               "mvin_score_l2_folded_ordered_fwd")
+    return item_emb, scores, sig
+
+
+def fold_step_counts():
+    buf = (C.c_longlong * 2)()
+    _lib.check(_lib.load().mvin_debug_read_fold_steps(buf), "mvin_debug_read_fold_steps")
+    return int(buf[0]), int(buf[1])
+
+
 def gather_mix(table, adj_entity, adj_relation, node_ids, rel_score_t, rowbias, nodes, nodes_per_group, K, nR,
                relu=False):
     lib = _lib.load()
```
